# xiph/daala

Measured on NVIDIA H100. Metric: encoder Mpixels/s on 4K YUV420 intra, higher is better.
Workload: dtype int32

## Files before the change

### daala_b200/csrc/abi_host.cu

```cuda
#include <cuda_runtime.h>
#include <stdio.h>
#include <stdlib.h>
#include <string.h>

#include <stddef.h>

#include <mutex>

#include "daala_b200.h"
#include "frame_transform.h"

extern "C" {
int daala_b200_launch_forward(const FrameXformParams* prm, int nplanes, cudaStream_t stream);
int daala_b200_launch_forward_no_tma(const FrameXformParams* prm, int nplanes, cudaStream_t stream);
int daala_b200_launch_inverse(const FrameXformParams* prm, int nplanes, cudaStream_t stream);
int daala_b200_launch_inverse_lapped_only(const FrameXformParams* prm, int nplanes, cudaStream_t stream);
int daala_b200_launch_sb_postfilter_store(const FrameXformParams* prm, int nplanes, cudaStream_t stream);
int daala_b200_launch_plane_sb_filter(int32_t* c, int stride, int nhsb, int nvsb, int xdec, int ydec,
                                      int post, cudaStream_t stream);
int daala_b200_launch_block_transform(int32_t* blocks, int count, int ln, int mode, cudaStream_t stream);
int daala_b200_launch_filter4(int32_t* v, long count, int post, cudaStream_t stream);
int daala_b200_launch_haar_blocks(int32_t* blocks, int count, int ln, int inverse, cudaStream_t stream);
int daala_b200_pvq_helper_launch(void* buf, int op, void* stream);
int daala_b200_pvq_helper_bytes(void);
int daala_b200_launch_lapfilter(int32_t* v, long count, int n, int post, cudaStream_t stream);
int daala_b200_launch_split_filter(int32_t* blocks, int count, int n, int post, int hfilter, int vfilter,
                                   cudaStream_t stream);
}

namespace {

[[noreturn]] void fatal(const char* what, cudaError_t err) {
  fprintf(stderr, "libdaala_b200: fatal: %s: %s (no CPU fallback exists)\n", what,
          cudaGetErrorString(err));
  abort();
}

#define CK(call)                                    \
  do {                                              \
    cudaError_t e_ = (call);                        \
    if (e_ != cudaSuccess) fatal(#call, e_);        \
  } while (0)

struct HostCtx {
  cudaStream_t stream = nullptr;
  void* pinned = nullptr;
  void* dev = nullptr;
  size_t cap = 0;
  std::mutex mu;

  void ensure(size_t bytes) {
    if (!stream) {
      int n = 0;
      cudaError_t e = cudaGetDeviceCount(&n);
      if (e != cudaSuccess || n == 0) fatal("cudaGetDeviceCount", e == cudaSuccess ? cudaErrorNoDevice : e);
      CK(cudaStreamCreateWithFlags(&stream, cudaStreamNonBlocking));
    }
    if (bytes > cap) {
      size_t ncap = cap ? cap : (size_t)1 << 20;
      while (ncap < bytes) ncap <<= 1;
      if (pinned) CK(cudaFreeHost(pinned));
      if (dev) CK(cudaFree(dev));
      CK(cudaMallocHost(&pinned, ncap));
      CK(cudaMalloc(&dev, ncap));
      cap = ncap;
    }
  }
  void h2d(size_t bytes) { CK(cudaMemcpyAsync(dev, pinned, bytes, cudaMemcpyHostToDevice, stream)); }
  void d2h(size_t bytes) {
    CK(cudaMemcpyAsync(pinned, dev, bytes, cudaMemcpyDeviceToHost, stream));
    CK(cudaStreamSynchronize(stream));
  }
};

HostCtx& ctx() {
  static HostCtx c;
  return c;
}

void check_launch(int rc, const char* what) {
  if (rc != 0) fatal(what, (cudaError_t)rc);
}

void dct1d(int ln, bool inverse, od_coeff* out, int out_stride, const od_coeff* in, int in_stride) {
  HostCtx& c = ctx();
  std::lock_guard<std::mutex> g(c.mu);
  const int n = 1 << ln;
  c.ensure(sizeof(od_coeff) * n * n);
  od_coeff* p = (od_coeff*)c.pinned;
  memset(p, 0, sizeof(od_coeff) * n * n);
  for (int i = 0; i < n; i++) p[i] = in[i * in_stride];
  c.h2d(sizeof(od_coeff) * n * n);
  check_launch(daala_b200_launch_block_transform((int32_t*)c.dev, 1, ln, inverse ? 3 : 2, c.stream),
               "block_transform(1d)");
  c.d2h(sizeof(od_coeff) * n);
  for (int i = 0; i < n; i++) out[i * out_stride] = p[i];
}

void haar2d(int ln, bool inverse, od_coeff* out, int out_stride, const od_coeff* in, int in_stride) {
  HostCtx& c = ctx();
  std::lock_guard<std::mutex> g(c.mu);
  const int n = 1 << ln;
  c.ensure(sizeof(od_coeff) * n * n);
  od_coeff* p = (od_coeff*)c.pinned;
  for (int i = 0; i < n; i++) memcpy(p + i * n, in + (size_t)i * in_stride, sizeof(od_coeff) * n);
  c.h2d(sizeof(od_coeff) * n * n);
  check_launch(daala_b200_launch_haar_blocks((int32_t*)c.dev, 1, ln, inverse ? 1 : 0, c.stream), "haar_blocks");
  c.d2h(sizeof(od_coeff) * n * n);
  for (int i = 0; i < n; i++) memcpy(out + (size_t)i * out_stride, p + i * n, sizeof(od_coeff) * n);
}

void dct2d(int ln, bool inverse, od_coeff* out, int out_stride, const od_coeff* in, int in_stride) {
  HostCtx& c = ctx();
  std::lock_guard<std::mutex> g(c.mu);
  const int n = 1 << ln;
  c.ensure(sizeof(od_coeff) * n * n);
  od_coeff* p = (od_coeff*)c.pinned;
  for (int i = 0; i < n; i++) memcpy(p + i * n, in + (size_t)i * in_stride, sizeof(od_coeff) * n);
  c.h2d(sizeof(od_coeff) * n * n);
  check_launch(daala_b200_launch_block_transform((int32_t*)c.dev, 1, ln, inverse ? 1 : 0, c.stream),
               "block_transform(2d)");
  c.d2h(sizeof(od_coeff) * n * n);
  for (int i = 0; i < n; i++) memcpy(out + (size_t)i * out_stride, p + i * n, sizeof(od_coeff) * n);
}

void filter4(bool post, od_coeff* out, const od_coeff* in) {
  HostCtx& c = ctx();
  std::lock_guard<std::mutex> g(c.mu);
  c.ensure(sizeof(od_coeff) * 4);
  memcpy(c.pinned, in, sizeof(od_coeff) * 4);
  c.h2d(sizeof(od_coeff) * 4);
  check_launch(daala_b200_launch_filter4((int32_t*)c.dev, 1, post, c.stream), "filter4");
  c.d2h(sizeof(od_coeff) * 4);
  memcpy(out, c.pinned, sizeof(od_coeff) * 4);
}

void lapfilter_n(int n, bool post, od_coeff* out, const od_coeff* in) {
  HostCtx& c = ctx();
  std::lock_guard<std::mutex> g(c.mu);
  c.ensure(sizeof(od_coeff) * n);
  memcpy(c.pinned, in, sizeof(od_coeff) * n);
  c.h2d(sizeof(od_coeff) * n);
  check_launch(daala_b200_launch_lapfilter((int32_t*)c.dev, 1, n, post, c.stream), "lapfilter");
  c.d2h(sizeof(od_coeff) * n);
  memcpy(out, c.pinned, sizeof(od_coeff) * n);
}

void split_filter(bool post, od_coeff* c0, int stride, int bs, int hfilter, int vfilter) {
  HostCtx& c = ctx();
  std::lock_guard<std::mutex> g(c.mu);
  const int n = 4 << bs;
  c.ensure(sizeof(od_coeff) * n * n);
  od_coeff* p = (od_coeff*)c.pinned;
  for (int i = 0; i < n; i++) memcpy(p + i * n, c0 + (size_t)i * stride, sizeof(od_coeff) * n);
  c.h2d(sizeof(od_coeff) * n * n);
  check_launch(daala_b200_launch_split_filter((int32_t*)c.dev, 1, n, post, hfilter, vfilter, c.stream),
               "split_filter");
  c.d2h(sizeof(od_coeff) * n * n);
  for (int i = 0; i < n; i++) memcpy(c0 + (size_t)i * stride, p + i * n, sizeof(od_coeff) * n);
}

void plane_sb_filter(bool post, od_coeff* c0, int stride, int nhsb, int nvsb, int xdec, int ydec) {
  HostCtx& c = ctx();
  std::lock_guard<std::mutex> g(c.mu);
  const int w = (nhsb * 64) >> xdec, h = (nvsb * 64) >> ydec;
  const size_t bytes = sizeof(od_coeff) * (size_t)w * h;
  c.ensure(bytes);
  od_coeff* p = (od_coeff*)c.pinned;
  for (int i = 0; i < h; i++) memcpy(p + (size_t)i * w, c0 + (size_t)i * stride, sizeof(od_coeff) * w);
  c.h2d(bytes);
  check_launch(daala_b200_launch_plane_sb_filter((int32_t*)c.dev, w, nhsb, nvsb, xdec, ydec, post, c.stream),
               "plane_sb_filter");
  c.d2h(bytes);
  for (int i = 0; i < h; i++) memcpy(c0 + (size_t)i * stride, p + (size_t)i * w, sizeof(od_coeff) * w);
}

}

extern "C" {

#define DAALA_B200_DCT(N, LN)                                                                     \
  void od_bin_fdct##N(od_coeff* y, const od_coeff* x, int xstride) { dct1d(LN, false, y, 1, x, xstride); } \
  void od_bin_idct##N(od_coeff* x, int xstride, const od_coeff* y) { dct1d(LN, true, x, xstride, y, 1); }  \
  void od_bin_fdct##N##x##N(od_coeff* y, int ystride, const od_coeff* x, int xstride) {          \
    dct2d(LN, false, y, ystride, x, xstride);                                                    \
  }                                                                                              \
  void od_bin_idct##N##x##N(od_coeff* x, int xstride, const od_coeff* y, int ystride) {          \
    dct2d(LN, true, x, xstride, y, ystride);                                                     \
  }
DAALA_B200_DCT(4, 2)
DAALA_B200_DCT(8, 3)
DAALA_B200_DCT(16, 4)
DAALA_B200_DCT(32, 5)
DAALA_B200_DCT(64, 6)

void od_haar(od_coeff* y, int ystride, const od_coeff* x, int xstride, int ln) { haar2d(ln, false, y, ystride, x, xstride); }
void od_haar_inv(od_coeff* x, int xstride, const od_coeff* y, int ystride, int ln) { haar2d(ln, true, x, xstride, y, ystride); }

const od_dct_func_2d OD_FDCT_2D_CUDA[6] = {od_bin_fdct4x4,   od_bin_fdct8x8,   od_bin_fdct16x16,
                                           od_bin_fdct32x32, od_bin_fdct64x64, nullptr};
const od_dct_func_2d OD_IDCT_2D_CUDA[6] = {od_bin_idct4x4,   od_bin_idct8x8,   od_bin_idct16x16,
                                           od_bin_idct32x32, od_bin_idct64x64, nullptr};

void od_pre_filter4(od_coeff _y[4], const od_coeff _x[4]) { filter4(false, _y, _x); }
void od_post_filter4(od_coeff _x[4], const od_coeff _y[4]) { filter4(true, _x, _y); }

void od_pre_filter8(od_coeff _y[8], const od_coeff _x[8]) { lapfilter_n(8, false, _y, _x); }
void od_post_filter8(od_coeff _x[8], const od_coeff _y[8]) { lapfilter_n(8, true, _x, _y); }
void od_pre_filter16(od_coeff _y[16], const od_coeff _x[16]) { lapfilter_n(16, false, _y, _x); }
void od_post_filter16(od_coeff _x[16], const od_coeff _y[16]) { lapfilter_n(16, true, _x, _y); }
void od_pre_filter32(od_coeff _y[32], const od_coeff _x[32]) { lapfilter_n(32, false, _y, _x); }
void od_post_filter32(od_coeff _x[32], const od_coeff _y[32]) { lapfilter_n(32, true, _x, _y); }

const od_dct_func_2d OD_FDCT_2D_C[6] = {od_bin_fdct4x4,   od_bin_fdct8x8,   od_bin_fdct16x16,
                                        od_bin_fdct32x32, od_bin_fdct64x64, nullptr};
const od_dct_func_2d OD_IDCT_2D_C[6] = {od_bin_idct4x4,   od_bin_idct8x8,   od_bin_idct16x16,
                                        od_bin_idct32x32, od_bin_idct64x64, nullptr};
const od_fdct_func_1d OD_FDCT_1D[6] = {od_bin_fdct4, od_bin_fdct8, od_bin_fdct16, od_bin_fdct32, od_bin_fdct64, nullptr};
const od_idct_func_1d OD_IDCT_1D[6] = {od_bin_idct4, od_bin_idct8, od_bin_idct16, od_bin_idct32, od_bin_idct64, nullptr};

const od_filter_func OD_PRE_FILTER_CUDA[4] = {od_pre_filter4, od_pre_filter8, od_pre_filter16, od_pre_filter32};
const od_filter_func OD_POST_FILTER_CUDA[4] = {od_post_filter4, od_post_filter8, od_post_filter16, od_post_filter32};

const od_filter_func OD_PRE_FILTER[5] = {od_pre_filter4, od_pre_filter8, od_pre_filter16, od_pre_filter32, nullptr};
const od_filter_func OD_POST_FILTER[5] = {od_post_filter4, od_post_filter8, od_post_filter16, od_post_filter32, nullptr};
const int OD_FILTER_PARAMS4[4] = {85, 75, -15, 33};

int daala_b200_lapfilter(int32_t* v, long count, int n, int post, void* stream) {
  return daala_b200_launch_lapfilter(v, count, n, post, (cudaStream_t)stream);
}

void od_prefilter_split(od_coeff* c0, int stride, int bs, int f, int hfilter, int vfilter) {
  (void)f;
  split_filter(false, c0, stride, bs, hfilter, vfilter);
}

void od_postfilter_split(od_coeff* c0, int stride, int bs, int f, int q, unsigned char* skip,
                         int skip_stride, int hfilter, int vfilter) {
  (void)f; (void)q; (void)skip; (void)skip_stride;
  split_filter(true, c0, stride, bs, hfilter, vfilter);
}

void od_apply_prefilter_frame_sbs(od_coeff* c, int stride, int nhsb, int nvsb, int xdec, int ydec) {
  plane_sb_filter(false, c, stride, nhsb, nvsb, xdec, ydec);
}

void od_apply_postfilter_frame_sbs(od_coeff* c, int stride, int nhsb, int nvsb, int xdec, int ydec,
                                   int q, unsigned char* skip, int skip_stride) {
  (void)q; (void)skip; (void)skip_stride;
  plane_sb_filter(true, c, stride, nhsb, nvsb, xdec, ydec);
}

void od_mc_predict1fmv8_cuda(void* state, unsigned char* dst, const unsigned char* src, int systride,
                             int32_t mvx, int32_t mvy, int log_xblk_sz, int log_yblk_sz) {
  (void)state;
  HostCtx& c = ctx();
  std::lock_guard<std::mutex> g(c.mu);
  const int nx = 1 << log_xblk_sz, ny = 1 << log_yblk_sz;
  const int W = nx + 5, H = ny + 5;
  const size_t win = (size_t)W * H, job_off = (win + 15) & ~(size_t)15, out_off = job_off + 16;
  c.ensure(out_off + (size_t)nx * ny);
  unsigned char* p = (unsigned char*)c.pinned;
  const unsigned char* s0 = src + ((mvx >> 3) - 2) + (ptrdiff_t)((mvy >> 3) - 2) * systride;
  const int c_lo = (mvx & 7) ? 0 : 2, c_hi = (mvx & 7) ? W : 2 + nx;
  const int r_lo = (mvy & 7) ? 0 : 2, r_hi = (mvy & 7) ? H : 2 + ny;
  memset(p, 0, win);
  for (int r = r_lo; r < r_hi; r++) memcpy(p + (size_t)r * W + c_lo, s0 + (ptrdiff_t)r * systride + c_lo, c_hi - c_lo);
  daala_b200_match_job job;
  memset(&job, 0, sizeof(job));
  job.mvx = mvx & 7; job.mvy = mvy & 7; job.x0 = 2; job.y0 = 2; job.log_blk = (uint8_t)log_xblk_sz;
  memcpy(p + job_off, &job, sizeof(job));
  c.h2d(out_off);
  unsigned char* d = (unsigned char*)c.dev;
  check_launch(daala_b200_mc_predict1fmv_batch(d, W, d + out_off, nx * ny, (const daala_b200_match_job*)(d + job_off),
                                               1, log_yblk_sz, c.stream), "mc_predict1fmv");
  CK(cudaMemcpyAsync(p + out_off, d + out_off, (size_t)nx * ny, cudaMemcpyDeviceToHost, c.stream));
  CK(cudaStreamSynchronize(c.stream));
  memcpy(dst, p + out_off, (size_t)nx * ny);
}

static void blend_host(unsigned char* dst, int dystride, const unsigned char* src[4], int oc, int s, int lx, int ly) {
  HostCtx& c = ctx();
  std::lock_guard<std::mutex> g(c.mu);
  const int nx = 1 << lx, ny = 1 << ly, n2 = nx * ny;
  c.ensure((size_t)5 * n2);
  unsigned char* p = (unsigned char*)c.pinned;
  for (int k = 0; k < 4; k++) memcpy(p + (size_t)k * n2, src[k], n2);
  c.h2d((size_t)4 * n2);
  unsigned char* d = (unsigned char*)c.dev;
  check_launch(daala_b200_mc_blend_packed(d, n2, d + (size_t)4 * n2, nx, oc, s, lx, ly, c.stream), "mc_blend");
  CK(cudaMemcpyAsync(p + (size_t)4 * n2, d + (size_t)4 * n2, n2, cudaMemcpyDeviceToHost, c.stream));
  CK(cudaStreamSynchronize(c.stream));
  for (int j = 0; j < ny; j++) memcpy(dst + (size_t)j * dystride, p + (size_t)4 * n2 + (size_t)j * nx, nx);
}

void od_mc_blend_full8_cuda(unsigned char* dst, int dystride, const unsigned char* src[4], int log_xblk_sz,
                            int log_yblk_sz) {
  blend_host(dst, dystride, src, 0, 3, log_xblk_sz, log_yblk_sz);
}

void od_mc_blend_full_split8_cuda(unsigned char* dst, int dystride, const unsigned char* src[4], int c, int s,
                                  int log_xblk_sz, int log_yblk_sz) {
  blend_host(dst, dystride, src, c, s, log_xblk_sz, log_yblk_sz);
}

static int32_t match_host(int ln, int use_satd, const unsigned char* src, int systride, const unsigned char* ref,
                          int dystride) {
  HostCtx& c = ctx();
  std::lock_guard<std::mutex> g(c.mu);
  const int n = 1 << ln, n2 = n * n;
  const size_t job_off = (size_t)2 * n2, res_off = job_off + 16;
  c.ensure(res_off + 16);
  unsigned char* p = (unsigned char*)c.pinned;
  for (int j = 0; j < n; j++) {
    memcpy(p + (size_t)j * n, src + (ptrdiff_t)j * systride, n);
    memcpy(p + n2 + (size_t)j * n, ref + (ptrdiff_t)j * dystride, n);
  }
  daala_b200_match_job job;
  memset(&job, 0, sizeof(job));
  job.log_blk = (uint8_t)ln;
  memcpy(p + job_off, &job, sizeof(job));
  c.h2d(res_off);
  unsigned char* d = (unsigned char*)c.dev;
  check_launch(daala_b200_mc_match_candidates(d, n, d + n2, n, (const daala_b200_match_job*)(d + job_off), 1,
                                              use_satd, (int32_t*)(d + res_off), c.stream), "mc_match");
  CK(cudaMemcpyAsync(p + res_off, d + res_off, 4, cudaMemcpyDeviceToHost, c.stream));
  CK(cudaStreamSynchronize(c.stream));
  int32_t r;
  memcpy(&r, p + res_off, 4);
  return r;
}

#define DAALA_B200_MATCH(N, LN)                                                                            \
  int32_t od_mc_compute_sad8_##N##x##N##_cuda(const unsigned char* src, int systride, const unsigned char* ref, \
                                              int dystride) {                                             \
    return match_host(LN, 0, src, systride, ref, dystride);                                               \
  }                                                                                                       \
  int32_t od_mc_compute_satd8_##N##x##N##_cuda(const unsigned char* src, int systride, const unsigned char* ref, \
                                               int dystride) {                                            \
    return match_host(LN, 1, src, systride, ref, dystride);                                               \
  }
DAALA_B200_MATCH(4, 2)
DAALA_B200_MATCH(8, 3)
DAALA_B200_MATCH(16, 4)
DAALA_B200_MATCH(32, 5)
DAALA_B200_MATCH(64, 6)

struct PvqHelperBuf {
  int32_t args[16];
  int16_t a16[2][128];
  int32_t a32[2][128];
  int16_t qmi[128];
  double dargs[2];
};

static PvqHelperBuf* helper_begin(HostCtx& c) {
  if ((size_t)daala_b200_pvq_helper_bytes() != sizeof(PvqHelperBuf)) fatal("pvq helper layout", cudaErrorInvalidValue);
  c.ensure(sizeof(PvqHelperBuf));
  PvqHelperBuf* b = (PvqHelperBuf*)c.pinned;
  memset(b, 0, sizeof(*b));
  return b;
}

static void helper_run(HostCtx& c, int op) {
  c.h2d(sizeof(PvqHelperBuf));
  check_launch(daala_b200_pvq_helper_launch(c.dev, op, c.stream), "pvq_helper");
  c.d2h(sizeof(PvqHelperBuf));
}

#define HELPER_SCALAR(OP, ...)                      \
  HostCtx& c = ctx();                               \
  std::lock_guard<std::mutex> g_(c.mu);             \
  PvqHelperBuf* b = helper_begin(c);                \
  { int32_t v_[] = {__VA_ARGS__}; memcpy(b->args, v_, sizeof(v_)); } \
  helper_run(c, OP);

int16_t od_pvq_sin(int32_t x) { HELPER_SCALAR(0, x) return (int16_t)b->args[15]; }
int16_t od_pvq_cos(int32_t x) { HELPER_SCALAR(1, x) return (int16_t)b->args[15]; }
int32_t od_gain_expand(int32_t cg, int q0, int16_t beta) { HELPER_SCALAR(6, cg, q0, beta) return b->args[15]; }
int od_pvq_compute_max_theta(int32_t qcg, int16_t beta) { HELPER_SCALAR(8, qcg, beta) return b->args[15]; }
int32_t od_pvq_compute_theta(int t, int max_theta) { HELPER_SCALAR(9, t, max_theta) return b->args[15]; }
int od_pvq_compute_k(int32_t qcg, int itheta, int32_t theta, int noref, int n, int16_t beta, int nodesync) {
  (void)theta; (void)nodesync;
  HELPER_SCALAR(10, qcg, itheta, noref, n, beta)
  return b->args[15];
}

int od_vector_log_mag(const od_coeff* x, int n) {
  HostCtx& c = ctx();
  std::lock_guard<std::mutex> g_(c.mu);
  PvqHelperBuf* b = helper_begin(c);
  b->args[0] = n;
  memcpy(b->a32[0], x, sizeof(od_coeff) * n);
  helper_run(c, 2);
  return b->args[15];
}

int od_compute_householder(int16_t* r, int n, int32_t gr, int* sign, int shift) {
  HostCtx& c = ctx();
  std::lock_guard<std::mutex> g_(c.mu);
  PvqHelperBuf* b = helper_begin(c);
  b->args[0] = n; b->args[1] = gr; b->args[2] = shift;
  memcpy(b->a16[0], r, sizeof(int16_t) * n);
  helper_run(c, 3);
  memcpy(r, b->a16[0], sizeof(int16_t) * n);
  *sign = b->args[14];
  return b->args[15];
}

void od_apply_householder(int16_t* out, const int16_t* x, const int16_t* r, int n) {
  HostCtx& c = ctx();
  std::lock_guard<std::mutex> g_(c.mu);
  PvqHelperBuf* b = helper_begin(c);
  b->args[0] = n;
  memcpy(b->a16[0], r, sizeof(int16_t) * n);
  memcpy(b->a16[1], x, sizeof(int16_t) * n);
  helper_run(c, 4);
  memcpy(out, b->a16[1], sizeof(int16_t) * n);
}

void od_pvq_synthesis_partial(od_coeff* xcoeff, const od_coeff* ypulse, const int16_t* r, int n, int noref,
                              int32_t g, int32_t theta, int m, int s, const int16_t* qm_inv) {
  HostCtx& c = ctx();
  std::lock_guard<std::mutex> g_(c.mu);
  PvqHelperBuf* b = helper_begin(c);
  b->args[0] = n; b->args[1] = noref; b->args[2] = g; b->args[3] = theta; b->args[4] = m; b->args[5] = s;
  memcpy(b->a32[0], ypulse, sizeof(od_coeff) * (n - !noref));
  if (r) memcpy(b->a16[0], r, sizeof(int16_t) * n);
  memcpy(b->qmi, qm_inv, sizeof(int16_t) * n);
  helper_run(c, 5);
  memcpy(xcoeff, b->a32[1], sizeof(od_coeff) * n);
}

int32_t od_pvq_compute_gain(const int16_t* x, int n, int q0, int32_t* g, int16_t beta, int bshift) {
  HostCtx& c = ctx();
  std::lock_guard<std::mutex> g_(c.mu);
  PvqHelperBuf* b = helper_begin(c);
  b->args[0] = n; b->args[1] = q0; b->args[2] = beta; b->args[3] = bshift;
  memcpy(b->a16[0], x, sizeof(int16_t) * n);
  helper_run(c, 7);
  *g = b->args[14];
  return b->args[15];
}

int od_rdo_quant(od_coeff x, int q, double delta0, double pvq_norm_lambda) {
  HostCtx& c = ctx();
  std::lock_guard<std::mutex> g_(c.mu);
  PvqHelperBuf* b = helper_begin(c);
  b->args[0] = x; b->args[1] = q; b->dargs[0] = delta0; b->dargs[1] = pvq_norm_lambda;
  helper_run(c, 11);
  return b->args[15];
}

int daala_b200_forward_frame(const daala_b200_frame* f, int nplanes, void* stream) {
  return daala_b200_launch_forward(f, nplanes, (cudaStream_t)stream);
}
int daala_b200_forward_frame_no_tma(const daala_b200_frame* f, int nplanes, void* stream) {
  return daala_b200_launch_forward_no_tma(f, nplanes, (cudaStream_t)stream);
}
int daala_b200_inverse_frame(const daala_b200_frame* f, int nplanes, void* stream) {
  return daala_b200_launch_inverse(f, nplanes, (cudaStream_t)stream);
}
int daala_b200_inverse_frame_lapped(const daala_b200_frame* f, int nplanes, void* stream) {
  return daala_b200_launch_inverse_lapped_only(f, nplanes, (cudaStream_t)stream);
}
int daala_b200_sb_postfilter_store_frame(const daala_b200_frame* f, int nplanes, void* stream) {
  return daala_b200_launch_sb_postfilter_store(f, nplanes, (cudaStream_t)stream);
}
int daala_b200_plane_sb_filter(int32_t* c, int stride, int nhsb, int nvsb, int xdec, int ydec, int post,
                               void* stream) {
  return daala_b200_launch_plane_sb_filter(c, stride, nhsb, nvsb, xdec, ydec, post, (cudaStream_t)stream);
}
int daala_b200_haar_blocks(int32_t* blocks, int count, int ln, int inverse, void* stream) {
  return daala_b200_launch_haar_blocks(blocks, count, ln, inverse, (cudaStream_t)stream);
}

int daala_b200_block_transform(int32_t* blocks, int count, int ln, int mode, void* stream) {
  return daala_b200_launch_block_transform(blocks, count, ln, mode, (cudaStream_t)stream);
}

int daala_b200_device_count(void) {
  int n = 0;
  if (cudaGetDeviceCount(&n) != cudaSuccess) return 0;
  return n;
}

const char* daala_b200_version(void) { return "daala_b200 0.1 (sm_90a)"; }

}
```

### daala_b200/csrc/frame_transform.cu

```cuda
#include <cuda.h>
#include <cuda_runtime.h>
#include <cudaTypedefs.h>
#include <stdint.h>
#include <stdio.h>
#include <string.h>

#include "gen/dct_lifting.cuh"
#include "lapped_filter.cuh"
#include "frame_transform.h"

namespace daala_b200 {

#ifndef DAALA_XFORM_THREADS
#define DAALA_XFORM_THREADS 64
#endif
constexpr int kThreads = DAALA_XFORM_THREADS;
constexpr int kPostThreads = 128;
constexpr int kCtasPerSm = 512 / kThreads;
constexpr int kGridCap = 132 * 8;
constexpr int kMaxB = 64;
constexpr int kHalo = 2;
constexpr int kMaxT = kMaxB + 2 * kHalo;
constexpr int kMaxPitch = kMaxT + 1;

// ... 413 lines not shown
k_inverse_sb(const __grid_constant__ FrameXformParams prm) {
  __shared__ int tile_s[kMaxB * kMaxPitch];
  __shared__ SbLists lists;
  const PlaneXform& pl = prm.plane[blockIdx.y];
  if (pl.xdec == 0) inverse_sb_body<0>(prm, pl, tile_s, lists);
  else inverse_sb_body<1>(prm, pl, tile_s, lists);
}

template <int XDEC>
__device__ __forceinline__ void sb_postfilter_store_body(const FrameXformParams& prm,
                                                         const PlaneXform& pl, int* tile_s) {
  constexpr int B = kMaxB >> XDEC;
  constexpr int T = B + 2 * kHalo;
  constexpr int P = T + 1;
  const int sbx = blockIdx.x % prm.nhsb, sby = prm.sb_row0 + blockIdx.x / prm.nhsb;
  const int fr = blockIdx.z;
  const int32_t* lap = pl.lapped + fr * pl.lapped_frame_pitch;
  const int x0 = sbx * B, y0 = sby * B;
  const int pw = prm.nhsb * B, ph = prm.nvsb * B;
  const int32_t* core = lap + (size_t)y0 * pl.lapped_stride + x0;
  if (rows_aligned16(core, pl.lapped_stride)) {
    tile_copy4<B, P, false, kPostThreads>(tile_s + kHalo * P + kHalo, const_cast<int32_t*>(core), pl.lapped_stride);
    for (int i = threadIdx.x; i < 4 * T + 4 * B; i += kPostThreads) {
      int r, c;
      if (i < 4 * T) {
        const int k = i / T;
        r = k < 2 ? k : B + k;
        c = i - k * T;
      } else {
        const int j = i - 4 * T, k = j / B;
        c = k < 2 ? k : B + k;
        r = j - k * B + kHalo;
      }
      const int gx = x0 + c - kHalo, gy = y0 + r - kHalo;
      int v = 0;
      if (gx >= 0 && gx < pw && gy >= 0 && gy < ph) v = lap[(size_t)gy * pl.lapped_stride + gx];
      tile_s[r * P + c] = v;
    }
  } else {
    for (int i = threadIdx.x; i < T * T; i += kPostThreads) {
      int r = i / T, c = i - r * T;
      int gx = x0 + c - kHalo, gy = y0 + r - kHalo;
      int v = 0;
      if (gx >= 0 && gx < pw && gy >= 0 && gy < ph) v = lap[(size_t)gy * pl.lapped_stride + gx];
      tile_s[r * P + c] = v;
    }
  }
  __syncthreads();
  const bool left = sbx > 0, right = sbx + 1 < prm.nhsb;
  for (int i = threadIdx.x; i < 2 * T; i += kPostThreads) {
    int e = i >= T, r = i - e * T;
    if (e == 0 ? left : right) lap4_inplace<true>(tile_s + r * P + (e ? B : 0), 1);
  }
  __syncthreads();
  const bool top = sby > 0, bottom = sby + 1 < prm.nvsb;
  for (int i = threadIdx.x; i < 2 * B; i += kPostThreads) {
    int c = i % B + kHalo, e = i / B;
    if (e == 0 ? top : bottom) lap4_inplace<true>(tile_s + (e ? B : 0) * P + c, P);
  }
  __syncthreads();
  if (prm.post16[blockIdx.y]) {
    int16_t* d16 = prm.post16[blockIdx.y] + fr * pl.pixel_out_frame_pitch + (size_t)y0 * pl.pixel_out_stride + x0;
    for (int i = threadIdx.x; i < B * B / 2; i += kPostThreads) {
      int r = i / (B / 2), c2 = (i % (B / 2)) * 2;
      const int* p = tile_s + (r + kHalo) * P + c2 + kHalo;
      const unsigned w = ((unsigned)p[0] & 0xffffu) | ((unsigned)p[1] << 16);
      *reinterpret_cast<unsigned*>(d16 + (size_t)r * pl.pixel_out_stride + c2) = w;
    }
    return;
  }
  uint8_t* dst = pl.pixels_out + fr * pl.pixel_out_frame_pitch + (size_t)y0 * pl.pixel_out_stride + x0;
  for (int i = threadIdx.x; i < B * B / 4; i += kPostThreads) {
    int r = i / (B / 4), c4 = (i % (B / 4)) * 4;
    const int* p = tile_s + (r + kHalo) * P + c4 + kHalo;
    unsigned w = 0;
#pragma unroll
    for (int k = 0; k < 4; k++) {
      int v = ((p[k] + 8) >> 4) + 128;
      v = v < 0 ? 0 : (v > 255 ? 255 : v);
      w |= (unsigned)v << (8 * k);
    }
    *reinterpret_cast<unsigned*>(dst + (size_t)r * pl.pixel_out_stride + c4) = w;
  }
}

__global__ void __launch_bounds__(kPostThreads)
k_sb_postfilter_store(const __grid_constant__ FrameXformParams prm) {
  __shared__ int tile_s[kMaxT * kMaxPitch];
  const PlaneXform& pl = prm.plane[blockIdx.y];
  if (pl.xdec == 0) sb_postfilter_store_body<0>(prm, pl, tile_s);
  else sb_postfilter_store_body<1>(prm, pl, tile_s);
}

template <bool kPost>
__global__ void k_plane_sb_edges(int32_t* c, int stride, int nhsb, int nvsb, int sbw, int sbh,
                                 bool vertical_taps) {
  const int w = nhsb * sbw, h = nvsb * sbh;
  const int along = vertical_taps ? w : h;
  const int edges = (vertical_taps ? nvsb : nhsb) - 1;
  const long total = (long)along * edges;
  for (long i = blockIdx.x * (long)blockDim.x + threadIdx.x; i < total;
       i += (long)gridDim.x * blockDim.x) {
    int a = (int)(i % along), e = (int)(i / along) + 1;
    if (vertical_taps) lap4_inplace<kPost>(c + (size_t)(e * sbh - 2) * stride + a, stride);
    else lap4_inplace<kPost>(c + (size_t)a * stride + e * sbw - 2, 1);
  }
}

template <int L>
__global__ void __launch_bounds__(64)
k_block_transform(int32_t* blocks, int mode) {
  constexpr int N = 1 << L;
  constexpr int P = N + 5;
  __shared__ int t[N * P];
  int32_t* blk = blocks + (size_t)blockIdx.x * N * N;
  for (int i = threadIdx.x; i < N * N; i += blockDim.x) t[(i / N) * P + (i % N)] = blk[i];
  __syncthreads();
  const bool fwd = (mode & 1) == 0;
  const int passes = mode < 2 ? 2 : 1;
  for (int pass = 0; pass < passes; pass++) {
    bool cols = mode < 2 ? (fwd ? pass == 0 : pass == 1) : false;
    if (threadIdx.x < N) {
      int* p = cols ? t + threadIdx.x : t + threadIdx.x * P;
      int stride = cols ? P : 1;
      int v[N];
#pragma unroll
      for (int k = 0; k < N; k++) v[k] = p[k * stride];
      if (fwd) Lifting<N>::fwd(v); else Lifting<N>::inv(v);
#pragma unroll
      for (int k = 0; k < N; k++) p[k * stride] = v[k];
    }
    __syncthreads();
  }
  for (int i = threadIdx.x; i < N * N; i += blockDim.x) blk[i] = t[(i / N) * P + (i % N)];
}

__global__ void k_filter4_batch(int32_t* v, long count, int post) {
  for (long i = blockIdx.x * (long)blockDim.x + threadIdx.x; i < count;
       i += (long)gridDim.x * blockDim.x) {
    if (post) lap4_inplace<true>(v + 4 * i, 1); else lap4_inplace<false>(v + 4 * i, 1);
  }
}

template <int N>
__global__ void k_lapfilter_batch(int32_t* v, long count, int post) {
  for (long i = blockIdx.x * (long)blockDim.x + threadIdx.x; i < count; i += (long)gridDim.x * blockDim.x) {
    int t[N];
#pragma unroll
    for (int k = 0; k < N; k++) t[k] = v[i * N + k];
    if (post) LapFilter<N>::post(t); else LapFilter<N>::pre(t);
#pragma unroll
    for (int k = 0; k < N; k++) v[i * N + k] = t[k];
  }
}

__global__ void k_split_filter_batch(int32_t* blocks, int n, int post, int hfilter, int vfilter) {
  int32_t* b = blocks + (size_t)blockIdx.x * n * n;
  for (int phase = 0; phase < 2; phase++) {
    bool vertical_taps = post ? phase == 1 : phase == 0;
    if (vertical_taps ? hfilter : vfilter) {
      for (int i = threadIdx.x; i < n; i += blockDim.x) {
        if (vertical_taps) {
          if (post) lap4_inplace<true>(b + (n / 2 - 2) * n + i, n); else lap4_inplace<false>(b + (n / 2 - 2) * n + i, n);
        } else {
          if (post) lap4_inplace<true>(b + i * n + n / 2 - 2, 1); else lap4_inplace<false>(b + i * n + n / 2 - 2, 1);
        }
      }
    }
    __syncthreads();
  }
}

}

using namespace daala_b200;

template <bool kInverse>
__global__ void __launch_bounds__(256) k_haar_blocks(int32_t* __restrict__ blocks, int ln) {
  __shared__ int t[64 * 64];
  const int n = 1 << ln;
  int32_t* g = blocks + (size_t)blockIdx.x * n * n;
  if (!kInverse) {
    for (int i = threadIdx.x; i < n * n; i += 256) t[i] = g[i];
    __syncthreads();
    for (int level = 0; level < ln; level++) {
      const int np = n >> level >> 1;
      int keep[4];
      int q = 0;
      for (int idx = threadIdx.x; idx < np * np; idx += 256, q++) {
        const int i = idx / np, j = idx - i * np;
        int ll = t[2 * i * n + 2 * j], lh = t[(2 * i + 1) * n + 2 * j];
        int hl = t[2 * i * n + 2 * j + 1], hh = t[(2 * i + 1) * n + 2 * j + 1];
        ll += hl;
        hh -= lh;
        const int m = (ll - hh) >> 1;
        lh = m - lh;
        hl = m - hl;
        ll -= lh;
        hh += hl;
        keep[q] = ll;
        g[i * n + j + np] = lh;
        g[(i + np) * n + j] = hl;
        g[(i + np) * n + j + np] = hh;
      }
      __syncthreads();
      q = 0;
      for (int idx = threadIdx.x; idx < np * np; idx += 256, q++) {
        const int i = idx / np, j = idx - i * np;
        t[i * n + j] = keep[q];
      }
      __syncthreads();
    }
    if (threadIdx.x == 0) g[0] = t[0];
  } else {
    if (threadIdx.x == 0) t[0] = g[0];
    __syncthreads();
    for (int level = ln - 1; level >= 0; level--) {
      const int np = 1 << (ln - 1 - level);
      int a4[4], b4[4], c4[4], d4[4];
      int q = 0;
      for (int idx = threadIdx.x; idx < np * np; idx += 256, q++) {
        const int i = idx / np, j = idx - i * np;
        int ll = t[i * n + j], lh = g[i * n + j + np], hl = g[(i + np) * n + j], hh = g[(i + np) * n + j + np];
        ll += hl;
        hh -= lh;
        const int m = (ll - hh) >> 1;
        lh = m - lh;
        hl = m - hl;
        ll -= lh;
        hh += hl;
        a4[q] = ll; b4[q] = lh; c4[q] = hl; d4[q] = hh;
      }
      __syncthreads();
      q = 0;
      for (int idx = threadIdx.x; idx < np * np; idx += 256, q++) {
        const int i = idx / np, j = idx - i * np;
        t[2 * i * n + 2 * j] = a4[q];
        t[(2 * i + 1) * n + 2 * j] = b4[q];
        t[2 * i * n + 2 * j + 1] = c4[q];
        t[(2 * i + 1) * n + 2 * j + 1] = d4[q];
      }
      __syncthreads();
    }
    for (int i = threadIdx.x; i < n * n; i += 256) g[i] = t[i];
  }
}

extern "C" {

static bool encode_input_maps(const FrameXformParams* prm, int nplanes, TmaMaps* maps) {
  static PFN_cuTensorMapEncodeTiled_v12000 encode = nullptr;
  static bool tried = false;
  if (!tried) {
    tried = true;
    void* fn = nullptr;
    cudaDriverEntryPointQueryResult q;
    if (cudaGetDriverEntryPoint("cuTensorMapEncodeTiled", &fn, cudaEnableDefault, &q) == cudaSuccess &&
        q == cudaDriverEntryPointSuccess)
      encode = (PFN_cuTensorMapEncodeTiled_v12000)fn;
  }
  if (!encode) return false;
  memset(maps, 0, sizeof(*maps));
  for (int p = 0; p < nplanes; p++) {
    const PlaneXform& pl = prm->plane[p];
    const int B = kMaxB >> pl.xdec;
    const cuuint64_t w = (cuuint64_t)prm->nhsb * B, h = (cuuint64_t)prm->nvsb * B;
    const cuuint64_t fpitch = prm->nframes > 1 ? (cuuint64_t)pl.pixel_frame_pitch : w * h;
    if (((uintptr_t)pl.pixels & 15) || (pl.pixel_stride & 15) || (fpitch & 15) || pl.pixel_stride <= 0) return false;
    cuuint64_t dims[3] = {w, h, (cuuint64_t)prm->nframes};
    cuuint64_t strides[2] = {(cuuint64_t)pl.pixel_stride, fpitch};
    cuuint32_t box[3] = {(cuuint32_t)(pl.xdec ? RawTile<1>::width : RawTile<0>::width),
                         (cuuint32_t)(B + 2 * kHalo), 1};
    cuuint32_t estr[3] = {1, 1, 1};
    CUresult r = encode(&maps->plane[p], CU_TENSOR_MAP_DATA_TYPE_UINT8, 3, (void*)pl.pixels, dims, strides, box,
                        estr, CU_TENSOR_MAP_INTERLEAVE_NONE, CU_TENSOR_MAP_SWIZZLE_NONE,
                        CU_TENSOR_MAP_L2_PROMOTION_L2_128B, CU_TENSOR_MAP_FLOAT_OOB_FILL_NONE);
    if (r != CUDA_SUCCESS) return false;
  }
  return true;
}

int daala_b200_launch_forward(const FrameXformParams* prm, int nplanes, cudaStream_t stream) {
  dim3 grid(prm->nhsb * prm->sb_rows, nplanes, prm->nframes);
  TmaMaps maps;
  if (encode_input_maps(prm, nplanes, &maps))
    k_forward_sb_tma<<<grid, kThreads, 0, stream>>>(*prm, maps.plane[0], maps.plane[1], maps.plane[2]);
  else k_forward_sb<<<grid, kThreads, 0, stream>>>(*prm);
  return (int)cudaGetLastError();
}

int daala_b200_launch_forward_no_tma(const FrameXformParams* prm, int nplanes, cudaStream_t stream) {
  dim3 grid(prm->nhsb * prm->sb_rows, nplanes, prm->nframes);
  k_forward_sb<<<grid, kThreads, 0, stream>>>(*prm);
  return (int)cudaGetLastError();
}

int daala_b200_launch_inverse(const FrameXformParams* prm, int nplanes, cudaStream_t stream) {
  dim3 grid(prm->nhsb * prm->sb_rows, nplanes, prm->nframes);
  k_inverse_sb<<<grid, kThreads, 0, stream>>>(*prm);
  k_sb_postfilter_store<<<grid, kPostThreads, 0, stream>>>(*prm);
  return (int)cudaGetLastError();
}

int daala_b200_launch_inverse_lapped_only(const FrameXformParams* prm, int nplanes, cudaStream_t stream) {
  dim3 grid(prm->nhsb * prm->sb_rows, nplanes, prm->nframes);
  k_inverse_sb<<<grid, kThreads, 0, stream>>>(*prm);
  return (int)cudaGetLastError();
}

int daala_b200_launch_sb_postfilter_store(const FrameXformParams* prm, int nplanes, cudaStream_t stream) {
  dim3 grid(prm->nhsb * prm->sb_rows, nplanes, prm->nframes);
  k_sb_postfilter_store<<<grid, kPostThreads, 0, stream>>>(*prm);
  return (int)cudaGetLastError();
}

int daala_b200_launch_plane_sb_filter(int32_t* c, int stride, int nhsb, int nvsb, int xdec, int ydec,
                                      int post, cudaStream_t stream) {
  const int sbw = 64 >> xdec, sbh = 64 >> ydec;
  for (int phase = 0; phase < 2; phase++) {
    bool vertical_taps = post ? phase == 1 : phase == 0;
    long total = vertical_taps ? (long)nhsb * sbw * (nvsb - 1) : (long)nvsb * sbh * (nhsb - 1);
    if (total <= 0) continue;
    int blocks = (int)((total + 255) / 256);
    if (blocks > kGridCap) blocks = kGridCap;
    if (post) k_plane_sb_edges<true><<<blocks, 256, 0, stream>>>(c, stride, nhsb, nvsb, sbw, sbh, vertical_taps);
    else k_plane_sb_edges<false><<<blocks, 256, 0, stream>>>(c, stride, nhsb, nvsb, sbw, sbh, vertical_taps);
  }
  return (int)cudaGetLastError();
}

int daala_b200_launch_block_transform(int32_t* blocks, int count, int ln, int mode, cudaStream_t stream) {
  if (count <= 0) return 0;
  switch (ln) {
    case 2: k_block_transform<2><<<count, 64, 0, stream>>>(blocks, mode); break;
    case 3: k_block_transform<3><<<count, 64, 0, stream>>>(blocks, mode); break;
    case 4: k_block_transform<4><<<count, 64, 0, stream>>>(blocks, mode); break;
    case 5: k_block_transform<5><<<count, 64, 0, stream>>>(blocks, mode); break;
    case 6: k_block_transform<6><<<count, 64, 0, stream>>>(blocks, mode); break;
    default: return (int)cudaErrorInvalidValue;
  }
  return (int)cudaGetLastError();
}

int daala_b200_launch_haar_blocks(int32_t* blocks, int count, int ln, int inverse, cudaStream_t stream) {
  if (count <= 0) return 0;
  if (ln < 1 || ln > 6) return (int)cudaErrorInvalidValue;
  if (inverse) k_haar_blocks<true><<<count, 256, 0, stream>>>(blocks, ln);
  else k_haar_blocks<false><<<count, 256, 0, stream>>>(blocks, ln);
  return (int)cudaGetLastError();
}

int daala_b200_launch_filter4(int32_t* v, long count, int post, cudaStream_t stream) {
  if (count <= 0) return 0;
  int blocks = (int)((count + 255) / 256);
  if (blocks > kGridCap) blocks = kGridCap;
  k_filter4_batch<<<blocks, 256, 0, stream>>>(v, count, post);
  return (int)cudaGetLastError();
}

int daala_b200_launch_lapfilter(int32_t* v, long count, int n, int post, cudaStream_t stream) {
  if (count <= 0) return 0;
  int blocks = (int)((count + 127) / 128);
  if (blocks > kGridCap) blocks = kGridCap;
  if (n == 4) k_filter4_batch<<<blocks, 128, 0, stream>>>(v, count, post);
  else if (n == 8) k_lapfilter_batch<8><<<blocks, 128, 0, stream>>>(v, count, post);
  else if (n == 16) k_lapfilter_batch<16><<<blocks, 128, 0, stream>>>(v, count, post);
  else if (n == 32) k_lapfilter_batch<32><<<blocks, 128, 0, stream>>>(v, count, post);
  else return (int)cudaErrorInvalidValue;
  return (int)cudaGetLastError();
}

int daala_b200_launch_split_filter(int32_t* blocks, int count, int n, int post, int hfilter, int vfilter,
                                   cudaStream_t stream) {
  if (count <= 0) return 0;
  k_split_filter_batch<<<count, 64, 0, stream>>>(blocks, n, post, hfilter, vfilter);
  return (int)cudaGetLastError();
}

}
```

### daala_b200/csrc/kf_engine.cu

```cuda
#include <cuda_runtime.h>
#include <math.h>
#include <stdint.h>
#include <stdio.h>
#include <stdlib.h>
#include <string.h>

#include <algorithm>
#include <cmath>
#include <mutex>
#include <new>
#include <vector>

#include "daala_b200.h"
#include "dering_search.h"
#include "late_skip.h"
#include "mc_batch.h"
#include "gen/coding_order.inc"
#include "pvq_math.cuh"
#include "pvq_warp.cuh"
#include "pvq_common.cuh"

namespace daala_b200 {
namespace kf {

using namespace daala_b200::pvq;

enum Cnt {
  kNLuma = 0, kNChroma, kLumaCoefs, kChromaCoefs,
  kNItemsL = 4,
  kNItemsC = 7,
  kTotalHi = 14,
  kNHeads = 15,
  kNHeads0 = 16,
  kError = 17,
  kDepsDone = 18,
  kMcBadRef = 19,
  kMcBeyond = 20,
  kHeadLoL = 32,
  kHeadLoC = 64,
  kHeadHi = 96,
  kTailHi = 128,
  kDoneHi = 160,
  kHeadCh = 192,
  kWaiters = 224,
  kTraceN = 240,
  kCntWords = 256
};

constexpr int kTile = 1024;
constexpr int kMaxLevels = 4096;
constexpr int kLevelBins = kMaxLevels * 3;

struct Lists {
  const uint8_t* bsize;
  int bstride;
  long long bsize_pitch;
  int F, UW, UH;
  int u_row0, u_rows;
  int ntiles;
  int4* tile_sum;
  int32_t* unit_lbase;
  daala_b200_pvq_block* luma;
  daala_b200_pvq_block* chroma;
  int32_t* dep_top;
  int32_t* dep_left;
  int32_t* succ_bottom;
  int32_t* succ_right;
  uint32_t* items_l[3];
  uint32_t* items_c[3];
  uint32_t* heads;
  uint32_t* heads0;
  uint32_t* heads_raw;
  int32_t* head_bin;
  int32_t* head_hist;
  int32_t* head_cursor;
  int32_t* cnt;
  int32_t* lvl_hist;
  int32_t* lvl_cursor;
  uint32_t* lvl_items;
  int nlevels;
  int max_luma, max_chroma;
};

__device__ __forceinline__ int4 add4(int4 a, int4 b) { return make_int4(a.x + b.x, a.y + b.y, a.z + b.z, a.w + b.w); }

__device__ __forceinline__ int4 unit_counts(int b, int ux, int uy) {
  if (b == 0) return make_int4(4, 64, 1, 16);
  const int span = 1 << (b - 1);
  if ((ux & (span - 1)) | (uy & (span - 1))) return make_int4(0, 0, 0, 0);
  const int lc = b == 1 ? 64 : b == 2 ? 256 : 512;
  const int cc = b == 1 ? 16 : b == 2 ? 64 : b == 3 ? 256 : 512;
  return make_int4(1, lc, 1, cc);
}

__device__ __forceinline__ bool unit_of(const Lists& L, long long i, int* f, int* uy, int* ux, int* b) {
  const long long per = (long long)L.u_rows * L.UW;
  if (i >= per * L.F) return false;
  *f = (int)(i / per);
  const int r = (int)(i - (long long)*f * per);
  *uy = L.u_row0 + r / L.UW;
  *ux = r % L.UW;
  *b = L.bsize[*f * L.bsize_pitch + (long long)*uy * L.bstride + *ux];
  return true;
}

__global__ void __launch_bounds__(kTile) k_unit_tile_sums(const __grid_constant__ Lists L) {
  __shared__ int4 part[32];
  const long long i = (long long)blockIdx.x * kTile + threadIdx.x;
  int f, uy, ux, b;
  int4 v = make_int4(0, 0, 0, 0);
  if (unit_of(L, i, &f, &uy, &ux, &b)) v = unit_counts(b, ux, uy);
#pragma unroll
  for (int o = 16; o > 0; o >>= 1) {
    v.x += __shfl_xor_sync(0xffffffffu, v.x, o);
    v.y += __shfl_xor_sync(0xffffffffu, v.y, o);
    v.z += __shfl_xor_sync(0xffffffffu, v.z, o);
    v.w += __shfl_xor_sync(0xffffffffu, v.w, o);
  }
  if ((threadIdx.x & 31) == 0) part[threadIdx.x >> 5] = v;
  __syncthreads();
  if (threadIdx.x == 0) {
    int4 s = make_int4(0, 0, 0, 0);
    for (int w = 0; w < kTile / 32; w++) s = add4(s, part[w]);
    L.tile_sum[blockIdx.x] = s;
  }
}

__global__ void __launch_bounds__(1024) k_tile_scan(const __grid_constant__ Lists L) {
  __shared__ int4 part[1024];
  __shared__ int4 carry;
  const int t = threadIdx.x;
  if (t == 0) carry = make_int4(0, 0, 0, 0);
  __syncthreads();
  for (int base = 0; base < L.ntiles; base += 1024) {
    const int i = base + t;
    const int4 v = i < L.ntiles ? L.tile_sum[i] : make_int4(0, 0, 0, 0);
    part[t] = v;
    __syncthreads();
    for (int o = 1; o < 1024; o <<= 1) {
      const int4 a = t >= o ? part[t - o] : make_int4(0, 0, 0, 0);
      __syncthreads();
      part[t] = add4(part[t], a);
      __syncthreads();
    }
    const int4 incl = part[t], c = carry;
    if (i < L.ntiles) L.tile_sum[i] = make_int4(c.x + incl.x - v.x, c.y + incl.y - v.y, c.z + incl.z - v.z, c.w + incl.w - v.w);
    __syncthreads();
    if (t == 1023) carry = add4(c, incl);
    __syncthreads();
  }
  if (t == 0) {
    const int4 tot = carry;
    L.cnt[kNLuma] = tot.x;
    L.cnt[kLumaCoefs] = tot.y;
    L.cnt[kNChroma] = 2 * tot.z;
    L.cnt[kChromaCoefs] = 2 * tot.w;
    for (int c = 0; c < 3; c++) {
      L.cnt[kNItemsL + c] = 0;
      L.cnt[kNItemsC + c] = 0;
    }
    L.cnt[kTotalHi] = 0;
    L.cnt[kNHeads] = 0;
    L.cnt[kNHeads0] = 0;
    L.cnt[kDepsDone] = 0;
    L.cnt[kError] = tot.x > L.max_luma || 2 * tot.z > L.max_chroma ? 1 : 0;
  }
}

__device__ __forceinline__ void put_block(daala_b200_pvq_block* dst, int coef_off, int x0, int y0, int bs, int pli,
                                          int xdec, int frame) {
  int32_t* w = reinterpret_cast<int32_t*>(dst);
  w[0] = coef_off;
  w[1] = (x0 & 0xffff) | (y0 << 16);
  w[2] = bs | (pli << 8) | (xdec << 16) | (frame << 24);
}

__global__ void __launch_bounds__(kTile) k_unit_emit(const __grid_constant__ Lists L) {
  __shared__ int4 wsum[32];
  const long long i = (long long)blockIdx.x * kTile + threadIdx.x;
  const int lane = threadIdx.x & 31, warp = threadIdx.x >> 5;
  int f = 0, uy = 0, ux = 0, b = 0;
  const bool valid = unit_of(L, i, &f, &uy, &ux, &b);
  const int4 v = valid ? unit_counts(b, ux, uy) : make_int4(0, 0, 0, 0);
  int4 s = v;
#pragma unroll
  for (int o = 1; o < 32; o <<= 1) {
    int4 a;
    a.x = __shfl_up_sync(0xffffffffu, s.x, o);
    a.y = __shfl_up_sync(0xffffffffu, s.y, o);
    a.z = __shfl_up_sync(0xffffffffu, s.z, o);
    a.w = __shfl_up_sync(0xffffffffu, s.w, o);
    if (lane >= o) s = add4(s, a);
  }
  if (lane == 31) wsum[warp] = s;
  __syncthreads();
  int4 pre = L.tile_sum[blockIdx.x];
  for (int w = 0; w < warp; w++) pre = add4(pre, wsum[w]);
  pre = make_int4(pre.x + s.x - v.x, pre.y + s.y - v.y, pre.z + s.z - v.z, pre.w + s.w - v.w);
  if (!valid) return;
  L.unit_lbase[((long long)f * L.UH + uy) * L.UW + ux] = pre.x;
  if (v.x == 0) return;
  if (pre.x + v.x > L.max_luma || 2 * (pre.z + v.z) > L.max_chroma) return;
  if (b == 0) {
    for (int q = 0; q < 4; q++)
      put_block(L.luma + pre.x + q, pre.y + 16 * q, ux * 8 + (q & 1) * 4, uy * 8 + (q >> 1) * 4, 0, 0, 0, f);
  } else {
    put_block(L.luma + pre.x, pre.y, ux * 8, uy * 8, b, 0, 0, f);
  }
  const int cbs = (b > 1 ? b : 1) - 1;
  const int xd = 1 | (b == 0 ? 0x80 : 0);
  put_block(L.chroma + 2 * pre.z, 2 * pre.w, ux * 4, uy * 4, cbs, 1, xd, f);
  put_block(L.chroma + 2 * pre.z + 1, 2 * pre.w + v.w, ux * 4, uy * 4, cbs, 2, xd, f);
}

__device__ __forceinline__ int band_class(int band) { return band < 3 ? 0 : band < 6 ? 1 : 2; }

__device__ __forceinline__ int level_bin(int band, int bs, int x0, int y0, int y_first) {
  const int sh = bs + 2, bx = x0 >> sh, by = (y0 - y_first) >> sh;
  const int r = band % 3;
  const int lvl = band == 0 ? bx + by : r == 1 ? by : bx;
  return lvl * 3 + (2 - band_class(band));
}

__device__ __forceinline__ int append(uint32_t* list, int32_t* counter, bool pred, uint32_t v) {
  const unsigned m = __ballot_sync(__activemask(), pred);
  if (!pred) return -1;
  const int lane = threadIdx.x & 31, leader = __ffs(m) - 1;
  int base = 0;
  if (lane == leader) base = atomicAdd(counter, __popc(m));
  base = __shfl_sync(m, base, leader);
  const int pos = base + __popc(m & ((1u << lane) - 1u));
  list[pos] = v;
  return pos;
}

__device__ __forceinline__ int count_key(int32_t* ctr, int key) {
  const unsigned same = __match_any_sync(__activemask(), key);
  const int lane = threadIdx.x & 31, leader = __ffs(same) - 1;
  int base = 0;
  if (lane == leader) base = atomicAdd(&ctr[key], __popc(same));
  return __shfl_sync(same, base, leader) + __popc(same & ((1u << lane) - 1u));
}

constexpr int kChainCost0 = 7, kChainCost1 = 9, kChainCost2 = 18;
__device__ __forceinline__ int weight_bin(int len, int band) {
  const int c = band_class(band);
  const int w = len * (c == 0 ? kChainCost0 : c == 1 ? kChainCost1 : kChainCost2);
  return kLevelBins - 1 - min(w, kLevelBins - 1);
}

__device__ int chain_length(const Lists& L, const uint8_t* map, int x0, int y0, int bs, bool down) {
  const int nn = 4 << bs, y_end = (L.u_row0 + L.u_rows) * 8, x_end = L.UW * 8;
  int len = 1;
  for (int x = x0 + (down ? 0 : nn), y = y0 + (down ? nn : 0); x < x_end && y < y_end;
       x += down ? 0 : nn, y += down ? nn : 0, len++) {
    if (map[(long long)(y >> 3) * L.bstride + (x >> 3)] != bs) break;
    const int py = down ? y - 1 : y, px = down ? x : x - 1;
    if (map[(long long)(py >> 3) * L.bstride + (px >> 3)] != bs) break;
  }
  return len;
}

template <int kThreads>
__device__ __forceinline__ void scan_bins(int32_t* hist, int32_t* cursor) {
  __shared__ int part[kThreads];
  constexpr int kPer = kLevelBins / kThreads;
  const int t = threadIdx.x;
  int v[kPer], sum = 0;
#pragma unroll
  for (int i = 0; i < kPer; i++) {
    v[i] = __ldcg(hist + t * kPer + i);
    sum += v[i];
  }
  part[t] = sum;
  __syncthreads();
  for (int o = 1; o < kThreads; o <<= 1) {
    const int add = t >= o ? part[t - o] : 0;
    __syncthreads();
    part[t] += add;
    __syncthreads();
  }
  int run = part[t] - sum;
#pragma unroll
  for (int i = 0; i < kPer; i++) {
    hist[t * kPer + i] = run;
    cursor[t * kPer + i] = run;
    run += v[i];
  }
}

__global__ void __launch_bounds__(256) k_luma_deps(const __grid_constant__ Lists L) {
  const int n = min(L.cnt[kNLuma], L.max_luma);
  const int nth = gridDim.x * blockDim.x;
  for (int base = blockIdx.x * blockDim.x; base < n; base += nth) {
    const int blk = base + threadIdx.x;
    const bool in = blk < n;
    int bs = 0, top = -1, left = -1;
    if (in) {
      const daala_b200_pvq_block b = L.luma[blk];
      const int x0 = b.x0, y0 = b.y0, f = b.frame;
      bs = b.bs;
      const int nn = 4 << bs;
      const uint8_t* map = L.bsize + f * L.bsize_pitch;
      if (y0 - nn >= L.u_row0 * 8 && map[(long long)((y0 - 1) >> 3) * L.bstride + (x0 >> 3)] == bs) {
        const int ty = y0 - nn;
        top = L.unit_lbase[((long long)f * L.UH + (ty >> 3)) * L.UW + (x0 >> 3)] +
              (bs == 0 ? ((ty >> 2) & 1) * 2 + ((x0 >> 2) & 1) : 0);
      }
      if (x0 > 0 && map[(long long)(y0 >> 3) * L.bstride + ((x0 - 1) >> 3)] == bs) {
        const int lx = x0 - nn;
        left = L.unit_lbase[((long long)f * L.UH + (y0 >> 3)) * L.UW + (lx >> 3)] +
               (bs == 0 ? ((y0 >> 2) & 1) * 2 + ((lx >> 2) & 1) : 0);
      }
      L.dep_top[blk] = top;
      L.dep_left[blk] = left;
      if (top >= 0) L.succ_bottom[top] = blk;
      if (left >= 0) L.succ_right[left] = blk;
    }
    const int nb = in ? num_bands(bs) : 0;
    int len_down = 0, len_across = 0;
    if (nb > 1) {
      const daala_b200_pvq_block b = L.luma[blk];
      const uint8_t* map = L.bsize + b.frame * L.bsize_pitch;
      if (top < 0) len_down = chain_length(L, map, b.x0, b.y0, bs, true);
      if (left < 0) len_across = chain_length(L, map, b.x0, b.y0, bs, false);
    }
    int chain = 0;
    for (int band = 0; band < 9; band++) {
      const bool has = band < nb;
      const bool is_free = band == 3 || band == 6;
      const int r = band % 3;
      const bool waits = band == 0 ? (top >= 0 || left >= 0) : r == 1 ? top >= 0 : left >= 0;
      const uint32_t item = ((uint32_t)blk << 4) | band;
      if (band == 3 || band == 6) {
        append(L.items_l[band_class(band)], &L.cnt[kNItemsL + band_class(band)], has, item);
      } else if (band == 0) {
        append(L.heads0, &L.cnt[kNHeads0], has && !waits, item);
      } else {
        const int pos = append(L.heads_raw, &L.cnt[kNHeads], has && !waits, item);
        if (pos >= 0) {
          const int bin = weight_bin(r == 1 ? len_down : len_across, band);
          L.head_bin[pos] = bin;
          count_key(L.head_hist, bin);
        }
      }
      chain += has && !is_free;
      if (has && !is_free && L.lvl_hist) {
        const daala_b200_pvq_block b = L.luma[blk];
        atomicAdd(&L.lvl_hist[level_bin(band, bs, b.x0, b.y0, L.u_row0 * 8)], 1);
      }
    }
#pragma unroll
    for (int o = 16; o > 0; o >>= 1) chain += __shfl_xor_sync(0xffffffffu, chain, o);
    if ((threadIdx.x & 31) == 0 && chain) atomicAdd(&L.cnt[kTotalHi], chain);
  }
  __shared__ bool last;
  __threadfence();
  __syncthreads();
  if (threadIdx.x == 0) last = atomicAdd(&L.cnt[kDepsDone], 1) == (int)gridDim.x - 1;
  __syncthreads();
  if (last) {
    __threadfence();
    scan_bins<256>(L.head_hist, L.head_cursor);
  }
}

__global__ void __launch_bounds__(1024) k_level_scan(const __grid_constant__ Lists L) {
  scan_bins<1024>(L.lvl_hist, L.lvl_cursor);
}

__global__ void __launch_bounds__(256) k_level_scatter(const __grid_constant__ Lists L) {
  const int n = min(L.cnt[kNLuma], L.max_luma);
  for (int blk = blockIdx.x * blockDim.x + threadIdx.x; blk < n; blk += gridDim.x * blockDim.x) {
    const daala_b200_pvq_block b = L.luma[blk];
    const int nb = num_bands(b.bs);
    for (int band = 0; band < nb; band++) {
      if (band == 3 || band == 6) continue;
      const int pos = atomicAdd(&L.lvl_cursor[level_bin(band, b.bs, b.x0, b.y0, L.u_row0 * 8)], 1);
      L.lvl_items[pos] = ((uint32_t)blk << 4) | band;
    }
  }
}

__global__ void __launch_bounds__(256) k_chroma_items(const __grid_constant__ Lists L) {
  const int nh = L.cnt[kNHeads];
  for (int i = blockIdx.x * blockDim.x + threadIdx.x; i < nh; i += gridDim.x * blockDim.x)
    L.heads[count_key(L.head_cursor, L.head_bin[i])] = L.heads_raw[i];
  const int n = min(L.cnt[kNChroma], L.max_chroma);
  for (int blk = blockIdx.x * blockDim.x + threadIdx.x; blk < n; blk += gridDim.x * blockDim.x) {
    const int bs = L.chroma[blk].bs;
    const int nb = num_bands(bs);
    for (int band = 0; band < nb; band++) {
      const int c = band_class(band);
      const unsigned m = __activemask();
      const unsigned same = __match_any_sync(m, c);
      const int leader = __ffs(same) - 1, lane = threadIdx.x & 31;
      int base = 0;
      if (lane == leader) base = atomicAdd(&L.cnt[kNItemsC + c], __popc(same));
      base = __shfl_sync(same, base, leader);
      L.items_c[c][base + __popc(same & ((1u << lane) - 1u))] = ((uint32_t)blk << 4) | band;
    }
  }
}

__global__ void __launch_bounds__(256) k_luma_items(const __grid_constant__ Lists L) {
  const int n = min(L.cnt[kNLuma], L.max_luma);
  const int nth = gridDim.x * blockDim.x;
  for (int base = blockIdx.x * blockDim.x; base < n; base += nth) {
    const int blk = base + threadIdx.x;
    const int nb = blk < n ? num_bands(L.luma[blk].bs) : 0;
    for (int band = 0; band < 9; band++) {
      const int c = band_class(band);
      append(L.items_l[c], &L.cnt[kNItemsL + c], band < nb, ((uint32_t)blk << 4) | band);
    }
  }
}

struct Stage {
  daala_b200_pvq_params prm;
  const uint32_t* items[3];
  const uint32_t* heads;
  const uint32_t* heads0;
  uint32_t* ring;
  const int32_t* dep_top;
  const int32_t* dep_left;
  const int32_t* succ_bottom;
  const int32_t* succ_right;
  int32_t* join0;
  int32_t* cnt;
  int n_items_at, head_lo_at, n_blocks_at;
  int max_blocks;
  int16_t* sp_vec[3];
  int32_t* sp_lanes[3];
  int32_t* sp_uni[3];
  int16_t* sp_snap[3];
  int sp_slots[3];
  int sp_chunks[3];
  const int32_t* lvl_off;
  const uint32_t* lvl_items;
  int nlevels, lvl_slots;
  int16_t* lv_vec; int32_t* lv_lanes; int32_t* lv_uni; int16_t* lv_snap;
  int32_t* lv_bar;
  int32_t* pre_ev;
  int16_t* pre_snap;
  int max_waiters;
  int skip_lo;
  const double* rsqrt_tbl;
  int16_t* res_pack;
  const int32_t* cfl_plane;
  long long cfl_pitch;
  int cfl_stride;
  int32_t* dc_resid;
  const daala_b200_kf_frame_quant* fq;
#ifdef DAALA_B200_CHAIN_TRACE
  struct ChainTraceRec* trace;
  int trace_cap;
#endif
};

#ifdef DAALA_B200_CHAIN_TRACE
struct ChainTraceRec {
  unsigned long long t0, t1;
  uint32_t item;
  uint32_t cta;
  uint16_t sm;
  uint8_t bs;
  uint8_t kind;
  uint32_t pad;
};

__device__ __forceinline__ unsigned long long globaltimer() {
  unsigned long long t;
  asm volatile("mov.u64 %0, %%globaltimer;" : "=l"(t));
  return t;
}

__device__ __noinline__ void trace_item(const Stage& S, uint32_t item, int kind, unsigned long long t0, int lane) {
  __syncwarp();
  if (lane != 0) return;
  const unsigned long long t1 = globaltimer();
  const int i = atomicAdd(&S.cnt[kTraceN], 1);
  if (i >= S.trace_cap) return;
  uint32_t sm;
  asm volatile("mov.u32 %0, %%smid;" : "=r"(sm));
  ChainTraceRec r;
  r.t0 = t0;
  r.t1 = t1;
  r.item = item;
  r.cta = blockIdx.x;
  r.sm = (uint16_t)sm;
  r.bs = (uint8_t)S.prm.blocks[item >> 4].bs;
  r.kind = (uint8_t)kind;
  r.pad = 0;
  S.trace[i] = r;
}
#endif

enum { kGatherLuma = 0, kGatherChroma = 1, kGatherInter = 2 };
template <int kKind>
__global__ void __launch_bounds__(256) k_gather(const __grid_constant__ Stage S) {
  const daala_b200_pvq_params& prm = S.prm;
  const int n = min(S.cnt[S.n_blocks_at], S.max_blocks);
  const int lane = threadIdx.x & 31;
  const int nwarps = (gridDim.x * blockDim.x) >> 5;
  for (int blk = (blockIdx.x * blockDim.x + threadIdx.x) >> 5; blk < n; blk += nwarps) {
    const daala_b200_pvq_block b = prm.blocks[blk];
    const int ln = b.bs + 2;
    const int len = ln >= 5 ? 512 : 1 << (2 * ln);
    const int stride = prm.plane_stride[b.pli];
    const int32_t* src = prm.coef_plane[b.pli] + b.frame * prm.plane_frame_pitch[b.pli] + (size_t)b.y0 * stride + b.x0;
    int32_t* vin = prm.in + b.coef_off;
    if (kKind == kGatherLuma) {
      for (int i = lane; i < len; i += 32) vin[i] = i == 0 ? src[0] : src[scan_to_raster(i, ln, stride)];
    } else if (kKind == kGatherInter) {
      const int32_t* psrc = prm.pred_plane[b.pli] + b.frame * prm.plane_frame_pitch[b.pli] + (size_t)b.y0 * stride + b.x0;
      int32_t* vref = prm.ref + b.coef_off;
      for (int i = lane; i < len; i += 32) {
        const int at = i == 0 ? 0 : scan_to_raster(i, ln, stride);
        vin[i] = src[at];
        vref[i] = psrc[at];
      }
    } else {
      const int32_t* psrc = S.cfl_plane + b.frame * S.cfl_pitch + (size_t)b.y0 * S.cfl_stride + b.x0;
      int32_t* vref = prm.ref + b.coef_off;
      const int qoff = prm.qm_stride + ((((1 << (2 * b.bs)) - 1) << 4) / 3);
      int32_t xy = 0;
      for (int i = lane; i < len; i += 32) {
        const int32_t vi = i == 0 ? src[0] : src[scan_to_raster(i, ln, stride)];
        const int32_t vr = i == 0 ? psrc[0] : psrc[scan_to_raster(i, ln, S.cfl_stride)];
        vin[i] = vi;
        vref[i] = vr;
        if (i >= 1 && i < 16) {
          const int32_t rq = vr * prm.qm[qoff + i], inq = vi * prm.qm[qoff + i];
          xy += (int32_t)((rq * (int64_t)inq) >> ((kQmShift + 4) << 1));
        }
      }
#pragma unroll
      for (int o = 16; o > 0; o >>= 1) xy += __shfl_xor_sync(0xffffffffu, xy, o);
      const int flip = xy < 0;
      __syncwarp();
      if (flip) {
        const int end = band_start(num_bands(b.bs));
        for (int i = 1 + lane; i < end; i += 32) vref[i] = -vref[i];
      }
      if (lane == 0) prm.res_flip[blk] = flip;
    }
  }
}

__global__ void __launch_bounds__(256) k_cfl_plane(const __grid_constant__ Stage S, int32_t* pred_plane) {
  const daala_b200_pvq_params& prm = S.prm;
  const int n = min(S.cnt[S.n_blocks_at], S.max_blocks);
  const int lane = threadIdx.x & 31;
  const int nwarps = (gridDim.x * blockDim.x) >> 5;
  for (int blk = (blockIdx.x * blockDim.x + threadIdx.x) >> 5; blk < n; blk += nwarps) {
    const daala_b200_pvq_block b = prm.blocks[blk];
    if (b.pli != 1) continue;
    const int nn = 4 << b.bs;
    const int lstride = prm.plane_stride[0];
    const int32_t* luma = prm.coef_plane[0] + b.frame * prm.plane_frame_pitch[0] + (size_t)(2 * b.y0) * lstride + 2 * b.x0;
    int32_t* dst = pred_plane + b.frame * S.cfl_pitch + (size_t)b.y0 * S.cfl_stride + b.x0;
    if (b.xdec & 0x80) {
      const int scaling4[4][4] = {{128, 128, 100, 36}, {128, 80, 71, 35}, {100, 71, 35, 31}, {36, 35, 31, 18}};
      if (lane < 4) {
        const int x = lane & 1, y = lane >> 1;
        int ll = luma[(size_t)y * lstride + x], lh = luma[(size_t)y * lstride + x + 4];
        int hl = luma[(size_t)(y + 4) * lstride + x], hh = luma[(size_t)(y + 4) * lstride + x + 4];
        ll += lh; hh -= hl;
        const int t = (ll - hh) >> 1;
        hl = t - hl; lh = t - lh;
        ll -= hl; hh += lh;
        const int hs = x & 1, vs = y & 1;
        int r, c;
        r = 2 * y + vs; c = 2 * x + hs;         dst[(size_t)r * S.cfl_stride + c] = (scaling4[c][r] * ll + 64) >> 7;
        r = 2 * y + vs; c = 2 * x + 1 - hs;     dst[(size_t)r * S.cfl_stride + c] = (scaling4[c][r] * lh + 64) >> 7;
        r = 2 * y + 1 - vs; c = 2 * x + hs;     dst[(size_t)r * S.cfl_stride + c] = (scaling4[c][r] * hl + 64) >> 7;
        r = 2 * y + 1 - vs; c = 2 * x + 1 - hs; dst[(size_t)r * S.cfl_stride + c] = (scaling4[c][r] * hh + 64) >> 7;
      }
    } else {
      const int lim = nn > 32 ? 32 : nn;
      for (int i = lane; i < lim * lim; i += 32) {
        const int r = i / lim, c = i % lim;
        dst[(size_t)r * S.cfl_stride + c] = luma[(size_t)r * lstride + c];
      }
    }
  }
}

constexpr int kPersistThreads = 32;
constexpr int kPersistCtas = 32;
static_assert(kPersistCtas * (kPersistThreads / 32 * kSnapEntries * (int)sizeof(int16_t) + 1024) <= 228 * 1024,
              "k_pvq_persist's shared scratch does not fit kPersistCtas CTAs per SM");
constexpr uint32_t kNoItem = 0xffffffffu;
constexpr uint32_t kExit = 0xfffffffeu;

__device__ __forceinline__ int ld_relaxed(const int32_t* p) {
  int v;
  asm volatile("ld.relaxed.gpu.global.s32 %0, [%1];" : "=r"(v) : "l"(p) : "memory");
  return v;
}

__device__ __forceinline__ void push_chain(const Stage& S, int blk, int band) {
  const int pos = atomicAdd(&S.cnt[kTailHi], 1) - S.cnt[kNHeads0];
  st_release((int*)&S.ring[pos], (int)(((uint32_t)blk << 4) | band));
}

template <bool kIntra>
__device__ __forceinline__ uint32_t next_item(const Stage& S, int lane, int* done, bool* waiter) {
  int slot = -1, head = -1, lo = -1, nheads0 = 0, fin = -1;
  if (lane == 0) {
    const int n2 = S.cnt[S.n_items_at + 2], n1 = S.cnt[S.n_items_at + 1], n0 = S.cnt[S.n_items_at];
    const int nlo = S.skip_lo ? 0 : n0 + n1 + n2;
    if (kIntra) {
      nheads0 = S.cnt[kNHeads0];
      if (*done) {
        const int d = atomicAdd(&S.cnt[kDoneHi], *done) + *done;
        if (d == S.cnt[kNLuma]) {
          __threadfence();
          fin = ld_relaxed(&S.cnt[kTailHi]) - nheads0;
        }
      }
      if (ld_relaxed(&S.cnt[kHeadHi]) < ld_relaxed(&S.cnt[kTailHi])) slot = atomicAdd(&S.cnt[kHeadHi], 1);
      if (slot < 0 && ld_relaxed(&S.cnt[kHeadCh]) < S.cnt[kNHeads]) {
        const int h = atomicAdd(&S.cnt[kHeadCh], 1);
        if (h < S.cnt[kNHeads]) head = h;
      }
    }
    if (slot < 0 && head < 0 && ld_relaxed(&S.cnt[S.head_lo_at]) < nlo) {
      const int l = atomicAdd(&S.cnt[S.head_lo_at], 1);
      if (l < nlo) lo = l;
    }
    if (kIntra && slot < 0 && head < 0 && lo < 0) {
      if (!*waiter && atomicAdd(&S.cnt[kWaiters], 1) < S.max_waiters) *waiter = true;
      if (*waiter) slot = atomicAdd(&S.cnt[kHeadHi], 1);
    }
  }
  *done = 0;
  if (kIntra) {
    fin = __shfl_sync(0xffffffffu, fin, 0);
    if (fin >= 0) {
      const int nw = (gridDim.x * blockDim.x) >> 5;
#pragma unroll 1
      for (int i = lane; i <= nw; i += 32) st_release((int*)&S.ring[fin + i], (int)kExit);
    }
    head = __shfl_sync(0xffffffffu, head, 0);
    if (head >= 0) return S.heads[head];
  }
  slot = __shfl_sync(0xffffffffu, slot, 0);
  lo = __shfl_sync(0xffffffffu, lo, 0);
  if (slot >= 0) {
    nheads0 = __shfl_sync(0xffffffffu, nheads0, 0);
    if (slot < nheads0) return S.heads0[slot];
    uint32_t v;
    while ((v = (uint32_t)ld_acquire((const int*)&S.ring[slot - nheads0])) == kNoItem) __nanosleep(500);
    return v == kExit ? kNoItem : v;
  }
  if (lo >= 0) {
    const int n2 = S.cnt[S.n_items_at + 2], n1 = S.cnt[S.n_items_at + 1];
    return lo < n2 ? S.items[2][lo] : lo < n2 + n1 ? S.items[1][lo - n2] : S.items[0][lo - n2 - n1];
  }
  return kNoItem;
}

__device__ __forceinline__ void intra_band_ref(const Stage& S, int blk, int band, int coef_off, int lane) {
  const daala_b200_pvq_params& prm = S.prm;
  const int start = band_start(band);
  const int bn = band_start(band + 1) - start;
  const int r = band % 3;
  int top = -1, left = -1;
  if (band == 0 || r == 1) top = S.dep_top[blk];
  if (band == 0 || r == 2) left = S.dep_left[blk];
  if (band == 3 || band == 6) top = left = -1;
  const int32_t* ot = top >= 0 ? prm.out + prm.blocks[top].coef_off : nullptr;
  const int32_t* ol = left >= 0 ? prm.out + prm.blocks[left].coef_off : nullptr;
  bool low_from_top = false;
  if (band == 0) {
    double g1 = 0, g2 = 0;
    if (ot) { double a = __ldcg(ot + 2), bb = __ldcg(ot + 5), c = __ldcg(ot + 9); g1 += a * a; g1 += bb * bb; g1 += c * c; }
    if (ol) { double a = __ldcg(ol + 1), bb = __ldcg(ol + 4), c = __ldcg(ol + 7); g2 += a * a; g2 += bb * bb; g2 += c * c; }
    low_from_top = g1 > g2;
  }
  int32_t* vref = prm.ref + coef_off;
  for (int i = start + lane; i < start + bn; i += 32) {
    int r2, c2;
    scan_rc(i, &r2, &c2);
    int32_t p = 0;
    if (r2 == 0 && c2 > 0 && ot && (c2 >= 4 || low_from_top)) p = __ldcg(ot + i);
    if (c2 == 0 && r2 > 0 && ol && (r2 >= 4 || !low_from_top)) p = __ldcg(ol + i);
    vref[i] = p;
  }
}

template <bool kIntra>
__device__ __forceinline__ void run_item(const Stage& S, uint32_t item, int lane, int16_t* snap) {
  const daala_b200_pvq_params& prm = S.prm;
  const int blk = (int)(item >> 4), band = (int)(item & 15);
  const daala_b200_pvq_block b = prm.blocks[blk];
  const int bs = b.bs, pli = b.pli;
  const int start = band_start(band);
  const int bn = band_start(band + 1) - start;
  const size_t off = (size_t)b.coef_off + start;
  if (kIntra) intra_band_ref(S, blk, band, b.coef_off, lane);
  int qidx = bs * (bs + 1) + (band + 1) - (band + 1) / 3;
  int q = (prm.q0 * prm.pvq_qm_q4[pli][qidx]) >> 4;
  if (q < 1) q = 1;
  const int beta = (prm.use_masking && pli == 0 && bs > 0) ? kBeta15 : kBeta1;
  const int qoff = (b.xdec & 1 ? prm.qm_stride : 0) + ((((1 << (2 * bs)) - 1) << 4) / 3) + start;
  int itheta, max_theta, k;
  double skip_term;
  const bool pre = kIntra && S.pre_ev && band != 3 && band != 6;
  const int32_t* pev = pre ? S.pre_ev + (off >> 3) * kPreEvWords : nullptr;
  const int16_t* psn = pre ? S.pre_snap + 2 * off : nullptr;
  const int gain = quantise_band_warp<0>(lane, snap, S.rsqrt_tbl, prm.out + off, prm.in + off, prm.ref + off, bn, q,
                                         prm.y + off, &itheta, &max_theta, &k, beta, &skip_term, prm.is_keyframe, pli,
                                         prm.qm + qoff, prm.qm_inv + qoff, prm.pvq_norm_lambda, pev, psn);
  if (lane == 0) {
    const size_t r = (size_t)blk * 9 + band;
    prm.res_skip_term[r] = skip_term;
    short4 pk;
    pk.x = (short)gain; pk.y = (short)itheta; pk.z = (short)max_theta; pk.w = (short)k;
    reinterpret_cast<short4*>(S.res_pack)[r] = pk;
  }
}

struct ItemGeom {
  int blk, band, bn, q, beta, pli, qoff;
  size_t off;
};
__device__ __forceinline__ int band_q(const daala_b200_pvq_params& prm, const daala_b200_kf_frame_quant* fq, int frame,
                                      int pli, int qidx) {
  return fq ? (fq[frame].q0 * fq[frame].pvq_qm_q4[pli][qidx]) >> 4 : (prm.q0 * prm.pvq_qm_q4[pli][qidx]) >> 4;
}
__device__ __forceinline__ ItemGeom item_geom(const daala_b200_pvq_params& prm, uint32_t item,
                                              const daala_b200_kf_frame_quant* fq) {
  ItemGeom g;
  g.blk = (int)(item >> 4);
  g.band = (int)(item & 15);
  const daala_b200_pvq_block b = prm.blocks[g.blk];
  const int bs = b.bs;
  g.pli = b.pli;
  const int start = band_start(g.band);
  g.bn = band_start(g.band + 1) - start;
  g.off = (size_t)b.coef_off + start;
  const int qidx = bs * (bs + 1) + (g.band + 1) - (g.band + 1) / 3;
  int q = band_q(prm, fq, b.frame, g.pli, qidx);
  g.q = q < 1 ? 1 : q;
  g.beta = (prm.use_masking && g.pli == 0 && bs > 0) ? kBeta15 : kBeta1;
  g.qoff = (b.xdec & 1 ? prm.qm_stride : 0) + ((((1 << (2 * bs)) - 1) << 4) / 3) + start;
  return g;
}

template <int kPhase, bool kZeroRef, int kMode, bool kFq = false>
__global__ void __launch_bounds__(128) k_pvq_split(const __grid_constant__ Stage S, int cls, int chunk) {
  const daala_b200_pvq_params& prm = S.prm;
  const int lane = threadIdx.x & 31;
  const int slots = S.sp_slots[cls];
  const int first = chunk * slots;
  const int count = min(S.cnt[S.n_items_at + cls] - first, slots);
  const int vs = cls == 2 ? 128 : 32;
  const int nwarps = (gridDim.x * blockDim.x) >> 5;
  for (int i = (blockIdx.x * blockDim.x + threadIdx.x) >> 5; i < count; i += nwarps) {
    const ItemGeom g = item_geom(prm, S.items[cls][first + i], kFq ? S.fq : nullptr);
    int16_t* vec = S.sp_vec[cls] + (size_t)i * 3 * vs;
    int32_t* lanes = S.sp_lanes[cls] + (size_t)i * kCtxLaneWords * 16;
    int32_t* uni = S.sp_uni[cls] + (size_t)i * kCtxUniWords;
    int16_t* snap = S.sp_snap[cls] + (size_t)i * kMaxEvents * vs;
    const int32_t* r0 = kZeroRef ? nullptr : prm.ref + g.off;
    BandCtx B;
    if (kPhase == 0) {
      band_setup<kMode>(lane, B, prm.in + g.off, r0, g.bn, g.q, g.beta, prm.is_keyframe, g.pli, prm.qm + g.qoff,
                 prm.pvq_norm_lambda, S.rsqrt_tbl);
      band_ctx_store_setup(lane, B, g.bn, vec, vs, lanes, uni);
    } else if (kPhase == 1) {
      band_ctx_load_search(lane, B, g.bn, vec, vs, lanes);
      band_search<kMode>(lane, B, g.bn, snap, vs, S.rsqrt_tbl);
      band_ctx_store_search(lane, B, lanes);
    } else {
      band_ctx_load_finish(lane, B, g.bn, vec, vs, lanes, uni);
      int itheta, max_theta, k;
      double skip_term;
      const int gain = band_finish<kMode>(lane, B, snap, vs, prm.out + g.off, r0, g.bn, g.q, prm.y + g.off, &itheta, &max_theta, &k,
                                   g.beta, &skip_term, prm.is_keyframe, g.pli, prm.qm_inv + g.qoff, prm.pvq_norm_lambda);
      if (lane == 0) {
        const size_t r = (size_t)g.blk * 9 + g.band;
        prm.res_skip_term[r] = skip_term;
        short4 pk;
        pk.x = (short)gain; pk.y = (short)itheta; pk.z = (short)max_theta; pk.w = (short)k;
        reinterpret_cast<short4*>(S.res_pack)[r] = pk;
      }
    }
  }
}

template <int kMode>
__global__ void __launch_bounds__(128) k_pvq_prepass(const __grid_constant__ Stage S) {
  const daala_b200_pvq_params& prm = S.prm;
  __shared__ int16_t snap_all[4][2 * kMaxN];
  const int lane = threadIdx.x & 31;
  int16_t* snap = snap_all[threadIdx.x >> 5];
  const int nblk = min(S.cnt[S.n_blocks_at], S.max_blocks);
  const int nwarps = (gridDim.x * blockDim.x) >> 5;
  const int per = kMode == 2 ? 2 : 5;
  for (long long i = (blockIdx.x * blockDim.x + threadIdx.x) >> 5; i < (long long)nblk * per; i += nwarps) {
    const int blk = (int)(i / per), sel = (int)(i % per);
    const int band = kMode == 2 ? 7 + sel : (sel < 3 ? sel : sel + 1);
    if (band >= num_bands(prm.blocks[blk].bs)) continue;
    const ItemGeom g = item_geom(prm, ((uint32_t)blk << 4) | band, nullptr);
    BandCtx B;
    band_setup<kMode>(lane, B, prm.in + g.off, nullptr, g.bn, g.q, g.beta, prm.is_keyframe, g.pli, prm.qm + g.qoff,
                      prm.pvq_norm_lambda, S.rsqrt_tbl);
    band_search<kMode>(lane, B, g.bn, snap, kMaxN, S.rsqrt_tbl);
    band_noref_export(lane, B, g.bn, snap, kMaxN, S.pre_ev + (g.off >> 3) * kPreEvWords, S.pre_snap + 2 * g.off);
  }
}

__device__ __forceinline__ void grid_barrier(int32_t* bar, int* target, int nctas) {
  __syncthreads();
  if (threadIdx.x == 0) {
    *target += nctas;
    __threadfence();
    atomicAdd(bar, 1);
    while (ld_acquire(bar) < *target) {}
  }
  __syncthreads();
}

__global__ void __launch_bounds__(128, 4) k_pvq_levels(const __grid_constant__ Stage S) {
  const daala_b200_pvq_params& prm = S.prm;
  __shared__ int bar_target;
  if (threadIdx.x == 0) bar_target = 0;
  const int lane = threadIdx.x & 31;
  const int w = (blockIdx.x * blockDim.x + threadIdx.x) >> 5;
  const int nwarps = (gridDim.x * blockDim.x) >> 5;
  const int total = S.cnt[kTotalHi];
  constexpr int vs = 128;
  for (int lvl = 0; lvl < S.nlevels; lvl++) {
    const int base = S.lvl_off[lvl * 3];
    const int end = lvl + 1 < kMaxLevels ? S.lvl_off[(lvl + 1) * 3] : total;
    if (end - base > S.lvl_slots && threadIdx.x == 0 && blockIdx.x == 0) S.cnt[kError] = 2;
    const int n = min(end - base, S.lvl_slots);
    if (n <= 0) continue;
    for (int phase = 0; phase < 3; phase++) {
      for (int i = w; i < n; i += nwarps) {
        const uint32_t item = S.lvl_items[base + i];
        const ItemGeom g = item_geom(prm, item, nullptr);
        int16_t* vec = S.lv_vec + (size_t)i * 3 * vs;
        int32_t* lanes = S.lv_lanes + (size_t)i * kCtxLaneWords * 16;
        int32_t* uni = S.lv_uni + (size_t)i * kCtxUniWords;
        int16_t* snap = S.lv_snap + (size_t)i * kMaxEvents * vs;
        BandCtx B;
        if (phase == 0) {
          intra_band_ref(S, g.blk, g.band, (int)(g.off - band_start(g.band)), lane);
          band_setup<0>(lane, B, prm.in + g.off, prm.ref + g.off, g.bn, g.q, g.beta, prm.is_keyframe, g.pli,
                        prm.qm + g.qoff, prm.pvq_norm_lambda, S.rsqrt_tbl);
          band_ctx_store_setup(lane, B, g.bn, vec, vs, lanes, uni);
        } else if (phase == 1) {
          band_ctx_load_search(lane, B, g.bn, vec, vs, lanes);
          band_search<0>(lane, B, g.bn, snap, vs, S.rsqrt_tbl);
          band_ctx_store_search(lane, B, lanes);
        } else {
          band_ctx_load_finish(lane, B, g.bn, vec, vs, lanes, uni);
          int itheta, max_theta, k;
          double skip_term;
          const int gain = band_finish<0>(lane, B, snap, vs, prm.out + g.off, prm.ref + g.off, g.bn, g.q, prm.y + g.off,
                                          &itheta, &max_theta, &k, g.beta, &skip_term, prm.is_keyframe, g.pli,
                                          prm.qm_inv + g.qoff, prm.pvq_norm_lambda);
          if (lane == 0) {
            const size_t r = (size_t)g.blk * 9 + g.band;
            prm.res_skip_term[r] = skip_term;
            short4 pk;
            pk.x = (short)gain; pk.y = (short)itheta; pk.z = (short)max_theta; pk.w = (short)k;
            reinterpret_cast<short4*>(S.res_pack)[r] = pk;
          }
        }
      }
      grid_barrier(S.lv_bar, &bar_target, gridDim.x);
    }
  }
}

template <bool kIntra>
__global__ void __launch_bounds__(kPersistThreads, kPersistCtas) k_pvq_persist(const __grid_constant__ Stage S) {
  __shared__ __align__(16) int16_t snap_all[kPersistThreads / 32][kSnapEntries];
  const int lane = threadIdx.x & 31;
  int16_t* snap = snap_all[threadIdx.x >> 5];
  int done = 0;
  bool waiter = false;
  for (;;) {
    uint32_t item = next_item<kIntra>(S, lane, &done, &waiter);
    if (item == kNoItem) return;
#ifdef DAALA_B200_CHAIN_TRACE
    int kind = (item & 15) == 0 ? 0 : (item & 15) == 3 || (item & 15) == 6 ? 2 : 1;
#endif
    for (;;) {
      const int band = (int)(item & 15);
#ifdef DAALA_B200_CHAIN_TRACE
      const unsigned long long t0 = globaltimer();
#endif
      run_item<kIntra>(S, item, lane, snap);
#ifdef DAALA_B200_CHAIN_TRACE
      if (kIntra) trace_item(S, item, kind, t0, lane);
      kind = 3;
#endif
      if (!kIntra || band == 3 || band == 6) break;
      done += band == 0;
      __threadfence();
      __syncwarp();
      uint32_t next = kNoItem;
      if (lane == 0) {
        const int blk = (int)(item >> 4);
        if (band == 0) {
          const int nb[2] = {S.succ_bottom[blk], S.succ_right[blk]};
          for (int i = 0; i < 2; i++) {
            if (nb[i] < 0) continue;
            const int need = (S.dep_top[nb[i]] >= 0) + (S.dep_left[nb[i]] >= 0);
            if (need == 2 && atomicAdd(&S.join0[nb[i]], 1) != 1) continue;
            if (next == kNoItem) {
              next = (uint32_t)nb[i] << 4;
            } else {
              __threadfence();
              push_chain(S, nb[i], 0);
            }
          }
        } else {
          const int nb = band % 3 == 1 ? S.succ_bottom[blk] : S.succ_right[blk];
          if (nb >= 0) next = ((uint32_t)nb << 4) | band;
        }
      }
      next = __shfl_sync(0xffffffffu, next, 0);
      if (next == kNoItem) break;
      __threadfence();
      item = next;
    }
  }
}

__global__ void k_fill_rsqrt(double* tbl) {
  const int i = blockIdx.x * blockDim.x + threadIdx.x;
  if (i < kTableDoubles) pvq_fill_rsqrt_table(tbl, i);
}

__global__ void k_begin_pvq(int32_t* cnt, int luma) {
  if (threadIdx.x == 0 && blockIdx.x == 0) {
    if (luma) {
      cnt[kHeadLoL] = 0;
      cnt[kHeadHi] = 0;
      cnt[kTailHi] = cnt[kNHeads0];
      cnt[kDoneHi] = 0;
      cnt[kHeadCh] = 0;
      cnt[kWaiters] = 0;
#ifdef DAALA_B200_CHAIN_TRACE
      cnt[kTraceN] = 0;
#endif
    } else {
      cnt[kHeadLoC] = 0;
    }
  }
}

template <bool kInter>
__global__ void __launch_bounds__(256) k_finish_scatter(const __grid_constant__ Stage S) {
  const daala_b200_pvq_params& prm = S.prm;
  const int n = min(S.cnt[S.n_blocks_at], S.max_blocks);
  const int lane = threadIdx.x & 31;
  const int nwarps = (gridDim.x * blockDim.x) >> 5;
  for (int blk = (blockIdx.x * blockDim.x + threadIdx.x) >> 5; blk < n; blk += nwarps) {
    const daala_b200_pvq_block b = prm.blocks[blk];
    const int ln = b.bs + 2, nn = 1 << ln;
    const int len = ln >= 5 ? 512 : 1 << (2 * ln);
    const int stride = prm.plane_stride[b.pli];
    int32_t* dst = prm.coef_plane[b.pli] + b.frame * prm.plane_frame_pitch[b.pli] + (size_t)b.y0 * stride + b.x0;
    const int32_t* src = prm.out + b.coef_off;
    if (lane == 0) {
      const int nb = num_bands(b.bs);
      double sd = 0;
      for (int i = 0; i < nb; i++) sd += prm.res_skip_term[(size_t)blk * 9 + i];
      prm.res_skip_diff[blk] = sd;
      if (!kInter) {
        prm.out[b.coef_off] = prm.in[b.coef_off];
      } else {
        int dc_quant = band_q(prm, S.fq, b.frame, b.pli, b.bs * (b.bs + 1));
        if (dc_quant < 1) dc_quant = 1;
        const int32_t r = prm.ref[b.coef_off], diff = prm.in[b.coef_off] - r;
        int qdc = 0;
        if (abs(diff) >= dc_quant * 141 / 256) {
          const int half = ((dc_quant + 1) >> 1) - 1;
          qdc = (diff + (diff < 0 ? -half : half)) / dc_quant;
        }
        prm.out[b.coef_off] = dst[0] = qdc * dc_quant + r;
        prm.res_dc[blk] = qdc;
        if (S.dc_resid) S.dc_resid[blk] = diff;
      }
    }
    if (ln >= 5) {
      const int32_t* mdp = kInter ? prm.pred_plane[b.pli] + b.frame * prm.plane_frame_pitch[b.pli] + (size_t)b.y0 * stride + b.x0
                                  : nullptr;
      for (int i = lane; i < nn * nn; i += 32) {
        const size_t at = (size_t)(i >> ln) * stride + (i & (nn - 1));
        if (i) dst[at] = kInter ? mdp[at] : 0;
      }
      __syncwarp();
    }
    for (int i = lane + 1; i < len; i += 32) dst[scan_to_raster(i, ln, stride)] = src[i];
    const int32_t* y = prm.y + b.coef_off;
    for (int i = lane; i < len; i += 32) prm.y16[b.coef_off + i] = i ? (int16_t)y[i] : (int16_t)0;
  }
}

__global__ void k_dering_thresholds(const uint8_t* __restrict__ level, int32_t* __restrict__ thr_luma,
                                    int32_t* __restrict__ thr_chroma, int n, int4 tl_lo, int2 tl_hi, int4 tc_lo, int2 tc_hi,
                                    const uint8_t* __restrict__ coded, uint8_t* __restrict__ applied,
                                    const int32_t* __restrict__ frame_tbl, int nsb) {
  const int i = blockIdx.x * blockDim.x + threadIdx.x;
  if (i >= n) return;
  const int tl[6] = {tl_lo.x, tl_lo.y, tl_lo.z, tl_lo.w, tl_hi.x, tl_hi.y};
  const int tc[6] = {tc_lo.x, tc_lo.y, tc_lo.z, tc_lo.w, tc_hi.x, tc_hi.y};
  int g = level[i] < 6 ? level[i] : 5;
  if (coded) {
    if (!coded[i]) g = 0;
    applied[i] = (uint8_t)g;
  }
  if (frame_tbl) {
    const int32_t* t = frame_tbl + (size_t)(i / nsb) * 12;
    thr_luma[i] = t[g];
    thr_chroma[i] = t[6 + g];
  } else {
    thr_luma[i] = tl[g];
    thr_chroma[i] = tc[g];
  }
}

struct Fin {
  const daala_b200_pvq_block* blocks[2];
  const uint8_t* skip[2];
  const int32_t* dc[2];
  const int32_t* cnt;
  int max_blocks[2];
  const int32_t* d[3];
  const int32_t* md[3];
  int32_t* out[3];
  long long plane_pitch[3];
  int plane_stride[3];
  uint8_t* bskip[3];
  long long skip_pitch[3];
  int skip_stride;
  uint8_t* coded;
  int nhsb, nvsb;
  int q0;
  uint8_t pvq_qm_q4[3][32];
  const daala_b200_kf_frame_quant* fq;
};

__device__ __forceinline__ bool fin_block(const Fin& P, int i, int* list, int* blk) {
  const int nl = min(P.cnt[kNLuma], P.max_blocks[0]), nc = min(P.cnt[kNChroma], P.max_blocks[1]);
  if (i >= nl + nc) return false;
  *list = i >= nl;
  *blk = i >= nl ? i - nl : i;
  return true;
}

__global__ void __launch_bounds__(256) k_fin_patch(const __grid_constant__ Fin P) {
  const int lane = threadIdx.x & 31;
  const int nwarps = (gridDim.x * blockDim.x) >> 5;
  int list, blk;
  for (int i = (blockIdx.x * blockDim.x + threadIdx.x) >> 5; fin_block(P, i, &list, &blk); i += nwarps) {
    const daala_b200_pvq_block b = P.blocks[list][blk];
    const int ln = b.bs + 2, nn = 1 << ln;
    const int stride = P.plane_stride[b.pli];
    const size_t o = b.frame * P.plane_pitch[b.pli] + (size_t)b.y0 * stride + b.x0;
    const int32_t* src = (P.skip[list][blk] ? P.md[b.pli] : P.d[b.pli]) + o;
    const int32_t* mdp = P.md[b.pli] + o;
    int32_t* dst = P.out[b.pli] + o;
    const int qidx = b.bs * (b.bs + 1);
    int dc_quant = P.fq ? (P.fq[b.frame].q0 * P.fq[b.frame].pvq_qm_q4[b.pli][qidx]) >> 4 : (P.q0 * P.pvq_qm_q4[b.pli][qidx]) >> 4;
    if (dc_quant < 1) dc_quant = 1;
    const int32_t dc0 = mdp[0] + P.dc[list][blk] * dc_quant;
    for (int k = lane; k < nn * nn; k += 32) {
      const size_t at = (size_t)(k >> ln) * stride + (k & (nn - 1));
      dst[at] = k ? src[at] : dc0;
    }
  }
}

__global__ void __launch_bounds__(256) k_fin_skip_map(const __grid_constant__ Fin P) {
  const int lane = threadIdx.x & 31;
  const int nwarps = (gridDim.x * blockDim.x) >> 5;
  int list, blk;
  for (int i = (blockIdx.x * blockDim.x + threadIdx.x) >> 5; fin_block(P, i, &list, &blk); i += nwarps) {
    const daala_b200_pvq_block b = P.blocks[list][blk];
    const uint8_t s = P.skip[list][blk] && P.dc[list][blk] == 0;
    const int nu = 1 << b.bs;
    uint8_t* m = P.bskip[b.pli] + b.frame * P.skip_pitch[b.pli] + (size_t)(b.y0 >> 2) * P.skip_stride + (b.x0 >> 2);
    for (int k = lane; k < nu * nu; k += 32) m[(size_t)(k >> b.bs) * P.skip_stride + (k & (nu - 1))] = s;
    if (lane == 0 && b.pli == 0 && !s) P.coded[((size_t)b.frame * P.nvsb + (b.y0 >> 6)) * P.nhsb + (b.x0 >> 6)] = 1;
  }
}

struct PoolStore {
  const uint8_t* src[3];
  uint8_t* pool[3];
  long long plane_bytes[3];
  const int32_t* slot;
};

__global__ void __launch_bounds__(256) k_fin_pool_store(const __grid_constant__ PoolStore S) {
  const int f = blockIdx.y / 3, p = blockIdx.y - 3 * f;
  const int slot = S.slot[f];
  if (slot < 0) return;
  const long long n = S.plane_bytes[p] >> 4;
  const uint4* __restrict__ src = reinterpret_cast<const uint4*>(S.src[p] + f * S.plane_bytes[p]);
  uint4* __restrict__ dst = reinterpret_cast<uint4*>(S.pool[p] + slot * S.plane_bytes[p]);
  for (long long i = (long long)blockIdx.x * blockDim.x + threadIdx.x; i < n; i += (long long)gridDim.x * blockDim.x)
    dst[i] = src[i];
}

struct Sym {
  const uint8_t* bsize;
  int bstride;
  long long bsize_pitch;
  int F, nhsb, sb_rows, u_row0;
  int nsb;
  uint32_t* unit_rank;
  uint32_t* sb_cnt;
  int32_t* sb_base;
  uint32_t* order;
  longlong2* off;
  longlong2* tile;
  long long* tot;
  int ntiles, cap_blocks;
  long long cap_bands, cap_bytes;
  daala_b200_kf_sym_frame* index;
  daala_b200_kf_sym_block* blocks;
  short4* bands;
  uint8_t* pulses;
  const daala_b200_pvq_block* list[2];
  const short4* res[2];
  const int32_t* y[2];
  const double* skip_diff[2];
  const int32_t* flip;
  const int32_t* cnt;
  int max_luma, max_chroma;
  daala_b200_kf_sym_dc* dc;
  const int32_t* qdc[2];
  const int32_t* dc_resid[2];
  daala_b200_kf_late_skip* late_skip;
  const daala_b200_kf_late_skip* ls_block[2];
};

__device__ __forceinline__ int sym_band_bytes(int band, short4 r) {
  if (r.w <= 0) return 0;
  const int n = band_start(band + 1) - band_start(band) - (r.y != -1);
  return r.w > 127 ? 2 * n : n;
}

__global__ void __launch_bounds__(256) k_sym_rank(const __grid_constant__ Sym S) {
  const int lane = threadIdx.x & 31;
  const int sb = (blockIdx.x * blockDim.x + threadIdx.x) >> 5;
  if (sb >= S.F * S.nsb) return;
  const int f = sb / S.nsb, r = sb % S.nsb;
  const int sby = r / S.nhsb, sbx = r % S.nhsb;
  const int uw = S.nhsb * 8;
  uint32_t v[2];
  long long at[2];
  for (int h = 0; h < 2; h++) {
    const int m = 2 * lane + h;
    const int dx = (m & 1) | ((m >> 1) & 2) | ((m >> 2) & 4);
    const int dy = ((m >> 1) & 1) | ((m >> 2) & 2) | ((m >> 3) & 4);
    const int ux = sbx * 8 + dx, uy = S.u_row0 + sby * 8 + dy;
    const int b = S.bsize[f * S.bsize_pitch + (long long)uy * S.bstride + ux];
    const int4 c = unit_counts(b, ux, uy);
    v[h] = (uint32_t)c.x | ((uint32_t)c.z << 16);
    at[h] = ((long long)f * S.sb_rows * 8 + (uy - S.u_row0)) * uw + ux;
  }
  const uint32_t s = v[0] + v[1];
  uint32_t inc = s;
#pragma unroll
  for (int o = 1; o < 32; o <<= 1) {
    const uint32_t a = __shfl_up_sync(0xffffffffu, inc, o);
    if (lane >= o) inc += a;
  }
  S.unit_rank[at[0]] = inc - s;
  S.unit_rank[at[1]] = inc - s + v[0];
  if (lane == 31) S.sb_cnt[sb] = inc;
}

__global__ void __launch_bounds__(1024) k_sym_sb_scan(const __grid_constant__ Sym S) {
  __shared__ int part[1024];
  __shared__ int carry;
  const int t = threadIdx.x;
  const int n = S.F * S.nsb;
  if (t == 0) carry = 0;
  __syncthreads();
  for (int base = 0; base < n; base += 1024) {
    const int i = base + t;
    const uint32_t c = i < n ? S.sb_cnt[i] : 0u;
    const int v = (int)(c & 0xffff) + 2 * (int)(c >> 16);
    part[t] = v;
    __syncthreads();
    for (int o = 1; o < 1024; o <<= 1) {
      const int a = t >= o ? part[t - o] : 0;
      __syncthreads();
      part[t] += a;
      __syncthreads();
    }
    const int incl = part[t], c0 = carry;
    if (i < n) S.sb_base[i] = c0 + incl - v;
    __syncthreads();
    if (t == 1023) carry = c0 + incl;
    __syncthreads();
  }
  if (t == 0) S.tot[0] = min(carry, S.cap_blocks);
}

__global__ void __launch_bounds__(256) k_sym_place(const __grid_constant__ Sym S) {
  const int nl = min(S.cnt[kNLuma], S.max_luma), nc = min(S.cnt[kNChroma], S.max_chroma);
  const int uw = S.nhsb * 8;
  for (int i = blockIdx.x * blockDim.x + threadIdx.x; i < nl + nc; i += gridDim.x * blockDim.x) {
    const int ch = i >= nl;
    const int blk = ch ? i - nl : i;
    const daala_b200_pvq_block b = S.list[ch][blk];
    const int sh = ch ? 2 : 3;
    const int ux = b.x0 >> sh, uy = b.y0 >> sh;
    const int sb = b.frame * S.nsb + ((uy - S.u_row0) >> 3) * S.nhsb + (ux >> 3);
    const uint32_t rk = S.unit_rank[((long long)b.frame * S.sb_rows * 8 + (uy - S.u_row0)) * uw + ux];
    const uint32_t sc = S.sb_cnt[sb];
    int pos = S.sb_base[sb];
    if (!ch) pos += (int)(rk & 0xffff) + (b.bs == 0 ? ((b.y0 >> 2) & 1) * 2 + ((b.x0 >> 2) & 1) : 0);
    else pos += (int)(sc & 0xffff) + (b.pli - 1) * (int)(sc >> 16) + (int)(rk >> 16);
    if (pos >= S.cap_blocks) continue;
    S.order[pos] = (uint32_t)blk | (ch ? 0x80000000u : 0u);
    const short4* r = S.res[ch] + (size_t)blk * 9;
    const int nb = num_bands(b.bs);
    long long bytes = 0;
    for (int j = 0; j < nb; j++) bytes += sym_band_bytes(j, r[j]);
    S.off[pos] = make_longlong2(nb, bytes);
  }
}

__device__ __forceinline__ longlong2 add2(longlong2 a, longlong2 b) { return make_longlong2(a.x + b.x, a.y + b.y); }

__global__ void __launch_bounds__(kTile) k_sym_tile_sums(const __grid_constant__ Sym S) {
  __shared__ longlong2 part[32];
  const long long i = (long long)blockIdx.x * kTile + threadIdx.x;
  longlong2 v = i < S.tot[0] ? S.off[i] : make_longlong2(0, 0);
#pragma unroll
  for (int o = 16; o > 0; o >>= 1) {
    v.x += __shfl_xor_sync(0xffffffffu, v.x, o);
    v.y += __shfl_xor_sync(0xffffffffu, v.y, o);
  }
  if ((threadIdx.x & 31) == 0) part[threadIdx.x >> 5] = v;
  __syncthreads();
  if (threadIdx.x == 0) {
    longlong2 s = make_longlong2(0, 0);
    for (int w = 0; w < kTile / 32; w++) s = add2(s, part[w]);
    S.tile[blockIdx.x] = s;
  }
}

__global__ void __launch_bounds__(1024) k_sym_tile_scan(const __grid_constant__ Sym S) {
  __shared__ longlong2 part[1024];
  __shared__ longlong2 carry;
  const int t = threadIdx.x;
  if (t == 0) carry = make_longlong2(0, 0);
  __syncthreads();
  for (int base = 0; base < S.ntiles; base += 1024) {
    const int i = base + t;
    const longlong2 v = i < S.ntiles ? S.tile[i] : make_longlong2(0, 0);
    part[t] = v;
    __syncthreads();
    for (int o = 1; o < 1024; o <<= 1) {
      const longlong2 a = t >= o ? part[t - o] : make_longlong2(0, 0);
      __syncthreads();
      part[t] = add2(part[t], a);
      __syncthreads();
    }
    const longlong2 incl = part[t], c = carry;
    if (i < S.ntiles) S.tile[i] = make_longlong2(c.x + incl.x - v.x, c.y + incl.y - v.y);
    __syncthreads();
    if (t == 1023) carry = add2(c, incl);
    __syncthreads();
  }
  if (t == 0) {
    S.tot[1] = carry.x;
    S.tot[2] = carry.y;
  }
}

__global__ void __launch_bounds__(kTile) k_sym_offsets(const __grid_constant__ Sym S) {
  __shared__ longlong2 wsum[32];
  const long long i = (long long)blockIdx.x * kTile + threadIdx.x;
  const int lane = threadIdx.x & 31, warp = threadIdx.x >> 5;
  const bool valid = i < S.tot[0];
  const longlong2 v = valid ? S.off[i] : make_longlong2(0, 0);
  longlong2 s = v;
#pragma unroll
  for (int o = 1; o < 32; o <<= 1) {
    const long long ax = __shfl_up_sync(0xffffffffu, s.x, o), ay = __shfl_up_sync(0xffffffffu, s.y, o);
    if (lane >= o) s = make_longlong2(s.x + ax, s.y + ay);
  }
  if (lane == 31) wsum[warp] = s;
  __syncthreads();
  longlong2 pre = S.tile[blockIdx.x];
  for (int w = 0; w < warp; w++) pre = add2(pre, wsum[w]);
  if (valid) S.off[i] = make_longlong2(pre.x + s.x - v.x, pre.y + s.y - v.y);
}

template <bool kInter>
__global__ void __launch_bounds__(256) k_sym_pack(const __grid_constant__ Sym S) {
  const int lane = threadIdx.x & 31;
  const long long n = S.tot[0];
  const int nwarps = (gridDim.x * blockDim.x) >> 5;
  for (long long slot = (blockIdx.x * blockDim.x + threadIdx.x) >> 5; slot < n; slot += nwarps) {
    const uint32_t id = S.order[slot];
    const int ch = id >> 31, blk = (int)(id & 0x7fffffffu);
    const daala_b200_pvq_block b = S.list[ch][blk];
    const long long first = S.sb_base[b.frame * S.nsb];
    const longlong2 o = S.off[slot], o0 = first < n ? S.off[first] : o;
    const short4* r = S.res[ch] + (size_t)blk * 9;
    const int nb = num_bands(b.bs);
    int bytes = 0;
    for (int j = 0; j < nb; j++) bytes += sym_band_bytes(j, r[j]);
    if (o.x + nb > S.cap_bands || o.y + bytes > S.cap_bytes) continue;
    if (lane == 0) {
      daala_b200_kf_sym_block rec;
      rec.skip_diff = S.skip_diff[ch][blk];
      rec.pulse_off = (uint32_t)(o.y - o0.y);
      rec.band_off = (uint32_t)(o.x - o0.x);
      rec.x0 = b.x0;
      rec.y0 = b.y0;
      rec.bs = b.bs;
      rec.pli = b.pli;
      rec.flip = !kInter && ch ? (uint8_t)S.flip[blk] : 0;
      rec.reserved = 0;
      S.blocks[slot] = rec;
      if (kInter) {
        daala_b200_kf_sym_dc d;
        d.qdc = S.qdc[ch][blk];
        d.dc_resid = S.dc_resid[ch][blk];
        S.dc[slot] = d;
        if (S.late_skip) S.late_skip[slot] = S.ls_block[ch][blk];
      }
    }
    if (lane < nb) S.bands[o.x + lane] = r[lane];
    const int32_t* y = S.y[ch] + b.coef_off;
    uint8_t* dst = S.pulses + o.y;
    for (int j = 0; j < nb; j++) {
      const short4 q = r[j];
      const int len = sym_band_bytes(j, q);
      if (!len) continue;
      const int st = band_start(j);
      if (q.w > 127) {
        for (int t = lane; t < len / 2; t += 32) {
          const int v = y[st + t];
          dst[2 * t] = (uint8_t)(v & 0xff);
          dst[2 * t + 1] = (uint8_t)((v >> 8) & 0xff);
        }
      } else {
        for (int t = lane; t < len; t += 32) dst[t] = (uint8_t)(y[st + t] & 0xff);
      }
      dst += len;
    }
  }
}

__global__ void k_sym_index(const __grid_constant__ Sym S) {
  for (int f = threadIdx.x; f < S.F; f += blockDim.x) {
    const long long n = S.tot[0];
    const long long s0 = S.sb_base[f * S.nsb];
    const long long s1 = f + 1 < S.F ? S.sb_base[(f + 1) * S.nsb] : n;
    const longlong2 a = s0 < n ? S.off[s0] : make_longlong2(S.tot[1], S.tot[2]);
    const longlong2 e = s1 < n ? S.off[s1] : make_longlong2(S.tot[1], S.tot[2]);
    daala_b200_kf_sym_frame x;
    x.first_block = s0;
    x.n_blocks = s1 - s0;
    x.first_band = a.x;
    x.n_bands = e.x - a.x;
    x.first_byte = a.y;
    x.n_bytes = e.y - a.y;
    S.index[f] = x;
  }
}

constexpr int kSymSegs = 6;
struct SymCopy {
  const uint8_t* src[kSymSegs];
  uint8_t* dst[kSymSegs];
  long long unit[kSymSegs];
  long long cap[kSymSegs];
  long long index_bytes;
  const long long* tot;
};

__global__ void __launch_bounds__(256) k_sym_copy(const __grid_constant__ SymCopy C) {
  const long long tid = (long long)blockIdx.x * blockDim.x + threadIdx.x;
  const long long nth = (long long)gridDim.x * blockDim.x;
  for (int seg = 0; seg < kSymSegs; seg++) {
    if (!C.dst[seg]) continue;
    const long long want = seg == 0 ? C.index_bytes : C.tot[seg >= 4 ? 0 : seg - 1] * C.unit[seg];
    const long long len = want < C.cap[seg] ? want : C.cap[seg];
    const uint8_t* s = C.src[seg];
    uint8_t* d = C.dst[seg];
    long long done = 0;
    if ((((uintptr_t)s | (uintptr_t)d) & 15) == 0) {
      const long long n16 = len >> 4;
      for (long long i = tid; i < n16; i += nth)
        reinterpret_cast<uint4*>(d)[i] = reinterpret_cast<const uint4*>(s)[i];
      done = n16 << 4;
    }
    for (long long i = done + tid; i < len; i += nth) d[i] = s[i];
  }
}

struct Unstream {
  const uint32_t* order;
  const long long* tot;
  const uint8_t* skip;
  const int32_t* dc;
  uint8_t* fin_skip[2];
  int32_t* fin_dc[2];
  const int32_t* form;
};

__global__ void __launch_bounds__(256) k_fin_unstream(const __grid_constant__ Unstream U) {
  if (!*U.form) return;
  const long long n = U.tot[0];
  for (long long slot = (long long)blockIdx.x * blockDim.x + threadIdx.x; slot < n;
       slot += (long long)gridDim.x * blockDim.x) {
    const uint32_t id = U.order[slot];
    const int ch = id >> 31, blk = (int)(id & 0x7fffffffu);
    U.fin_skip[ch][blk] = U.skip[slot];
    U.fin_dc[ch][blk] = U.dc[slot];
  }
}

}
}

using namespace daala_b200::kf;

extern "C" int daala_b200_launch_forward(const daala_b200_frame* prm, int nplanes, cudaStream_t stream);
extern "C" int daala_b200_launch_inverse(const daala_b200_frame* prm, int nplanes, cudaStream_t stream);
extern "C" int daala_b200_launch_inverse_lapped_only(const daala_b200_frame* prm, int nplanes, cudaStream_t stream);
extern "C" int daala_b200_launch_sb_postfilter_store(const daala_b200_frame* prm, int nplanes, cudaStream_t stream);

struct Dering {
  daala_b200_frame frame;
  const uint8_t* skip[3];
  long long skip_pitch[3];
  int skip_stride;
  uint8_t* level;
  const uint8_t* coded;
  uint8_t* applied;
  int tbl[2][6];
  const int32_t* frame_tbl;
  int32_t* thr[2];
  int32_t* dir;
  bool search;
  daala_b200_dering_search_batch sb;
};

struct daala_b200_kf {
  daala_b200_kf_config cfg;
  int nhsb, nvsb, F;
  int plane_w[3], plane_h[3];
  cudaStream_t stream;
  bool own_stream;
  cudaGraph_t graph;
  cudaGraphExec_t exec;
  bool captured;
  uint8_t* pixels[3];
  int32_t* coeffs[3];
  int32_t* lapped[3];
  uint8_t* pixels_out[3];
  uint8_t* pred_pixels[3];
  int32_t* pred_coeffs[3];
  uint8_t* bsize;
  int32_t* cfl_plane;
  int16_t *qm, *qm_inv;
  double* rsqrt_tbl;
  int16_t* sp_vec[3];
  int32_t* sp_lanes[3];
  int32_t* sp_uni[3];
  int16_t* sp_snap[3];
  int sp_slots[3];
  int16_t* lv_vec;
  int32_t* lv_lanes;
  int32_t* lv_uni;
  int16_t* lv_snap;
  int32_t* lv_bar;
  int lvl_slots, lvl_grid;
  Dering dering;
  Lists lists;
  Stage luma, chroma;
  Sym sym;
  daala_b200_frame frame;
  daala_b200_frame frame_pred;
  uint8_t* ref_pixels[3];
  int32_t* ref_slot;
  daala_b200_mv_pt* mv_grid;
  int32_t* ref_slot_next;
  int32_t* mv1_grid;
  uint32_t* mc_leaves;
  int32_t* mc_nleaves;
  daala_b200_mc_batch mc;
  uint8_t* fin_skip[2];
  int32_t* fin_dc[2];
  int32_t* dc_resid[2];
  int32_t* fin_coeffs[3];
  uint8_t* fin_pixels[3];
  uint8_t* fin_bskip[3];
  uint8_t *fin_level, *fin_coded;
  Fin fin;
  cudaGraph_t fin_graph;
  cudaGraphExec_t fin_exec;
  bool fin_captured;
  int fin_dc_limit;
  daala_b200_kf_frame_quant* fq;
  int32_t* fq_tbl;
  std::vector<int32_t> fq_tbl_host;
  int32_t* fin_slot_out;
  PoolStore store;
  uint8_t* fin_stream_skip;
  int32_t* fin_stream_dc;
  int32_t* fin_form;
  Unstream unstream;
  int32_t* d_orig[3];
  daala_b200_kf_late_skip* late_skip[2];
  daala_b200_late_skip_batch lsb;
  std::vector<uint8_t> slot_filled;
  bool have_step;
  daala_b200_kf_totals last_tot;
  std::vector<void*> allocs;
  size_t bytes_allocated;
  size_t chain_cap;
  int sms;
  char err[256];
};

#define KF_CHECK(x)                                                                       \
  do {                                                                                    \
    cudaError_t e_ = (x);                                                                 \
    if (e_ != cudaSuccess) {                                                              \
      snprintf(kf->err, sizeof(kf->err), "%s: %s", #x, cudaGetErrorString(e_));           \
      return (int)e_;                                                                     \
    }                                                                                     \
  } while (0)

template <class T>
static cudaError_t dalloc(daala_b200_kf* kf, T** p, size_t n) {
  const size_t bytes = (n ? n : 1) * sizeof(T);
  cudaError_t e = cudaMalloc((void**)p, bytes);
  if (e == cudaSuccess) {
    kf->allocs.push_back(*p);
    kf->bytes_allocated += bytes;
    e = cudaMemset(*p, 0, bytes);
  }
  return e;
}

static int kf_alloc(daala_b200_kf* kf) {
  const int F = kf->F;
  const bool inter = kf->cfg.inter != 0;
  const long long luma_px = (long long)kf->plane_w[0] * kf->plane_h[0];
  for (int p = 0; p < 3; p++) {
    const size_t n = (size_t)kf->plane_w[p] * kf->plane_h[p] * F;
    KF_CHECK(dalloc(kf, &kf->pixels[p], n));
    KF_CHECK(dalloc(kf, &kf->coeffs[p], n));
    KF_CHECK(dalloc(kf, &kf->lapped[p], n));
    KF_CHECK(dalloc(kf, &kf->pixels_out[p], n));
    if (inter) {
      KF_CHECK(dalloc(kf, &kf->pred_pixels[p], n));
      KF_CHECK(dalloc(kf, &kf->pred_coeffs[p], n));
    }
  }
  const int UW = kf->nhsb * 8, UH = kf->nvsb * 8;
  KF_CHECK(dalloc(kf, &kf->bsize, (size_t)F * UW * UH));
  if (!inter) KF_CHECK(dalloc(kf, &kf->cfl_plane, (size_t)kf->plane_w[1] * kf->plane_h[1] * F));
  if (kf->cfg.inter_mc) {
    daala_b200_mc_batch& B = kf->mc;
    const size_t nsb = (size_t)kf->nhsb * kf->nvsb;
    for (int p = 0; p < 3; p++) {
      KF_CHECK(dalloc(kf, &kf->ref_pixels[p], (size_t)kf->plane_w[p] * kf->plane_h[p] * kf->cfg.mc_refs));
      B.ref[p] = kf->ref_pixels[p];
      B.pred[p] = kf->pred_pixels[p];
      B.plane_w[p] = kf->plane_w[p];
      B.plane_h[p] = kf->plane_h[p];
    }
    KF_CHECK(dalloc(kf, &kf->ref_slot, (size_t)2 * F));
    KF_CHECK(dalloc(kf, &kf->mv_grid, (size_t)F * (kf->nvsb * 8 + 1) * (kf->nhsb * 8 + 1)));
    KF_CHECK(dalloc(kf, &kf->mc_leaves, (size_t)F * nsb * 64));
    KF_CHECK(dalloc(kf, &kf->mc_nleaves, (size_t)F * nsb));
    B.grid = kf->mv_grid;
    B.ref_slot = kf->ref_slot;
    B.leaves = kf->mc_leaves;
    B.nleaves = kf->mc_nleaves;
    B.F = F;
    B.nhsb = kf->nhsb;
    B.nvsb = kf->nvsb;
    B.nslots = kf->cfg.mc_refs;
    if (kf->cfg.mc_next) {
      KF_CHECK(dalloc(kf, &kf->ref_slot_next, (size_t)F));
      KF_CHECK(dalloc(kf, &kf->mv1_grid, (size_t)F * (kf->nvsb * 8 + 1) * (kf->nhsb * 8 + 1) * 2));
      B.ref_slot_next = kf->ref_slot_next;
      B.mv1 = kf->mv1_grid;
    }
  }
  if (kf->cfg.frame_quant) {
    KF_CHECK(dalloc(kf, &kf->fq, (size_t)F));
    KF_CHECK(dalloc(kf, &kf->fq_tbl, (size_t)F * 12));
    kf->fq_tbl_host.assign((size_t)F * 12, 0);
  }
  KF_CHECK(dalloc(kf, &kf->qm, (size_t)2 * kf->cfg.qm_stride));
  KF_CHECK(dalloc(kf, &kf->qm_inv, (size_t)2 * kf->cfg.qm_stride));
  KF_CHECK(dalloc(kf, &kf->rsqrt_tbl, (size_t)kTableDoubles));
  KF_CHECK(cudaMemcpy(kf->qm, kf->cfg.qm, sizeof(int16_t) * 2 * kf->cfg.qm_stride, cudaMemcpyHostToDevice));
  KF_CHECK(cudaMemcpy(kf->qm_inv, kf->cfg.qm_inv, sizeof(int16_t) * 2 * kf->cfg.qm_stride, cudaMemcpyHostToDevice));

  Lists& L = kf->lists;
  memset(&L, 0, sizeof(L));
  L.bsize = kf->bsize;
  L.bstride = UW;
  L.bsize_pitch = (long long)UW * UH;
  L.F = F;
  L.UW = UW;
  L.UH = UH;
  L.u_row0 = kf->cfg.sb_row0 * 8;
  L.u_rows = kf->cfg.sb_rows * 8;
  const long long nunits = (long long)F * L.u_rows * UW;
  L.ntiles = (int)((nunits + kTile - 1) / kTile);
  const int div = kf->cfg.max_blocks_div > 0 ? kf->cfg.max_blocks_div : 1;
  L.max_luma = (int)(nunits * 4 / div) + 64;
  L.max_chroma = (int)(nunits * 2 / div) + 64;
  KF_CHECK(dalloc(kf, &L.tile_sum, (size_t)L.ntiles));
  KF_CHECK(dalloc(kf, &L.unit_lbase, (size_t)F * UW * UH));
  KF_CHECK(dalloc(kf, &L.luma, (size_t)L.max_luma));
  KF_CHECK(dalloc(kf, &L.chroma, (size_t)L.max_chroma));
  const size_t ndep = inter ? 0 : (size_t)L.max_luma;
  KF_CHECK(dalloc(kf, &L.dep_top, ndep));
  KF_CHECK(dalloc(kf, &L.dep_left, ndep));
  KF_CHECK(dalloc(kf, &L.succ_bottom, ndep));
  KF_CHECK(dalloc(kf, &L.succ_right, ndep));
  const size_t luma_shard_px = (size_t)F * L.u_rows * UW * 64;
  kf->chain_cap = luma_shard_px / 16 + 64 + (size_t)kf->sms * 64;
  const size_t cap_l0 = (size_t)L.max_luma * 3 < luma_shard_px / 16 ? (size_t)L.max_luma * 3 : luma_shard_px / 16;
  const size_t cap_l[3] = {inter ? cap_l0 + 64 : 64, luma_shard_px / 64 + 64, luma_shard_px / 256 + 64};
  const size_t cap_c[3] = {(size_t)L.max_chroma * 3 / 2 + 64, luma_shard_px / 4 * 2 * 3 / 64 + 64,
                           luma_shard_px / 4 * 2 * 3 / 256 + 64};
  for (int c = 0; c < 3; c++) {
    KF_CHECK(dalloc(kf, &L.items_l[c], cap_l[c]));
    KF_CHECK(dalloc(kf, &L.items_c[c], cap_c[c]));
  }
  if (kf->cfg.split_free > 0 || inter) {
    const int slots[3] = {1 << 19, 1 << 19, 3 << 15};
    for (int c = 0; c < 3; c++) {
      const int vs = c == 2 ? 128 : 32;
      kf->sp_slots[c] = slots[c];
      KF_CHECK(dalloc(kf, &kf->sp_vec[c], (size_t)slots[c] * 3 * vs));
      KF_CHECK(dalloc(kf, &kf->sp_lanes[c], (size_t)slots[c] * kCtxLaneWords * 16));
      KF_CHECK(dalloc(kf, &kf->sp_uni[c], (size_t)slots[c] * kCtxUniWords));
      KF_CHECK(dalloc(kf, &kf->sp_snap[c], (size_t)slots[c] * kMaxEvents * vs));
    }
  }
  if (kf->cfg.level_chains) {
    KF_CHECK(dalloc(kf, &L.lvl_hist, (size_t)kLevelBins));
    KF_CHECK(dalloc(kf, &L.lvl_cursor, (size_t)kLevelBins));
    KF_CHECK(dalloc(kf, &L.lvl_items, kf->chain_cap));
    L.nlevels = (kf->plane_w[0] + L.u_rows * 8) / 4 + 2;
    if (L.nlevels >= kMaxLevels) return (int)cudaErrorInvalidValue;
    kf->lvl_slots = 2048 * F;
    KF_CHECK(dalloc(kf, &kf->lv_vec, (size_t)kf->lvl_slots * 3 * 128));
    KF_CHECK(dalloc(kf, &kf->lv_lanes, (size_t)kf->lvl_slots * kCtxLaneWords * 16));
    KF_CHECK(dalloc(kf, &kf->lv_uni, (size_t)kf->lvl_slots * kCtxUniWords));
    KF_CHECK(dalloc(kf, &kf->lv_snap, (size_t)kf->lvl_slots * kMaxEvents * 128));
    KF_CHECK(dalloc(kf, &kf->lv_bar, (size_t)32));
    int per_sm = 0;
    KF_CHECK(cudaOccupancyMaxActiveBlocksPerMultiprocessor(&per_sm, k_pvq_levels, 128, 0));
    if (per_sm < 1) return (int)cudaErrorLaunchOutOfResources;
    kf->lvl_grid = per_sm * kf->sms;
  }
  {
    const int want = kf->cfg.persist_ctas_per_sm > 0 ? kf->cfg.persist_ctas_per_sm : kPersistCtas;
    int per_sm[2] = {0, 0};
    KF_CHECK(cudaFuncSetAttribute(k_pvq_persist<true>, cudaFuncAttributePreferredSharedMemoryCarveout,
                                  cudaSharedmemCarveoutMaxShared));
    KF_CHECK(cudaFuncSetAttribute(k_pvq_persist<false>, cudaFuncAttributePreferredSharedMemoryCarveout,
                                  cudaSharedmemCarveoutMaxShared));
    KF_CHECK(cudaOccupancyMaxActiveBlocksPerMultiprocessor(&per_sm[0], k_pvq_persist<true>, kPersistThreads, 0));
    KF_CHECK(cudaOccupancyMaxActiveBlocksPerMultiprocessor(&per_sm[1], k_pvq_persist<false>, kPersistThreads, 0));
    if (per_sm[0] < want || per_sm[1] < want) {
      snprintf(kf->err, sizeof(kf->err), "k_pvq_persist: %d / %d CTAs per SM resident, %d wanted", per_sm[0],
               per_sm[1], want);
      return (int)cudaErrorLaunchOutOfResources;
    }
  }
  KF_CHECK(dalloc(kf, &L.heads, inter ? 0 : kf->chain_cap));
  KF_CHECK(dalloc(kf, &L.heads_raw, inter ? 0 : kf->chain_cap));
  KF_CHECK(dalloc(kf, &L.head_bin, inter ? 0 : kf->chain_cap));
  KF_CHECK(dalloc(kf, &L.head_hist, inter ? 0 : (size_t)kLevelBins));
  KF_CHECK(dalloc(kf, &L.head_cursor, inter ? 0 : (size_t)kLevelBins));
  KF_CHECK(dalloc(kf, &L.heads0, ndep));
  KF_CHECK(dalloc(kf, &L.cnt, (size_t)kCntWords));
  kf->mc.bad_ref = L.cnt + kMcBadRef;
  kf->mc.beyond = L.cnt + kMcBeyond;

  auto setup_stage = [&](Stage& S, bool chroma) -> int {
    memset(&S, 0, sizeof(S));
    daala_b200_pvq_params& p = S.prm;
    const size_t ncoef = chroma ? luma_shard_px / 2 + 1024 : luma_shard_px + 1024;
    const size_t nblk = chroma ? L.max_chroma : L.max_luma;
    p.blocks = chroma ? L.chroma : L.luma;
    KF_CHECK(dalloc(kf, &p.in, ncoef));
    KF_CHECK(dalloc(kf, &p.ref, ncoef));
    KF_CHECK(dalloc(kf, &p.out, ncoef));
    KF_CHECK(dalloc(kf, &p.y, ncoef));
    KF_CHECK(dalloc(kf, &p.y16, ncoef));
    KF_CHECK(dalloc(kf, &p.res_skip_term, nblk * 9));
    KF_CHECK(dalloc(kf, &p.res_skip_diff, nblk));
    KF_CHECK(dalloc(kf, &p.res_flip, nblk));
    KF_CHECK(dalloc(kf, &S.res_pack, nblk * 9 * 4));
    p.res_gain = p.res_theta = p.res_max_theta = p.res_k = nullptr;
    p.res_dc = nullptr;
    if (inter) KF_CHECK(dalloc(kf, &p.res_dc, nblk));
    p.qm = kf->qm;
    p.qm_inv = kf->qm_inv;
    for (int i = 0; i < 3; i++) {
      p.coef_plane[i] = kf->coeffs[i];
      p.pred_plane[i] = kf->pred_coeffs[i];
      p.plane_frame_pitch[i] = (long long)kf->plane_w[i] * kf->plane_h[i];
      p.plane_stride[i] = kf->plane_w[i];
    }
    p.qm_stride = kf->cfg.qm_stride;
    p.q0 = kf->cfg.q0 > 1 ? kf->cfg.q0 : 1;
    p.is_keyframe = inter ? 0 : 1;
    p.use_masking = kf->cfg.use_masking;
    p.pvq_norm_lambda = kf->cfg.pvq_norm_lambda;
    memcpy(p.pvq_qm_q4, kf->cfg.pvq_qm_q4, sizeof(p.pvq_qm_q4));
    S.fq = kf->fq;
    for (int c = 0; c < 3; c++) S.items[c] = chroma ? L.items_c[c] : L.items_l[c];
    S.cnt = L.cnt;
    S.rsqrt_tbl = kf->rsqrt_tbl;
    for (int c = 0; c < 3; c++) {
      S.sp_vec[c] = kf->sp_vec[c];
      S.sp_lanes[c] = kf->sp_lanes[c];
      S.sp_uni[c] = kf->sp_uni[c];
      S.sp_snap[c] = kf->sp_snap[c];
      S.sp_slots[c] = kf->sp_slots[c];
      const size_t cap = chroma ? cap_c[c] : cap_l[c];
      S.sp_chunks[c] = kf->sp_slots[c] > 0 ? (int)((cap + kf->sp_slots[c] - 1) / kf->sp_slots[c]) : 0;
    }
    S.skip_lo = chroma ? 0 : kf->cfg.split_free > 1;
    S.max_waiters = getenv("DAALA_B200_MAX_WAITERS") ? atoi(getenv("DAALA_B200_MAX_WAITERS")) : kf->sms * 8;
    if (!chroma && kf->cfg.noref_prepass) {
      KF_CHECK(dalloc(kf, &S.pre_ev, (ncoef / 8 + 2) * kPreEvWords));
      KF_CHECK(dalloc(kf, &S.pre_snap, 2 * ncoef));
    }
    if (!chroma) {
      S.lvl_off = L.lvl_hist;
      S.lvl_items = L.lvl_items;
      S.nlevels = L.nlevels;
      S.lvl_slots = kf->lvl_slots;
      S.lv_vec = kf->lv_vec;
      S.lv_lanes = kf->lv_lanes;
      S.lv_uni = kf->lv_uni;
      S.lv_snap = kf->lv_snap;
      S.lv_bar = kf->lv_bar;
    }
    S.n_items_at = chroma ? kNItemsC : kNItemsL;
    S.head_lo_at = chroma ? kHeadLoC : kHeadLoL;
    S.n_blocks_at = chroma ? kNChroma : kNLuma;
    S.max_blocks = (int)nblk;
#ifdef DAALA_B200_CHAIN_TRACE
    if (!chroma && !inter) {
      S.trace_cap = (int)(luma_shard_px / 16);
      KF_CHECK(dalloc(kf, &S.trace, (size_t)S.trace_cap));
    }
#endif
    if (!chroma) {
      S.dep_top = L.dep_top;
      S.dep_left = L.dep_left;
      S.succ_bottom = L.succ_bottom;
      S.succ_right = L.succ_right;
      S.heads = L.heads;
      S.heads0 = L.heads0;
      KF_CHECK(dalloc(kf, &S.ring, inter ? 0 : kf->chain_cap));
      KF_CHECK(dalloc(kf, &S.join0, ndep));
    } else {
      S.cfl_plane = kf->cfl_plane;
      S.cfl_pitch = (long long)kf->plane_w[1] * kf->plane_h[1];
      S.cfl_stride = kf->plane_w[1];
    }
    return 0;
  };
  int rc = setup_stage(kf->luma, false);
  if (rc) return rc;
  rc = setup_stage(kf->chroma, true);
  if (rc) return rc;
  (void)luma_px;
  if (kf->cfg.inter_finish || kf->cfg.symbol_stream == 2)
    for (int c = 0; c < 2; c++) {
      Stage& S = c ? kf->chroma : kf->luma;
      KF_CHECK(dalloc(kf, &kf->dc_resid[c], (size_t)S.max_blocks));
      S.dc_resid = kf->dc_resid[c];
    }
  if (kf->cfg.symbol_stream) {
    Sym& Y = kf->sym;
    memset(&Y, 0, sizeof(Y));
    Y.bsize = kf->bsize;
    Y.bstride = UW;
    Y.bsize_pitch = (long long)UW * UH;
    Y.F = F;
    Y.nhsb = kf->nhsb;
    Y.sb_rows = kf->cfg.sb_rows;
    Y.u_row0 = L.u_row0;
    Y.nsb = kf->nhsb * kf->cfg.sb_rows;
    Y.cap_blocks = L.max_luma + L.max_chroma;
    Y.ntiles = (Y.cap_blocks + kTile - 1) / kTile;
    const size_t ncoef = (luma_shard_px + 1024) + (luma_shard_px / 2 + 1024);
    KF_CHECK(dalloc(kf, &Y.unit_rank, (size_t)F * L.u_rows * UW));
    KF_CHECK(dalloc(kf, &Y.sb_cnt, (size_t)F * Y.nsb));
    KF_CHECK(dalloc(kf, &Y.sb_base, (size_t)F * Y.nsb));
    KF_CHECK(dalloc(kf, &Y.order, (size_t)Y.cap_blocks));
    KF_CHECK(dalloc(kf, &Y.off, (size_t)Y.cap_blocks));
    KF_CHECK(dalloc(kf, &Y.tile, (size_t)Y.ntiles));
    KF_CHECK(dalloc(kf, &Y.tot, (size_t)4));
    KF_CHECK(dalloc(kf, &Y.index, (size_t)F));
    KF_CHECK(dalloc(kf, &Y.blocks, (size_t)Y.cap_blocks));
    Y.cap_bands = (long long)(ncoef / 16);
    Y.cap_bytes = (long long)(2 * ncoef);
    KF_CHECK(dalloc(kf, &Y.bands, ncoef / 16));
    KF_CHECK(dalloc(kf, &Y.pulses, 2 * ncoef));
    for (int c = 0; c < 2; c++) {
      const Stage& S = c ? kf->chroma : kf->luma;
      Y.list[c] = S.prm.blocks;
      Y.res[c] = reinterpret_cast<const short4*>(S.res_pack);
      Y.y[c] = S.prm.y;
      Y.skip_diff[c] = S.prm.res_skip_diff;
    }
    Y.flip = kf->chroma.prm.res_flip;
    Y.cnt = L.cnt;
    Y.max_luma = L.max_luma;
    Y.max_chroma = L.max_chroma;
    if (kf->cfg.symbol_stream == 2) {
      KF_CHECK(dalloc(kf, &Y.dc, (size_t)Y.cap_blocks));
      for (int c = 0; c < 2; c++) {
        Y.qdc[c] = (c ? kf->chroma : kf->luma).prm.res_dc;
        Y.dc_resid[c] = kf->dc_resid[c];
      }
    }
  }
  if (kf->cfg.late_skip) {
    daala_b200_late_skip_batch& B = kf->lsb;
    memset(&B, 0, sizeof(B));
    long long px = 0;
    for (int p = 0; p < 3; p++) {
      const size_t n = (size_t)kf->plane_w[p] * kf->plane_h[p] * F;
      KF_CHECK(dalloc(kf, &kf->d_orig[p], n));
      px += (long long)n;
      B.d_orig[p] = kf->d_orig[p];
      B.d[p] = kf->coeffs[p];
      B.md[p] = kf->pred_coeffs[p];
      B.plane_pitch[p] = (long long)kf->plane_w[p] * kf->plane_h[p];
      B.plane_stride[p] = kf->plane_w[p];
    }
    for (int c = 0; c < 2; c++) {
      const Stage& S = c ? kf->chroma : kf->luma;
      KF_CHECK(dalloc(kf, &kf->late_skip[c], (size_t)S.max_blocks));
      B.blocks[c] = S.prm.blocks;
      B.count[c] = L.cnt + S.n_blocks_at;
      B.max_blocks[c] = S.max_blocks;
      B.out[c] = kf->late_skip[c];
    }
    KF_CHECK(dalloc(kf, &B.cls_items, (size_t)daala_b200_late_skip_class_caps(px, B.cls_off, B.cls_cap)));
    KF_CHECK(dalloc(kf, &B.cls_n, (size_t)4));
    B.q0 = kf->luma.prm.q0;
    memcpy(B.pvq_qm_q4, kf->cfg.pvq_qm_q4, sizeof(B.pvq_qm_q4));
    B.qm_is_flat = kf->cfg.qm_is_flat;
    B.use_activity_masking = kf->cfg.use_masking;
    B.coded_quantizer = kf->cfg.coded_quantizer;
    B.fq = kf->fq;
    if (kf->cfg.symbol_stream == 2) {
      Sym& Y = kf->sym;
      KF_CHECK(dalloc(kf, &Y.late_skip, (size_t)Y.cap_blocks));
      Y.ls_block[0] = kf->late_skip[0];
      Y.ls_block[1] = kf->late_skip[1];
    }
  }

  daala_b200_frame& f = kf->frame;
  memset(&f, 0, sizeof(f));
  for (int p = 0; p < 3; p++) {
    daala_b200_plane& pl = f.plane[p];
    pl.pixels = kf->pixels[p];
    pl.coeffs = kf->coeffs[p];
    pl.lapped = kf->lapped[p];
    pl.pixels_out = kf->pixels_out[p];
    pl.pixel_stride = pl.coeff_stride = pl.lapped_stride = pl.pixel_out_stride = kf->plane_w[p];
    pl.xdec = p ? 1 : 0;
    pl.pixel_frame_pitch = pl.coeff_frame_pitch = pl.lapped_frame_pitch = pl.pixel_out_frame_pitch =
        (long long)kf->plane_w[p] * kf->plane_h[p];
  }
  f.bsize = kf->bsize;
  f.bstride = UW;
  f.bsize_frame_pitch = (long long)UW * UH;
  f.nhsb = kf->nhsb;
  f.nvsb = kf->nvsb;
  f.pic_w = kf->cfg.pic_w;
  f.pic_h = kf->cfg.pic_h;
  f.haar_dc = inter ? 0 : 1;
  f.nframes = F;
  f.sb_row0 = kf->cfg.sb_row0;
  f.sb_rows = kf->cfg.sb_rows;
  kf->frame_pred = f;
  for (int p = 0; p < 3; p++) {
    kf->frame_pred.plane[p].pixels = kf->pred_pixels[p];
    kf->frame_pred.plane[p].coeffs = kf->pred_coeffs[p];
  }
  if (kf->cfg.inter_finish) {
    const size_t nsb = (size_t)F * kf->nhsb * kf->nvsb;
    Fin& P = kf->fin;
    memset(&P, 0, sizeof(P));
    for (int c = 0; c < 2; c++) {
      const Stage& S = c ? kf->chroma : kf->luma;
      KF_CHECK(dalloc(kf, &kf->fin_skip[c], (size_t)S.max_blocks));
      KF_CHECK(dalloc(kf, &kf->fin_dc[c], (size_t)S.max_blocks));
      P.blocks[c] = S.prm.blocks;
      P.skip[c] = kf->fin_skip[c];
      P.dc[c] = kf->fin_dc[c];
      P.max_blocks[c] = S.max_blocks;
    }
    P.cnt = L.cnt;
    P.skip_stride = kf->nhsb * 16;
    for (int p = 0; p < 3; p++) {
      const size_t n = (size_t)kf->plane_w[p] * kf->plane_h[p] * F;
      KF_CHECK(dalloc(kf, &kf->fin_coeffs[p], n));
      KF_CHECK(dalloc(kf, &kf->fin_pixels[p], n));
      P.skip_pitch[p] = (long long)(kf->plane_h[p] / 4) * P.skip_stride;
      KF_CHECK(dalloc(kf, &kf->fin_bskip[p], (size_t)P.skip_pitch[p] * F));
      P.d[p] = kf->coeffs[p];
      P.md[p] = kf->pred_coeffs[p];
      P.out[p] = kf->fin_coeffs[p];
      P.plane_pitch[p] = (long long)kf->plane_w[p] * kf->plane_h[p];
      P.plane_stride[p] = kf->plane_w[p];
      P.bskip[p] = kf->fin_bskip[p];
    }
    KF_CHECK(dalloc(kf, &kf->fin_level, nsb));
    KF_CHECK(dalloc(kf, &kf->fin_coded, nsb));
    P.coded = kf->fin_coded;
    P.nhsb = kf->nhsb;
    P.nvsb = kf->nvsb;
    P.q0 = kf->luma.prm.q0;
    memcpy(P.pvq_qm_q4, kf->cfg.pvq_qm_q4, sizeof(P.pvq_qm_q4));
    int dq_max = 1;
    for (int p = 0; p < 3; p++)
      for (int bs = 0; bs < 5; bs++) {
        const int dq = (P.q0 * P.pvq_qm_q4[p][bs * (bs + 1)]) >> 4;
        if (dq > dq_max) dq_max = dq;
      }
    kf->fin_dc_limit = DAALA_B200_KF_FINISH_DC_LIMIT / dq_max;
    P.fq = kf->fq;
    if (kf->cfg.inter_mc) {
      KF_CHECK(dalloc(kf, &kf->fin_slot_out, (size_t)F));
      PoolStore& W = kf->store;
      for (int p = 0; p < 3; p++) {
        W.src[p] = kf->fin_pixels[p];
        W.pool[p] = kf->ref_pixels[p];
        W.plane_bytes[p] = (long long)kf->plane_w[p] * kf->plane_h[p];
      }
      W.slot = kf->fin_slot_out;
    }
    if (kf->cfg.symbol_stream == 2) {
      Unstream& U = kf->unstream;
      KF_CHECK(dalloc(kf, &kf->fin_stream_skip, (size_t)kf->sym.cap_blocks));
      KF_CHECK(dalloc(kf, &kf->fin_stream_dc, (size_t)kf->sym.cap_blocks));
      KF_CHECK(dalloc(kf, &kf->fin_form, (size_t)1));
      U.order = kf->sym.order;
      U.tot = kf->sym.tot;
      U.skip = kf->fin_stream_skip;
      U.dc = kf->fin_stream_dc;
      for (int c = 0; c < 2; c++) {
        U.fin_skip[c] = kf->fin_skip[c];
        U.fin_dc[c] = kf->fin_dc[c];
      }
      U.form = kf->fin_form;
    }
  }
  const int dering = kf->cfg.dering ? kf->cfg.dering : kf->cfg.inter_finish;
  if (dering) {
    const size_t nsb = (size_t)F * kf->nhsb * kf->nvsb;
    Dering& D = kf->dering;
    D.frame = kf->frame;
    D.skip_stride = kf->nhsb * 16;
    uint8_t* zero_skip = nullptr;
    if (!kf->cfg.inter_finish) KF_CHECK(dalloc(kf, &zero_skip, nsb * 256 + 64));
    for (int p = 0; p < 3; p++) {
      KF_CHECK(dalloc(kf, &D.frame.post16[p], (size_t)kf->plane_w[p] * kf->plane_h[p] * F));
      if (kf->cfg.inter_finish) {
        D.frame.plane[p].coeffs = D.frame.plane[p].lapped = kf->fin_coeffs[p];
        D.frame.plane[p].pixels_out = kf->fin_pixels[p];
        D.skip[p] = kf->fin_bskip[p];
        D.skip_pitch[p] = kf->fin.skip_pitch[p];
      } else {
        D.skip[p] = zero_skip;
      }
    }
    KF_CHECK(dalloc(kf, &D.level, nsb));
    KF_CHECK(dalloc(kf, &D.thr[0], nsb));
    KF_CHECK(dalloc(kf, &D.thr[1], nsb));
    KF_CHECK(dalloc(kf, &D.dir, nsb * 64));
    D.coded = kf->fin_coded;
    D.applied = kf->fin_level;
    daala_b200_dering_threshold_table(kf->cfg.q0, D.tbl);
    D.frame_tbl = kf->fq_tbl;
    D.search = dering == 2;
    if (D.search) {
      daala_b200_dering_search_batch& b = D.sb;
      b.etmp = D.frame.post16[0];
      b.src = kf->pixels[0];
      b.etmp_pitch = b.src_pitch = (long long)kf->plane_w[0] * kf->plane_h[0];
      b.etmp_stride = b.src_stride = kf->plane_w[0];
      b.nframes = F;
      b.nhsb = kf->nhsb;
      b.nvsb = kf->nvsb;
      memcpy(b.threshold, D.tbl[0], sizeof(b.threshold));
      b.coded_quantizer = kf->cfg.coded_quantizer;
      b.qm_is_flat = kf->cfg.qm_is_flat;
      b.use_activity_masking = kf->cfg.use_masking;
      b.dering_lambda = kf->cfg.dering_lambda;
      b.bskip = D.skip[0];
      b.skip_stride = D.skip_stride;
      b.skip_pitch = D.skip_pitch[0];
      b.coded = D.coded;
      b.is_keyframe = inter ? 0 : 1;
      KF_CHECK(dalloc(kf, &b.filt, (size_t)kf->plane_w[0] * kf->plane_h[0] * F));
      KF_CHECK(dalloc(kf, &b.orig, nsb * 4096));
      KF_CHECK(dalloc(kf, &b.cand, nsb * 4096));
      KF_CHECK(dalloc(kf, &b.dist, nsb * 6));
      b.dir = D.dir;
      b.levels = D.level;
      if (kf->cfg.frame_quant) {
        b.fq = kf->fq;
        b.frame_tbl = kf->fq_tbl;
        KF_CHECK(dalloc(kf, &b.cand_thr, nsb * 5));
      }
    }
  }
  KF_CHECK(cudaDeviceSynchronize());
  k_fill_rsqrt<<<(kTableDoubles + 255) / 256, 256, 0, kf->stream>>>(kf->rsqrt_tbl);
  KF_CHECK(cudaGetLastError());
  KF_CHECK(cudaStreamSynchronize(kf->stream));
  return 0;
}

static int enqueue_dering(daala_b200_kf* kf, const Dering& D, cudaStream_t s) {
  int rc = daala_b200_launch_inverse_lapped_only(&D.frame, 3, s);
  if (!rc) rc = daala_b200_launch_sb_postfilter_store(&D.frame, 3, s);
  if (!rc && D.search) rc = daala_b200_dering_search_enqueue(&D.sb, s);
  if (rc) return rc;
  const int nsb = kf->nhsb * kf->nvsb;
  k_dering_thresholds<<<(kf->F * nsb + 255) / 256, 256, 0, s>>>(
      D.level, D.thr[0], D.thr[1], kf->F * nsb, make_int4(D.tbl[0][0], D.tbl[0][1], D.tbl[0][2], D.tbl[0][3]),
      make_int2(D.tbl[0][4], D.tbl[0][5]), make_int4(D.tbl[1][0], D.tbl[1][1], D.tbl[1][2], D.tbl[1][3]),
      make_int2(D.tbl[1][4], D.tbl[1][5]), D.coded, D.applied, D.frame_tbl, nsb);
  for (int p = 0; p < 3; p++) {
    const long long per = (long long)kf->plane_w[p] * kf->plane_h[p];
    daala_b200_dering_params dp;
    memset(&dp, 0, sizeof(dp));
    dp.y = nullptr;
    dp.x = D.frame.post16[p];
    dp.dir = D.dir;
    dp.bskip = D.skip[p];
    dp.sb_threshold = D.thr[p ? 1 : 0];
    dp.ystride = dp.xstride = kf->plane_w[p];
    dp.dir_stride = kf->nhsb * 8;
    dp.skip_stride = D.skip_stride;
    dp.nhsb = kf->nhsb;
    dp.nvsb = kf->nvsb;
    dp.xdec = p ? 1 : 0;
    dp.pli = p;
    dp.overlap = 1;
    dp.coeff_shift = 4;
    dp.dir_format = D.search ? 2 : 0;
    rc = daala_b200_dering_plane_frames(&dp, kf->F, per, per, (long long)nsb * 64, nsb, D.skip_pitch[p],
                                        D.frame.plane[p].pixels_out, s);
    if (rc) return rc;
  }
  return 0;
}

static int dering_launches(const Dering& D) { return 1 + 1 + (D.search ? 5 + 6 + 6 + 1 : 0) + 1 + 3; }

template <bool kZeroRef, bool kFq = false>
static void enqueue_split(daala_b200_kf* kf, const Stage& S, cudaStream_t s) {
  const int grid = kf->sms * 16;
  for (int cls = 2; cls >= 0; cls--) {
    for (int chunk = 0; chunk < S.sp_chunks[cls]; chunk++) {
      if (cls == 2) {
        k_pvq_split<0, kZeroRef, 2, kFq><<<grid, 128, 0, s>>>(S, cls, chunk);
        k_pvq_split<1, kZeroRef, 2><<<grid, 128, 0, s>>>(S, cls, chunk);
        k_pvq_split<2, kZeroRef, 2, kFq><<<grid, 128, 0, s>>>(S, cls, chunk);
      } else {
        k_pvq_split<0, kZeroRef, 1, kFq><<<grid, 128, 0, s>>>(S, cls, chunk);
        k_pvq_split<1, kZeroRef, 1><<<grid, 128, 0, s>>>(S, cls, chunk);
        k_pvq_split<2, kZeroRef, 1, kFq><<<grid, 128, 0, s>>>(S, cls, chunk);
      }
    }
  }
}

template <bool kInter>
static void enqueue_sym(const Sym& Y, int wide, cudaStream_t s) {
  k_sym_rank<<<(Y.F * Y.nsb + 7) / 8, 256, 0, s>>>(Y);
  k_sym_sb_scan<<<1, 1024, 0, s>>>(Y);
  k_sym_place<<<wide, 256, 0, s>>>(Y);
  k_sym_tile_sums<<<Y.ntiles, kTile, 0, s>>>(Y);
  k_sym_tile_scan<<<1, 1024, 0, s>>>(Y);
  k_sym_offsets<<<Y.ntiles, kTile, 0, s>>>(Y);
  k_sym_pack<kInter><<<wide, 256, 0, s>>>(Y);
  k_sym_index<<<1, 256, 0, s>>>(Y);
}

static int kf_enqueue_step_inter(daala_b200_kf* kf, int phases) {
  cudaStream_t s = kf->stream;
  const Lists& L = kf->lists;
  const int wide = kf->sms * 8;
  if (phases & DAALA_B200_KF_LISTS) {
    k_unit_tile_sums<<<L.ntiles, kTile, 0, s>>>(L);
    k_tile_scan<<<1, 1024, 0, s>>>(L);
    k_unit_emit<<<L.ntiles, kTile, 0, s>>>(L);
    k_luma_items<<<wide, 256, 0, s>>>(L);
    k_chroma_items<<<wide, 256, 0, s>>>(L);
    if (kf->cfg.inter_mc) {
      if (cudaMemsetAsync(L.cnt + kMcBadRef, 0, 2 * sizeof(int32_t), s) != cudaSuccess) return (int)cudaGetLastError();
      int rc = daala_b200_launch_mc_leaves(&kf->mc, wide, s);
      if (rc) return rc;
    }
  }
  if (phases & DAALA_B200_KF_FORWARD) {
    int rc = kf->cfg.inter_mc ? daala_b200_launch_mc_obmc(&kf->mc, wide, s) : 0;
    if (!rc) rc = daala_b200_launch_forward(&kf->frame, 3, s);
    if (rc) return rc;
    for (int p = 0; kf->cfg.late_skip && p < 3; p++)
      if (cudaMemcpyAsync(kf->d_orig[p], kf->coeffs[p], sizeof(int32_t) * kf->plane_w[p] * kf->plane_h[p] * kf->F,
                          cudaMemcpyDeviceToDevice, s) != cudaSuccess)
        return (int)cudaGetLastError();
    rc = daala_b200_launch_forward(&kf->frame_pred, 3, s);
    if (rc) return rc;
  }
  const bool core = (phases & DAALA_B200_KF_SEARCH_ONLY) != 0;
  for (const Stage* S : {&kf->luma, &kf->chroma}) {
    if (!(phases & (S == &kf->luma ? DAALA_B200_KF_PVQ_LUMA : DAALA_B200_KF_PVQ_CHROMA))) continue;
    if (!core) k_gather<kGatherInter><<<wide, 256, 0, s>>>(*S);
    if (S->fq) enqueue_split<false, true>(kf, *S, s);
    else enqueue_split<false>(kf, *S, s);
    if (!core) k_finish_scatter<true><<<wide, 256, 0, s>>>(*S);
  }
  if (!core && (phases & DAALA_B200_KF_PVQ_CHROMA) && kf->cfg.late_skip) {
    const int rc = daala_b200_late_skip_enqueue(&kf->lsb, kf->sms * 3, s);
    if (rc) return rc;
  }
  if (!core && (phases & DAALA_B200_KF_PVQ_CHROMA) && kf->cfg.symbol_stream) enqueue_sym<true>(kf->sym, wide, s);
  if (phases & DAALA_B200_KF_INVERSE) {
    int rc = daala_b200_launch_inverse(&kf->frame, 3, s);
    if (rc) return rc;
  }
  return (int)cudaGetLastError();
}

static int kf_enqueue_step(daala_b200_kf* kf, int phases) {
  if (kf->cfg.inter) return kf_enqueue_step_inter(kf, phases);
  cudaStream_t s = kf->stream;
  const Lists& L = kf->lists;
  const int wide = kf->sms * 8;
  if (phases & DAALA_B200_KF_LISTS) {
    k_unit_tile_sums<<<L.ntiles, kTile, 0, s>>>(L);
    k_tile_scan<<<1, 1024, 0, s>>>(L);
    k_unit_emit<<<L.ntiles, kTile, 0, s>>>(L);
    const size_t nl = (size_t)L.max_luma * sizeof(int32_t);
    if (cudaMemsetAsync(L.succ_bottom, 0xff, nl, s) != cudaSuccess || cudaMemsetAsync(L.succ_right, 0xff, nl, s) != cudaSuccess)
      return (int)cudaGetLastError();
    if (L.lvl_hist && cudaMemsetAsync(L.lvl_hist, 0, sizeof(int32_t) * kLevelBins, s) != cudaSuccess) return (int)cudaGetLastError();
    if (cudaMemsetAsync(L.head_hist, 0, sizeof(int32_t) * kLevelBins, s) != cudaSuccess) return (int)cudaGetLastError();
    k_luma_deps<<<wide, 256, 0, s>>>(L);
    if (L.lvl_hist) {
      k_level_scan<<<1, 1024, 0, s>>>(L);
      k_level_scatter<<<wide, 256, 0, s>>>(L);
    }
    k_chroma_items<<<wide, 256, 0, s>>>(L);
  }
  if (phases & DAALA_B200_KF_FORWARD) {
    int rc = daala_b200_launch_forward(&kf->frame, 3, s);
    if (rc) return rc;
  }
  const int persist = kf->sms * (kf->cfg.persist_ctas_per_sm > 0 ? kf->cfg.persist_ctas_per_sm : kPersistCtas);
  const bool core = (phases & DAALA_B200_KF_SEARCH_ONLY) != 0;
  if (phases & DAALA_B200_KF_PVQ_LUMA) {
    if (cudaMemsetAsync(kf->luma.ring, 0xff, kf->chain_cap * sizeof(uint32_t), s) != cudaSuccess ||
        cudaMemsetAsync(kf->luma.join0, 0, (size_t)kf->luma.max_blocks * sizeof(int32_t), s) != cudaSuccess)
      return (int)cudaGetLastError();
    k_begin_pvq<<<1, 32, 0, s>>>(kf->lists.cnt, 1);
    if (!core) k_gather<kGatherLuma><<<wide, 256, 0, s>>>(kf->luma);
    if (kf->cfg.split_free > 1) enqueue_split<true>(kf, kf->luma, s);
    if (kf->luma.pre_ev) {
      k_pvq_prepass<2><<<kf->sms * 16, 128, 0, s>>>(kf->luma);
      k_pvq_prepass<1><<<kf->sms * 16, 128, 0, s>>>(kf->luma);
    }
    if (kf->cfg.level_chains) {
      if (cudaMemsetAsync(kf->lv_bar, 0, sizeof(int32_t) * 32, s) != cudaSuccess) return (int)cudaGetLastError();
      k_pvq_levels<<<kf->lvl_grid, 128, 0, s>>>(kf->luma);
    } else {
      k_pvq_persist<true><<<persist, kPersistThreads, 0, s>>>(kf->luma);
    }
    if (!core) k_finish_scatter<false><<<wide, 256, 0, s>>>(kf->luma);
  }
  if (phases & DAALA_B200_KF_PVQ_CHROMA) {
    k_begin_pvq<<<1, 32, 0, s>>>(kf->lists.cnt, 0);
    if (!core) k_cfl_plane<<<wide, 256, 0, s>>>(kf->chroma, kf->cfl_plane);
    if (!core) k_gather<kGatherChroma><<<wide, 256, 0, s>>>(kf->chroma);
    if (kf->cfg.split_free > 0) enqueue_split<false>(kf, kf->chroma, s);
    else k_pvq_persist<false><<<persist, kPersistThreads, 0, s>>>(kf->chroma);
    if (!core) k_finish_scatter<false><<<wide, 256, 0, s>>>(kf->chroma);
    if (!core && kf->cfg.symbol_stream) enqueue_sym<false>(kf->sym, wide, s);
  }
  if (phases & DAALA_B200_KF_INVERSE) {
    int rc = kf->cfg.dering ? enqueue_dering(kf, kf->dering, s) : daala_b200_launch_inverse(&kf->frame, 3, s);
    if (rc) return rc;
  }
  return (int)cudaGetLastError();
}

static int kf_enqueue_finish(daala_b200_kf* kf) {
  cudaStream_t s = kf->stream;
  const int wide = kf->sms * 8;
  if (kf->fin_form) k_fin_unstream<<<wide, 256, 0, s>>>(kf->unstream);
  if (cudaMemsetAsync(kf->fin_coded, 0, (size_t)kf->F * kf->nhsb * kf->nvsb, s) != cudaSuccess)
    return (int)cudaGetLastError();
  k_fin_patch<<<wide, 256, 0, s>>>(kf->fin);
  k_fin_skip_map<<<wide, 256, 0, s>>>(kf->fin);
  const int rc = enqueue_dering(kf, kf->dering, s);
  if (rc) return rc;
  if (kf->fin_slot_out) k_fin_pool_store<<<dim3(wide > kf->F ? wide / kf->F : 1, 3 * kf->F), 256, 0, s>>>(kf->store);
  return (int)cudaGetLastError();
}

extern "C" {

static thread_local char g_create_err[256] = "null engine";

daala_b200_kf* daala_b200_kf_create(const daala_b200_kf_config* cfg) {
  snprintf(g_create_err, sizeof(g_create_err), "daala_b200_kf_create: invalid configuration");
  if (cfg && cfg->inter_mc && (cfg->inter_mc != 1 || cfg->inter != 1)) {
    snprintf(g_create_err, sizeof(g_create_err), "daala_b200_kf_create: inter_mc is 0 or 1, and 1 requires inter = 1");
    return nullptr;
  }
  if (cfg && cfg->mc_next && (cfg->mc_next != 1 || cfg->inter_mc != 1)) {
    snprintf(g_create_err, sizeof(g_create_err), "daala_b200_kf_create: mc_next is 0 or 1, and 1 requires inter_mc = 1");
    return nullptr;
  }
  if (cfg && cfg->inter_finish && (cfg->inter_finish < 0 || cfg->inter_finish > 2 || cfg->inter != 1)) {
    snprintf(g_create_err, sizeof(g_create_err),
             "daala_b200_kf_create: inter_finish is 0, 1 or 2, and 1 and 2 require inter = 1");
    return nullptr;
  }
  if (cfg && (cfg->symbol_stream < 0 || cfg->symbol_stream > 2 || (cfg->symbol_stream == 2 && cfg->inter != 1))) {
    snprintf(g_create_err, sizeof(g_create_err),
             "daala_b200_kf_create: symbol_stream is 0, 1 or 2, and 2 requires inter = 1 (a keyframe's DC goes through "
             "the Haar pyramid and has no scalar index)");
    return nullptr;
  }
  if (cfg && cfg->late_skip && (cfg->late_skip != 1 || cfg->inter != 1)) {
    snprintf(g_create_err, sizeof(g_create_err),
             "daala_b200_kf_create: late_skip is 0 or 1, and 1 requires inter = 1 (keyframes have no late skip)");
    return nullptr;
  }
  if (cfg && cfg->frame_quant && (cfg->frame_quant != 1 || cfg->inter != 1)) {
    snprintf(g_create_err, sizeof(g_create_err),
             "daala_b200_kf_create: frame_quant is 0 or 1, and 1 requires inter = 1 (a keyframe batch shares one quantizer)");
    return nullptr;
  }
  if (cfg && cfg->mc_refs < 0) {
    snprintf(g_create_err, sizeof(g_create_err), "daala_b200_kf_create: mc_refs < 0");
    return nullptr;
  }
  if (cfg && cfg->inter) {
    const char* with = cfg->inter != 1 ? "a value other than 0 or 1"
                       : cfg->dering ? "dering (the all-zero skip map of the deringing stage is a keyframe property)"
                       : cfg->symbol_stream == 1 ? "symbol_stream = 1 (its block record has no DC field; "
                                                   "symbol_stream = 2 is the P-frame stream)"
                       : cfg->noref_prepass ? "noref_prepass"
                       : cfg->level_chains ? "level_chains"
                       : cfg->sb_rows > 0 ? "a row shard (sb_rows > 0)" : nullptr;
    if (with) {
      snprintf(g_create_err, sizeof(g_create_err), "daala_b200_kf_create: inter is not defined with %s", with);
      return nullptr;
    }
  }
  if (!cfg || cfg->pic_w <= 0 || cfg->pic_h <= 0 || cfg->nframes <= 0 || cfg->nframes > 255 || !cfg->qm ||
      !cfg->qm_inv || cfg->qm_stride <= 0)
    return nullptr;
  daala_b200_kf* kf = new (std::nothrow) daala_b200_kf();
  if (!kf) return nullptr;
  kf->cfg = *cfg;
  if (kf->cfg.level_chains && kf->cfg.split_free < 2) kf->cfg.split_free = 2;
  kf->nhsb = (cfg->pic_w + 63) / 64;
  kf->nvsb = (cfg->pic_h + 63) / 64;
  kf->F = cfg->nframes;
  if (kf->cfg.inter_mc && kf->cfg.mc_refs == 0) kf->cfg.mc_refs = (kf->cfg.mc_next ? 3 : 2) * kf->F;
  if (!kf->cfg.inter_mc) kf->cfg.mc_refs = 0;
  kf->slot_filled.assign((size_t)kf->cfg.mc_refs, 0);
  if (kf->cfg.sb_rows <= 0) {
    kf->cfg.sb_row0 = 0;
    kf->cfg.sb_rows = kf->nvsb;
  }
  for (int p = 0; p < 3; p++) {
    kf->plane_w[p] = (kf->nhsb * 64) >> (p ? 1 : 0);
    kf->plane_h[p] = (kf->nvsb * 64) >> (p ? 1 : 0);
  }
  if ((long long)kf->plane_w[0] * kf->plane_h[0] * kf->F >= (1ll << 31)) {
    delete kf;
    return nullptr;
  }
  int dev = 0;
  cudaDeviceProp prop;
  if (cudaGetDevice(&dev) != cudaSuccess || cudaGetDeviceProperties(&prop, dev) != cudaSuccess) {
    delete kf;
    return nullptr;
  }
  kf->sms = prop.multiProcessorCount;
  if (cfg->stream) {
    kf->stream = (cudaStream_t)cfg->stream;
  } else {
    if (cudaStreamCreateWithFlags(&kf->stream, cudaStreamNonBlocking) != cudaSuccess) {
      delete kf;
      return nullptr;
    }
    kf->own_stream = true;
  }
  if (kf_alloc(kf) != 0) {
    fprintf(stderr, "daala_b200_kf_create: %s\n", kf->err);
    snprintf(g_create_err, sizeof(g_create_err), "daala_b200_kf_create: %s", kf->err);
    daala_b200_kf_destroy(kf);
    return nullptr;
  }
  return kf;
}

void daala_b200_kf_destroy(daala_b200_kf* kf) {
  if (!kf) return;
  cudaStreamSynchronize(kf->stream);
  if (kf->exec) cudaGraphExecDestroy(kf->exec);
  if (kf->graph) cudaGraphDestroy(kf->graph);
  if (kf->fin_exec) cudaGraphExecDestroy(kf->fin_exec);
  if (kf->fin_graph) cudaGraphDestroy(kf->fin_graph);
  for (void* p : kf->allocs) cudaFree(p);
  if (kf->own_stream) cudaStreamDestroy(kf->stream);
  delete kf;
}

const char* daala_b200_kf_error(const daala_b200_kf* kf) { return kf ? kf->err : g_create_err; }

#ifdef DAALA_B200_CHAIN_TRACE
int daala_b200_kf_chain_trace(daala_b200_kf* kf, void** recs, int* cap) {
  if (!kf || !recs || !cap) return (int)cudaErrorInvalidValue;
  *recs = kf->luma.trace;
  *cap = kf->luma.trace_cap;
  return 0;
}
#endif

int daala_b200_kf_launches_per_step(const daala_b200_kf* kf) {
  if (!kf) return 0;
  auto split = [](const Stage& S) { return 3 * (S.sp_chunks[0] + S.sp_chunks[1] + S.sp_chunks[2]); };
  if (kf->cfg.inter)
    return 5 + 2 + (2 + split(kf->luma)) + (2 + split(kf->chroma)) + 2 + (kf->cfg.inter_mc ? 2 : 0) +
           (kf->cfg.symbol_stream ? 8 : 0) + (kf->cfg.late_skip ? kLateSkipLaunches : 0);
  int n = 5 + (kf->cfg.level_chains ? 2 : 0);
  n += 1;
  n += 3 + 1 + (kf->cfg.split_free > 1 ? split(kf->luma) : 0) + (kf->luma.pre_ev ? 2 : 0);
  n += 4 + (kf->cfg.split_free > 0 ? split(kf->chroma) : 1);
  n += kf->cfg.dering ? dering_launches(kf->dering) : 2;
  if (kf->cfg.symbol_stream) n += 8;
  return n;
}

int daala_b200_kf_device_buffers(daala_b200_kf* kf, daala_b200_kf_buffers* out) {
  if (!kf || !out) return (int)cudaErrorInvalidValue;
  memset(out, 0, sizeof(*out));
  for (int p = 0; p < 3; p++) {
    out->pixels[p] = kf->pixels[p];
    out->coeffs[p] = kf->coeffs[p];
    out->lapped[p] = kf->lapped[p];
    out->pixels_out[p] = kf->pixels_out[p];
    out->plane_w[p] = kf->plane_w[p];
    out->plane_h[p] = kf->plane_h[p];
  }
  out->bsize = kf->bsize;
  out->counts = kf->lists.cnt;
  out->luma_blocks = kf->lists.luma;
  out->chroma_blocks = kf->lists.chroma;
  out->dep_top = kf->lists.dep_top;
  out->dep_left = kf->lists.dep_left;
  for (int c = 0; c < 3; c++) {
    out->luma_items[c] = kf->lists.items_l[c];
    out->chroma_items[c] = kf->lists.items_c[c];
  }
  out->luma_heads = kf->lists.heads;
  out->luma_heads0 = kf->lists.heads0;
  out->luma_heads_raw = kf->lists.heads_raw;
  out->luma_head_bin = kf->lists.head_bin;
  out->succ_bottom = kf->lists.succ_bottom;
  out->succ_right = kf->lists.succ_right;
  out->luma_res = kf->luma.res_pack;
  out->chroma_res = kf->chroma.res_pack;
  out->luma_y16 = kf->luma.prm.y16;
  out->chroma_y16 = kf->chroma.prm.y16;
  out->luma_skip_diff = kf->luma.prm.res_skip_diff;
  out->chroma_skip_diff = kf->chroma.prm.res_skip_diff;
  out->chroma_flip = kf->chroma.prm.res_flip;
  out->max_luma_blocks = kf->lists.max_luma;
  out->max_chroma_blocks = kf->lists.max_chroma;
  out->stream = kf->stream;
  out->bytes_allocated = (long long)kf->bytes_allocated;
  for (int p = 0; p < 3; p++) {
    out->pred_pixels[p] = kf->pred_pixels[p];
    out->pred_coeffs[p] = kf->pred_coeffs[p];
    out->ref_pixels[p] = kf->ref_pixels[p];
  }
  out->ref_slot = kf->ref_slot;
  out->mv_grid = kf->mv_grid;
  out->mc_refs = kf->cfg.mc_refs;
  out->ref_slot_next = kf->ref_slot_next;
  out->mv1_grid = kf->mv1_grid;
  out->frame_quant = kf->fq;
  return 0;
}

int daala_b200_kf_run_device(daala_b200_kf* kf, int phases, int use_graph) {
  if (!kf) return (int)cudaErrorInvalidValue;
  if (!use_graph || phases != DAALA_B200_KF_ALL) return kf_enqueue_step(kf, phases);
  if (!kf->captured) {
    int rc = kf_enqueue_step(kf, phases);
    if (rc) return rc;
    KF_CHECK(cudaStreamSynchronize(kf->stream));
    KF_CHECK(cudaStreamBeginCapture(kf->stream, cudaStreamCaptureModeThreadLocal));
    rc = kf_enqueue_step(kf, phases);
    cudaError_t e = cudaStreamEndCapture(kf->stream, &kf->graph);
    if (rc) return rc;
    KF_CHECK(e);
    KF_CHECK(cudaGraphInstantiate(&kf->exec, kf->graph, 0));
    kf->captured = true;
  }
  KF_CHECK(cudaGraphLaunch(kf->exec, kf->stream));
  return 0;
}

int daala_b200_kf_time_device(daala_b200_kf* kf, int phases, int use_graph, int reps, float* ms) {
  if (!kf || !ms || reps <= 0) return (int)cudaErrorInvalidValue;
  cudaEvent_t e0, e1;
  KF_CHECK(cudaEventCreate(&e0));
  KF_CHECK(cudaEventCreate(&e1));
  if (use_graph && phases == DAALA_B200_KF_ALL && !kf->captured) {
    int rc = daala_b200_kf_run_device(kf, phases, 1);
    if (rc) return rc;
  }
  KF_CHECK(cudaStreamSynchronize(kf->stream));
  KF_CHECK(cudaEventRecord(e0, kf->stream));
  for (int i = 0; i < reps; i++) {
    int rc = daala_b200_kf_run_device(kf, phases, use_graph);
    if (rc) return rc;
  }
  KF_CHECK(cudaEventRecord(e1, kf->stream));
  KF_CHECK(cudaEventSynchronize(e1));
  KF_CHECK(cudaEventElapsedTime(ms, e0, e1));
  cudaEventDestroy(e0);
  cudaEventDestroy(e1);
  return 0;
}

int daala_b200_kf_count_blocks(const uint8_t* bsize, int nframes, long long frame_pitch, int bstride, int nhsb,
                               int nvsb, int sb_row0, int sb_rows, daala_b200_kf_totals* out) {
  if (!bsize || !out) return (int)cudaErrorInvalidValue;
  long long nl = 0, cl = 0, nc = 0, cc = 0;
  if (sb_rows <= 0) { sb_row0 = 0; sb_rows = nvsb; }
  for (int f = 0; f < nframes; f++) {
    for (int uy = sb_row0 * 8; uy < (sb_row0 + sb_rows) * 8; uy++) {
      const uint8_t* row = bsize + f * frame_pitch + (long long)uy * bstride;
      for (int ux = 0; ux < nhsb * 8; ux++) {
        const int b = row[ux];
        if (b == 0) { nl += 4; cl += 64; nc += 1; cc += 16; continue; }
        const int span = 1 << (b - 1);
        if ((ux & (span - 1)) | (uy & (span - 1))) continue;
        nl += 1;
        cl += b == 1 ? 64 : b == 2 ? 256 : 512;
        nc += 1;
        cc += b == 1 ? 16 : b == 2 ? 64 : b == 3 ? 256 : 512;
      }
    }
  }
  out->n_luma = nl;
  out->luma_coefs = cl;
  out->n_chroma = 2 * nc;
  out->chroma_coefs = 2 * cc;
  return 0;
}

int daala_b200_kf_symbol_bounds(const daala_b200_kf_totals* t, int nframes, daala_b200_kf_sym_bounds* out) {
  if (!t || !out || nframes <= 0) return (int)cudaErrorInvalidValue;
  const long long blocks = t->n_luma + t->n_chroma, coefs = t->luma_coefs + t->chroma_coefs;
  out->index = nframes;
  out->blocks = blocks;
  out->bands = 9 * blocks < coefs / 16 ? 9 * blocks : coefs / 16;
  out->pulse_bytes = 2 * coefs;
  return 0;
}

static int sym_target(const void* p, long long cap, long long need, uint8_t** dev) {
  *dev = nullptr;
  if (!p) return 0;
  if (cap < need) return (int)cudaErrorInvalidValue;
  cudaPointerAttributes a;
  if (cudaPointerGetAttributes(&a, p) != cudaSuccess) {
    cudaGetLastError();
    return (int)cudaErrorInvalidValue;
  }
  if (a.type != cudaMemoryTypeHost || !a.devicePointer) return (int)cudaErrorInvalidValue;
  *dev = (uint8_t*)a.devicePointer;
  return 0;
}

static std::mutex g_compute_mu;
static cudaEvent_t g_last_compute = nullptr;

int daala_b200_kf_submit(daala_b200_kf* kf, const daala_b200_kf_io* io) {
  if (!kf || !io) return (int)cudaErrorInvalidValue;
  cudaStream_t s = kf->stream;
  const int F = kf->F;
  if (!io->bsize) return (int)cudaErrorInvalidValue;
  daala_b200_kf_totals tot;
  if (io->totals) tot = *io->totals;
  else daala_b200_kf_count_blocks(io->bsize, F, (long long)kf->nhsb * 8 * kf->nvsb * 8, kf->nhsb * 8, kf->nhsb, kf->nvsb,
                                  kf->cfg.sb_row0, kf->cfg.sb_rows, &tot);
  if (tot.n_luma > kf->lists.max_luma || tot.n_chroma > kf->lists.max_chroma) return (int)cudaErrorInvalidValue;
  const bool have_pred = io->pred_pixels[0] || io->pred_pixels[1] || io->pred_pixels[2];
  const bool need_dc = kf->cfg.symbol_stream != 2 && (!io->luma_dc || !io->chroma_dc);
  if (kf->cfg.inter && !kf->cfg.inter_mc &&
      (!io->pred_pixels[0] || !io->pred_pixels[1] || !io->pred_pixels[2] || need_dc)) {
    snprintf(kf->err, sizeof(kf->err), "daala_b200_kf_submit: an inter engine needs pred_pixels[0..2], luma_dc and chroma_dc");
    return (int)cudaErrorInvalidValue;
  }
  if ((io->ref_slot_next || io->mv1_grid) && !kf->cfg.mc_next) {
    snprintf(kf->err, sizeof(kf->err), "daala_b200_kf_submit: ref_slot_next and mv1_grid need an engine with mc_next");
    return (int)cudaErrorInvalidValue;
  }
  if (io->ref_resident && !kf->cfg.inter_mc) {
    snprintf(kf->err, sizeof(kf->err), "daala_b200_kf_submit: ref_resident needs an engine with inter_mc");
    return (int)cudaErrorInvalidValue;
  }
  if (kf->cfg.inter_mc) {
    const bool resident = io->ref_resident != 0;
    const bool any_ref = io->ref_pixels[0] || io->ref_pixels[1] || io->ref_pixels[2];
    const char* why = need_dc ? "luma_dc and chroma_dc are required"
                      : !io->mv_grid ? "mv_grid is required"
                      : io->ref_resident != 0 && io->ref_resident != 1 ? "ref_resident is 0 or 1"
                      : resident && any_ref ? "ref_resident: ref_pixels must be NULL (the step reads the pool as it stands)"
                      : resident && io->nrefs != 0 ? "ref_resident: nrefs must be 0"
                      : !resident && (!io->ref_pixels[0] || !io->ref_pixels[1] || !io->ref_pixels[2])
                          ? "ref_pixels[0..2] are required"
                      : !io->ref_slot ? "ref_slot is required"
                      : kf->cfg.mc_next && !io->ref_slot_next ? "mc_next: ref_slot_next is required"
                      : kf->cfg.mc_next && !io->mv1_grid ? "mc_next: mv1_grid is required"
                      : have_pred ? "pred_pixels is refused: the engine makes the prediction"
                      : !resident && (io->nrefs < 1 || io->nrefs > kf->cfg.mc_refs) ? "nrefs is outside [1, mc_refs]"
                                                                                    : nullptr;
    const int nslot = (kf->cfg.mc_next ? 3 : 2) * F;
    bool in_next = false;
    for (int i = 0; !why && i < nslot; i++) {
      const int32_t r = i < 2 * F ? io->ref_slot[i] : io->ref_slot_next[i - 2 * F];
      in_next = i >= 2 * F;
      if (!resident && (r < 0 || r >= io->nrefs)) why = "a ref_slot entry is outside [0, nrefs)";
      else if (resident && (r < 0 || r >= kf->cfg.mc_refs)) why = "ref_resident: a ref_slot entry is outside [0, mc_refs)";
      else if (resident && !kf->slot_filled[r])
        why = "ref_resident: a ref_slot entry names a pool slot that holds no picture (pool_load, a host-upload "
              "submit or a finish with ref_slot_out writes one)";
    }
    if (why) {
      snprintf(kf->err, sizeof(kf->err), "daala_b200_kf_submit: inter_mc: %s%s", why, in_next ? " (ref_slot_next)" : "");
      return (int)cudaErrorInvalidValue;
    }
  }
  const char* ls_why = (io->luma_late_skip || io->chroma_late_skip || io->sym_late_skip) && !kf->cfg.late_skip
                           ? "luma_late_skip / chroma_late_skip / sym_late_skip need an engine with late_skip = 1"
                       : io->sym_late_skip && kf->cfg.symbol_stream != 2
                           ? "sym_late_skip needs an engine with symbol_stream = 2"
                           : nullptr;
  if (ls_why) {
    snprintf(kf->err, sizeof(kf->err), "daala_b200_kf_submit: %s", ls_why);
    return (int)cudaErrorInvalidValue;
  }
  int fq_dc_limit = 0;
  if (io->frame_quant || kf->cfg.frame_quant) {
    const char* why = !kf->cfg.frame_quant ? "frame_quant needs an engine with frame_quant = 1"
                      : !io->frame_quant  ? "frame_quant: the records ([nframes]) are required"
                                          : nullptr;
    for (int f = 0; !why && f < F; f++) {
      const daala_b200_kf_frame_quant& r = io->frame_quant[f];
      if (r.q0 < 1 || r.q0 > DAALA_B200_KF_MAX_Q0) why = "a record's q0 is outside [1, 8191]";
      else if (r.coded_quantizer < 1 || r.coded_quantizer > 63) why = "a record's coded_quantizer is outside [1, 63]";
      else if (!std::isfinite(r.dering_lambda) || r.dering_lambda < 0) why = "a record's dering_lambda is negative or not finite";
      for (int p = 0; !why && p < 3; p++)
        for (int i = 0; i < 30; i++)
          if (r.pvq_qm_q4[p][i] < 1) {
            why = "a record's pvq_qm_q4 entry is 0";
            break;
          }
    }
    if (why) {
      snprintf(kf->err, sizeof(kf->err), "daala_b200_kf_submit: %s", why);
      return (int)cudaErrorInvalidValue;
    }
    fq_dc_limit = daala_b200_kf_frame_quant_derive(io->frame_quant, F,
                                                   reinterpret_cast<int32_t(*)[2][6]>(kf->fq_tbl_host.data()));
  }
  SymCopy sc;
  memset(&sc, 0, sizeof(sc));
  const bool want_sym = io->sym_index || io->sym_blocks || io->sym_bands || io->sym_pulses || io->sym_dc ||
                        io->sym_late_skip;
  if (want_sym) {
    if (!kf->cfg.symbol_stream) return (int)cudaErrorInvalidValue;
    if (io->sym_dc && kf->cfg.symbol_stream != 2) {
      snprintf(kf->err, sizeof(kf->err), "daala_b200_kf_submit: sym_dc needs an engine with symbol_stream = 2");
      return (int)cudaErrorInvalidValue;
    }
    daala_b200_kf_sym_bounds bd;
    daala_b200_kf_symbol_bounds(&tot, F, &bd);
    int e = sym_target(io->sym_index, io->sym_index_cap, bd.index, &sc.dst[0]);
    if (!e) e = sym_target(io->sym_blocks, io->sym_blocks_cap, bd.blocks, &sc.dst[1]);
    if (!e) e = sym_target(io->sym_bands, io->sym_bands_cap, bd.bands, &sc.dst[2]);
    if (!e) e = sym_target(io->sym_pulses, io->sym_pulses_cap, bd.pulse_bytes, &sc.dst[3]);
    if (!e) e = sym_target(io->sym_dc, io->sym_dc_cap, bd.blocks, &sc.dst[4]);
    if (e) return e;
    if (sym_target(io->sym_late_skip, io->sym_late_skip_cap, bd.blocks, &sc.dst[5])) {
      snprintf(kf->err, sizeof(kf->err),
               "daala_b200_kf_submit: sym_late_skip must be pinned host memory of at least "
               "daala_b200_kf_symbol_bounds(...).blocks records");
      return (int)cudaErrorInvalidValue;
    }
    const Sym& Y = kf->sym;
    sc.src[0] = (const uint8_t*)Y.index;
    sc.src[1] = (const uint8_t*)Y.blocks;
    sc.src[2] = (const uint8_t*)Y.bands;
    sc.src[3] = Y.pulses;
    sc.src[4] = (const uint8_t*)Y.dc;
    sc.src[5] = (const uint8_t*)Y.late_skip;
    sc.unit[1] = sizeof(daala_b200_kf_sym_block);
    sc.unit[2] = 4 * sizeof(int16_t);
    sc.unit[3] = 1;
    sc.unit[4] = sizeof(daala_b200_kf_sym_dc);
    sc.unit[5] = sizeof(daala_b200_kf_late_skip);
    sc.index_bytes = (long long)F * sizeof(daala_b200_kf_sym_frame);
    sc.tot = Y.tot;
    const long long host[kSymSegs] = {io->sym_index_cap * (long long)sizeof(daala_b200_kf_sym_frame),
                                      io->sym_blocks_cap * (long long)sizeof(daala_b200_kf_sym_block),
                                      io->sym_bands_cap * 8, io->sym_pulses_cap,
                                      io->sym_dc_cap * (long long)sizeof(daala_b200_kf_sym_dc),
                                      io->sym_late_skip_cap * (long long)sizeof(daala_b200_kf_late_skip)};
    const long long dev[kSymSegs] = {sc.index_bytes, (long long)Y.cap_blocks * (long long)sizeof(daala_b200_kf_sym_block),
                                     Y.cap_bands * 8, Y.cap_bytes,
                                     Y.dc ? (long long)Y.cap_blocks * (long long)sizeof(daala_b200_kf_sym_dc) : 0,
                                     Y.late_skip ? (long long)Y.cap_blocks * (long long)sizeof(daala_b200_kf_late_skip) : 0};
    for (int i = 0; i < kSymSegs; i++) sc.cap[i] = host[i] < dev[i] ? host[i] : dev[i];
  }
  for (int p = 0; p < 3; p++) {
    if (!io->pixels[p]) return (int)cudaErrorInvalidValue;
    KF_CHECK(cudaMemcpyAsync(kf->pixels[p], io->pixels[p], (size_t)kf->plane_w[p] * kf->plane_h[p] * F,
                             cudaMemcpyHostToDevice, s));
    if (kf->cfg.inter_mc) {
      if (!io->ref_resident)
        KF_CHECK(cudaMemcpyAsync(kf->ref_pixels[p], io->ref_pixels[p],
                                 (size_t)kf->plane_w[p] * kf->plane_h[p] * io->nrefs, cudaMemcpyHostToDevice, s));
    } else if (kf->cfg.inter)
      KF_CHECK(cudaMemcpyAsync(kf->pred_pixels[p], io->pred_pixels[p], (size_t)kf->plane_w[p] * kf->plane_h[p] * F,
                               cudaMemcpyHostToDevice, s));
  }
  if (kf->cfg.inter_mc) {
    if (!io->ref_resident) std::fill(kf->slot_filled.begin(), kf->slot_filled.begin() + io->nrefs, 1);
    KF_CHECK(cudaMemcpyAsync(kf->ref_slot, io->ref_slot, sizeof(int32_t) * 2 * F, cudaMemcpyHostToDevice, s));
    KF_CHECK(cudaMemcpyAsync(kf->mv_grid, io->mv_grid,
                             sizeof(daala_b200_mv_pt) * F * (kf->nvsb * 8 + 1) * (kf->nhsb * 8 + 1),
                             cudaMemcpyHostToDevice, s));
    if (kf->cfg.mc_next) {
      KF_CHECK(cudaMemcpyAsync(kf->ref_slot_next, io->ref_slot_next, sizeof(int32_t) * F, cudaMemcpyHostToDevice, s));
      KF_CHECK(cudaMemcpyAsync(kf->mv1_grid, io->mv1_grid,
                               sizeof(int32_t) * 2 * F * (kf->nvsb * 8 + 1) * (kf->nhsb * 8 + 1),
                               cudaMemcpyHostToDevice, s));
    }
  }
  if (kf->cfg.frame_quant) {
    KF_CHECK(cudaMemcpyAsync(kf->fq, io->frame_quant, sizeof(daala_b200_kf_frame_quant) * F, cudaMemcpyHostToDevice, s));
    KF_CHECK(cudaMemcpyAsync(kf->fq_tbl, kf->fq_tbl_host.data(), sizeof(int32_t) * 12 * F, cudaMemcpyHostToDevice, s));
  }
  const size_t map_bytes = (size_t)kf->nhsb * 8 * kf->nvsb * 8 * F;
  KF_CHECK(cudaMemcpyAsync(kf->bsize, io->bsize, map_bytes, cudaMemcpyHostToDevice, s));
  if (kf->cfg.dering == 1) {
    if (!io->dering_level) return (int)cudaErrorInvalidValue;
    KF_CHECK(cudaMemcpyAsync(kf->dering.level, io->dering_level, (size_t)kf->nhsb * kf->nvsb * F, cudaMemcpyHostToDevice, s));
  }
  int rc;
  {
    std::lock_guard<std::mutex> lock(g_compute_mu);
    if (!g_last_compute) KF_CHECK(cudaEventCreateWithFlags(&g_last_compute, cudaEventDisableTiming));
    else if (kf->cfg.level_chains) KF_CHECK(cudaStreamWaitEvent(s, g_last_compute, 0));
    rc = daala_b200_kf_run_device(kf, DAALA_B200_KF_ALL, 1);
    if (rc) return rc;
    KF_CHECK(cudaEventRecord(g_last_compute, s));
  }
  kf->have_step = true;
  kf->last_tot = tot;
  if (kf->cfg.frame_quant) kf->fin_dc_limit = fq_dc_limit;
  for (int p = 0; p < 3; p++)
    if (io->pixels_out[p])
      KF_CHECK(cudaMemcpyAsync(io->pixels_out[p], kf->pixels_out[p], (size_t)kf->plane_w[p] * kf->plane_h[p] * F,
                               cudaMemcpyDeviceToHost, s));
  if (io->luma_blocks) KF_CHECK(cudaMemcpyAsync(io->luma_blocks, kf->lists.luma, sizeof(daala_b200_pvq_block) * tot.n_luma, cudaMemcpyDeviceToHost, s));
  if (io->chroma_blocks) KF_CHECK(cudaMemcpyAsync(io->chroma_blocks, kf->lists.chroma, sizeof(daala_b200_pvq_block) * tot.n_chroma, cudaMemcpyDeviceToHost, s));
  if (io->luma_res) KF_CHECK(cudaMemcpyAsync(io->luma_res, kf->luma.res_pack, 8 * 9 * (size_t)tot.n_luma, cudaMemcpyDeviceToHost, s));
  if (io->chroma_res) KF_CHECK(cudaMemcpyAsync(io->chroma_res, kf->chroma.res_pack, 8 * 9 * (size_t)tot.n_chroma, cudaMemcpyDeviceToHost, s));
  if (io->luma_y16) KF_CHECK(cudaMemcpyAsync(io->luma_y16, kf->luma.prm.y16, 2 * (size_t)tot.luma_coefs, cudaMemcpyDeviceToHost, s));
  if (io->chroma_y16) KF_CHECK(cudaMemcpyAsync(io->chroma_y16, kf->chroma.prm.y16, 2 * (size_t)tot.chroma_coefs, cudaMemcpyDeviceToHost, s));
  if (io->luma_skip_diff) KF_CHECK(cudaMemcpyAsync(io->luma_skip_diff, kf->luma.prm.res_skip_diff, 8 * (size_t)tot.n_luma, cudaMemcpyDeviceToHost, s));
  if (io->chroma_skip_diff) KF_CHECK(cudaMemcpyAsync(io->chroma_skip_diff, kf->chroma.prm.res_skip_diff, 8 * (size_t)tot.n_chroma, cudaMemcpyDeviceToHost, s));
  if (io->chroma_flip) KF_CHECK(cudaMemcpyAsync(io->chroma_flip, kf->chroma.prm.res_flip, 4 * (size_t)tot.n_chroma, cudaMemcpyDeviceToHost, s));
  for (int p = 0; p < 3; p++)
    if (kf->cfg.inter_mc && io->pred_pixels_out[p])
      KF_CHECK(cudaMemcpyAsync(io->pred_pixels_out[p], kf->pred_pixels[p], (size_t)kf->plane_w[p] * kf->plane_h[p] * F,
                               cudaMemcpyDeviceToHost, s));
  if (kf->cfg.inter && io->luma_dc)
    KF_CHECK(cudaMemcpyAsync(io->luma_dc, kf->luma.prm.res_dc, 4 * (size_t)tot.n_luma, cudaMemcpyDeviceToHost, s));
  if (kf->cfg.inter && io->chroma_dc)
    KF_CHECK(cudaMemcpyAsync(io->chroma_dc, kf->chroma.prm.res_dc, 4 * (size_t)tot.n_chroma, cudaMemcpyDeviceToHost, s));
  if (kf->dc_resid[0] && io->luma_dc_resid)
    KF_CHECK(cudaMemcpyAsync(io->luma_dc_resid, kf->dc_resid[0], 4 * (size_t)tot.n_luma, cudaMemcpyDeviceToHost, s));
  if (kf->dc_resid[1] && io->chroma_dc_resid)
    KF_CHECK(cudaMemcpyAsync(io->chroma_dc_resid, kf->dc_resid[1], 4 * (size_t)tot.n_chroma, cudaMemcpyDeviceToHost, s));
  if (io->luma_late_skip)
    KF_CHECK(cudaMemcpyAsync(io->luma_late_skip, kf->late_skip[0], sizeof(daala_b200_kf_late_skip) * tot.n_luma,
                             cudaMemcpyDeviceToHost, s));
  if (io->chroma_late_skip)
    KF_CHECK(cudaMemcpyAsync(io->chroma_late_skip, kf->late_skip[1], sizeof(daala_b200_kf_late_skip) * tot.n_chroma,
                             cudaMemcpyDeviceToHost, s));
  if (io->counts) KF_CHECK(cudaMemcpyAsync(io->counts, kf->lists.cnt, sizeof(int32_t) * 32, cudaMemcpyDeviceToHost, s));
  if (io->dering_level_out && kf->cfg.dering)
    KF_CHECK(cudaMemcpyAsync(io->dering_level_out, kf->dering.level, (size_t)kf->nhsb * kf->nvsb * F, cudaMemcpyDeviceToHost, s));
// ... 153 lines not shown
```

Before: 2353.

## Fork intra keyframe pipeline onto a priority side stream and drop CfL plane

Splits the intra keyframe step across a second high-priority stream with events. The forward transform overlaps list building, chroma PVQ and chroma reconstruction overlap luma scatter and reconstruction, and dering is split per plane. The separate CfL prediction-plane kernel and its buffer are removed; chroma gather now reads luma PVQ input/output coefficients directly through a per-unit offset table, recomputing the 4x4 Haar-based CfL inline. This adds cross-stream ordering complexity and per-lane recomputation in the gather.

Result: faster. 2437 (median of 6 runs) (+3.6%).

```diff
diff --git a/daala_b200/csrc/abi_host.cu b/daala_b200/csrc/abi_host.cu
--- a/daala_b200/csrc/abi_host.cu
+++ b/daala_b200/csrc/abi_host.cu
@@ -14,8 +14,8 @@
 int daala_b200_launch_forward(const FrameXformParams* prm, int nplanes, cudaStream_t stream);
 int daala_b200_launch_forward_no_tma(const FrameXformParams* prm, int nplanes, cudaStream_t stream);
 int daala_b200_launch_inverse(const FrameXformParams* prm, int nplanes, cudaStream_t stream);
-int daala_b200_launch_inverse_lapped_only(const FrameXformParams* prm, int nplanes, cudaStream_t stream);
-int daala_b200_launch_sb_postfilter_store(const FrameXformParams* prm, int nplanes, cudaStream_t stream);
+int daala_b200_launch_inverse_lapped_only(const FrameXformParams* prm, int plane0, int nplanes, cudaStream_t stream);
+int daala_b200_launch_sb_postfilter_store(const FrameXformParams* prm, int plane0, int nplanes, cudaStream_t stream);
 int daala_b200_launch_plane_sb_filter(int32_t* c, int stride, int nhsb, int nvsb, int xdec, int ydec,
                                       int post, cudaStream_t stream);
 int daala_b200_launch_block_transform(int32_t* blocks, int count, int ln, int mode, cudaStream_t stream);
@@ -462,10 +462,10 @@
   return daala_b200_launch_inverse(f, nplanes, (cudaStream_t)stream);
 }
 int daala_b200_inverse_frame_lapped(const daala_b200_frame* f, int nplanes, void* stream) {
-  return daala_b200_launch_inverse_lapped_only(f, nplanes, (cudaStream_t)stream);
+  return daala_b200_launch_inverse_lapped_only(f, 0, nplanes, (cudaStream_t)stream);
 }
 int daala_b200_sb_postfilter_store_frame(const daala_b200_frame* f, int nplanes, void* stream) {
-  return daala_b200_launch_sb_postfilter_store(f, nplanes, (cudaStream_t)stream);
+  return daala_b200_launch_sb_postfilter_store(f, 0, nplanes, (cudaStream_t)stream);
 }
 int daala_b200_plane_sb_filter(int32_t* c, int stride, int nhsb, int nvsb, int xdec, int ydec, int post,
                                void* stream) {
diff --git a/daala_b200/csrc/frame_transform.cu b/daala_b200/csrc/frame_transform.cu
--- a/daala_b200/csrc/frame_transform.cu
+++ b/daala_b200/csrc/frame_transform.cu
@@ -739,15 +739,26 @@
   return (int)cudaGetLastError();
 }
 
-int daala_b200_launch_inverse_lapped_only(const FrameXformParams* prm, int nplanes, cudaStream_t stream) {
+static FrameXformParams plane_range(const FrameXformParams* prm, int plane0) {
+  FrameXformParams q = *prm;
+  for (int p = 0; p + plane0 < 3; p++) {
+    q.plane[p] = prm->plane[plane0 + p];
+    q.post16[p] = prm->post16[plane0 + p];
+  }
+  return q;
+}
+
+int daala_b200_launch_inverse_lapped_only(const FrameXformParams* prm, int plane0, int nplanes, cudaStream_t stream) {
+  if (plane0 < 0 || nplanes < 1 || plane0 + nplanes > 3) return (int)cudaErrorInvalidValue;
   dim3 grid(prm->nhsb * prm->sb_rows, nplanes, prm->nframes);
-  k_inverse_sb<<<grid, kThreads, 0, stream>>>(*prm);
-  return (int)cudaGetLastError();
-}
-
-int daala_b200_launch_sb_postfilter_store(const FrameXformParams* prm, int nplanes, cudaStream_t stream) {
+  k_inverse_sb<<<grid, kThreads, 0, stream>>>(plane_range(prm, plane0));
+  return (int)cudaGetLastError();
+}
+
+int daala_b200_launch_sb_postfilter_store(const FrameXformParams* prm, int plane0, int nplanes, cudaStream_t stream) {
+  if (plane0 < 0 || nplanes < 1 || plane0 + nplanes > 3) return (int)cudaErrorInvalidValue;
   dim3 grid(prm->nhsb * prm->sb_rows, nplanes, prm->nframes);
-  k_sb_postfilter_store<<<grid, kPostThreads, 0, stream>>>(*prm);
+  k_sb_postfilter_store<<<grid, kPostThreads, 0, stream>>>(plane_range(prm, plane0));
   return (int)cudaGetLastError();
 }
 
diff --git a/daala_b200/csrc/kf_engine.cu b/daala_b200/csrc/kf_engine.cu
--- a/daala_b200/csrc/kf_engine.cu
+++ b/daala_b200/csrc/kf_engine.cu
@@ -60,6 +60,7 @@
   int ntiles;
   int4* tile_sum;
   int32_t* unit_lbase;
+  int32_t* unit_loff;
   daala_b200_pvq_block* luma;
   daala_b200_pvq_block* chroma;
   int32_t* dep_top;
@@ -201,6 +202,7 @@
   L.unit_lbase[((long long)f * L.UH + uy) * L.UW + ux] = pre.x;
   if (v.x == 0) return;
   if (pre.x + v.x > L.max_luma || 2 * (pre.z + v.z) > L.max_chroma) return;
+  if (L.unit_loff) L.unit_loff[((long long)f * L.UH + uy) * L.UW + ux] = pre.y;
   if (b == 0) {
     for (int q = 0; q < 4; q++)
       put_block(L.luma + pre.x + q, pre.y + 16 * q, ux * 8 + (q & 1) * 4, uy * 8 + (q >> 1) * 4, 0, 0, 0, f);
@@ -447,9 +449,9 @@
   int skip_lo;
   const double* rsqrt_tbl;
   int16_t* res_pack;
-  const int32_t* cfl_plane;
-  long long cfl_pitch;
-  int cfl_stride;
+  const int32_t* cfl_in;
+  const int32_t* cfl_out;
+  const int32_t* cfl_loff;
   int32_t* dc_resid;
   const daala_b200_kf_frame_quant* fq;
 #ifdef DAALA_B200_CHAIN_TRACE
@@ -495,6 +497,25 @@
   S.trace[i] = r;
 }
 #endif
+
+__constant__ int kCflScaling4[4][4] = {{128, 128, 100, 36}, {128, 80, 71, 35}, {100, 71, 35, 31}, {36, 35, 31, 18}};
+
+__device__ __forceinline__ int32_t cfl_ref(const Stage& S, const daala_b200_pvq_block& b, int lo, int i) {
+  if (!(b.xdec & 0x80)) return i == 0 ? S.cfl_in[lo] : S.cfl_out[lo + i];
+  int r = 0, c = 0;
+  if (i) scan_rc(i, &r, &c);
+  const int y = r >> 1, x = c >> 1, at = y + 2 * x;
+  int ll = at ? S.cfl_out[lo + at] : S.cfl_in[lo];
+  int lh = at ? S.cfl_out[lo + 16 + at] : S.cfl_in[lo + 16];
+  int hl = at ? S.cfl_out[lo + 32 + at] : S.cfl_in[lo + 32];
+  int hh = at ? S.cfl_out[lo + 48 + at] : S.cfl_in[lo + 48];
+  ll += lh; hh -= hl;
+  const int t = (ll - hh) >> 1;
+  hl = t - hl; lh = t - lh;
+  ll -= hl; hh += lh;
+  const int v = r == 3 * y ? (c == 3 * x ? ll : lh) : (c == 3 * x ? hl : hh);
+  return (kCflScaling4[c][r] * v + 64) >> 7;
+}
 
 enum { kGatherLuma = 0, kGatherChroma = 1, kGatherInter = 2 };
 template <int kKind>
@@ -521,13 +542,14 @@
         vref[i] = psrc[at];
       }
     } else {
-      const int32_t* psrc = S.cfl_plane + b.frame * S.cfl_pitch + (size_t)b.y0 * S.cfl_stride + b.x0;
+      const int lo = S.cfl_loff[b.frame * (prm.plane_frame_pitch[b.pli] >> 4) + (long long)(b.y0 >> 2) * (stride >> 2) +
+                                (b.x0 >> 2)];
       int32_t* vref = prm.ref + b.coef_off;
       const int qoff = prm.qm_stride + ((((1 << (2 * b.bs)) - 1) << 4) / 3);
       int32_t xy = 0;
       for (int i = lane; i < len; i += 32) {
         const int32_t vi = i == 0 ? src[0] : src[scan_to_raster(i, ln, stride)];
-        const int32_t vr = i == 0 ? psrc[0] : psrc[scan_to_raster(i, ln, S.cfl_stride)];
+        const int32_t vr = cfl_ref(S, b, lo, i);
         vin[i] = vi;
         vref[i] = vr;
         if (i >= 1 && i < 16) {
@@ -544,45 +566,6 @@
         for (int i = 1 + lane; i < end; i += 32) vref[i] = -vref[i];
       }
       if (lane == 0) prm.res_flip[blk] = flip;
-    }
-  }
-}
-
-__global__ void __launch_bounds__(256) k_cfl_plane(const __grid_constant__ Stage S, int32_t* pred_plane) {
-  const daala_b200_pvq_params& prm = S.prm;
-  const int n = min(S.cnt[S.n_blocks_at], S.max_blocks);
-  const int lane = threadIdx.x & 31;
-  const int nwarps = (gridDim.x * blockDim.x) >> 5;
-  for (int blk = (blockIdx.x * blockDim.x + threadIdx.x) >> 5; blk < n; blk += nwarps) {
-    const daala_b200_pvq_block b = prm.blocks[blk];
-    if (b.pli != 1) continue;
-    const int nn = 4 << b.bs;
-    const int lstride = prm.plane_stride[0];
-    const int32_t* luma = prm.coef_plane[0] + b.frame * prm.plane_frame_pitch[0] + (size_t)(2 * b.y0) * lstride + 2 * b.x0;
-    int32_t* dst = pred_plane + b.frame * S.cfl_pitch + (size_t)b.y0 * S.cfl_stride + b.x0;
-    if (b.xdec & 0x80) {
-      const int scaling4[4][4] = {{128, 128, 100, 36}, {128, 80, 71, 35}, {100, 71, 35, 31}, {36, 35, 31, 18}};
-      if (lane < 4) {
-        const int x = lane & 1, y = lane >> 1;
-        int ll = luma[(size_t)y * lstride + x], lh = luma[(size_t)y * lstride + x + 4];
-        int hl = luma[(size_t)(y + 4) * lstride + x], hh = luma[(size_t)(y + 4) * lstride + x + 4];
-        ll += lh; hh -= hl;
-        const int t = (ll - hh) >> 1;
-        hl = t - hl; lh = t - lh;
-        ll -= hl; hh += lh;
-        const int hs = x & 1, vs = y & 1;
-        int r, c;
-        r = 2 * y + vs; c = 2 * x + hs;         dst[(size_t)r * S.cfl_stride + c] = (scaling4[c][r] * ll + 64) >> 7;
-        r = 2 * y + vs; c = 2 * x + 1 - hs;     dst[(size_t)r * S.cfl_stride + c] = (scaling4[c][r] * lh + 64) >> 7;
-        r = 2 * y + 1 - vs; c = 2 * x + hs;     dst[(size_t)r * S.cfl_stride + c] = (scaling4[c][r] * hl + 64) >> 7;
-        r = 2 * y + 1 - vs; c = 2 * x + 1 - hs; dst[(size_t)r * S.cfl_stride + c] = (scaling4[c][r] * hh + 64) >> 7;
-      }
-    } else {
-      const int lim = nn > 32 ? 32 : nn;
-      for (int i = lane; i < lim * lim; i += 32) {
-        const int r = i / lim, c = i % lim;
-        dst[(size_t)r * S.cfl_stride + c] = luma[(size_t)r * lstride + c];
-      }
     }
   }
 }
@@ -940,9 +923,10 @@
   if (i < kTableDoubles) pvq_fill_rsqrt_table(tbl, i);
 }
 
-__global__ void k_begin_pvq(int32_t* cnt, int luma) {
+enum { kBeginLuma = 1, kBeginChroma = 2 };
+__global__ void k_begin_pvq(int32_t* cnt, int stages) {
   if (threadIdx.x == 0 && blockIdx.x == 0) {
-    if (luma) {
+    if (stages & kBeginLuma) {
       cnt[kHeadLoL] = 0;
       cnt[kHeadHi] = 0;
       cnt[kTailHi] = cnt[kNHeads0];
@@ -952,9 +936,8 @@
 #ifdef DAALA_B200_CHAIN_TRACE
       cnt[kTraceN] = 0;
 #endif
-    } else {
-      cnt[kHeadLoC] = 0;
-    }
+    }
+    if (stages & kBeginChroma) cnt[kHeadLoC] = 0;
   }
 }
 
@@ -1440,8 +1423,10 @@
 
 extern "C" int daala_b200_launch_forward(const daala_b200_frame* prm, int nplanes, cudaStream_t stream);
 extern "C" int daala_b200_launch_inverse(const daala_b200_frame* prm, int nplanes, cudaStream_t stream);
-extern "C" int daala_b200_launch_inverse_lapped_only(const daala_b200_frame* prm, int nplanes, cudaStream_t stream);
-extern "C" int daala_b200_launch_sb_postfilter_store(const daala_b200_frame* prm, int nplanes, cudaStream_t stream);
+extern "C" int daala_b200_launch_inverse_lapped_only(const daala_b200_frame* prm, int plane0, int nplanes,
+                                                     cudaStream_t stream);
+extern "C" int daala_b200_launch_sb_postfilter_store(const daala_b200_frame* prm, int plane0, int nplanes,
+                                                     cudaStream_t stream);
 
 struct Dering {
   daala_b200_frame frame;
@@ -1459,12 +1444,16 @@
   daala_b200_dering_search_batch sb;
 };
 
+enum { kEvLists, kEvForward, kEvLumaBands, kEvLumaScatter, kEvChroma, kNumEvents };
+
 struct daala_b200_kf {
   daala_b200_kf_config cfg;
   int nhsb, nvsb, F;
   int plane_w[3], plane_h[3];
   cudaStream_t stream;
   bool own_stream;
+  cudaStream_t side;
+  cudaEvent_t ev[kNumEvents];
   cudaGraph_t graph;
   cudaGraphExec_t exec;
   bool captured;
@@ -1475,7 +1464,6 @@
   uint8_t* pred_pixels[3];
   int32_t* pred_coeffs[3];
   uint8_t* bsize;
-  int32_t* cfl_plane;
   int16_t *qm, *qm_inv;
   double* rsqrt_tbl;
   int16_t* sp_vec[3];
@@ -1575,7 +1563,6 @@
   }
   const int UW = kf->nhsb * 8, UH = kf->nvsb * 8;
   KF_CHECK(dalloc(kf, &kf->bsize, (size_t)F * UW * UH));
-  if (!inter) KF_CHECK(dalloc(kf, &kf->cfl_plane, (size_t)kf->plane_w[1] * kf->plane_h[1] * F));
   if (kf->cfg.inter_mc) {
     daala_b200_mc_batch& B = kf->mc;
     const size_t nsb = (size_t)kf->nhsb * kf->nvsb;
@@ -1633,6 +1620,7 @@
   L.max_chroma = (int)(nunits * 2 / div) + 64;
   KF_CHECK(dalloc(kf, &L.tile_sum, (size_t)L.ntiles));
   KF_CHECK(dalloc(kf, &L.unit_lbase, (size_t)F * UW * UH));
+  if (!inter) KF_CHECK(dalloc(kf, &L.unit_loff, (size_t)F * UW * UH));
   KF_CHECK(dalloc(kf, &L.luma, (size_t)L.max_luma));
   KF_CHECK(dalloc(kf, &L.chroma, (size_t)L.max_chroma));
   const size_t ndep = inter ? 0 : (size_t)L.max_luma;
@@ -1784,10 +1772,6 @@
       S.heads0 = L.heads0;
       KF_CHECK(dalloc(kf, &S.ring, inter ? 0 : kf->chain_cap));
       KF_CHECK(dalloc(kf, &S.join0, ndep));
-    } else {
-      S.cfl_plane = kf->cfl_plane;
-      S.cfl_pitch = (long long)kf->plane_w[1] * kf->plane_h[1];
-      S.cfl_stride = kf->plane_w[1];
     }
     return 0;
   };
@@ -1795,6 +1779,12 @@
   if (rc) return rc;
   rc = setup_stage(kf->chroma, true);
   if (rc) return rc;
+  if (!inter) {
+    Stage& C = kf->chroma;
+    C.cfl_in = kf->luma.prm.in;
+    C.cfl_out = kf->luma.prm.out;
+    C.cfl_loff = L.unit_loff;
+  }
   (void)luma_px;
   if (kf->cfg.inter_finish || kf->cfg.symbol_stream == 2)
     for (int c = 0; c < 2; c++) {
@@ -2051,43 +2041,56 @@
   return 0;
 }
 
-static int enqueue_dering(daala_b200_kf* kf, const Dering& D, cudaStream_t s) {
-  int rc = daala_b200_launch_inverse_lapped_only(&D.frame, 3, s);
-  if (!rc) rc = daala_b200_launch_sb_postfilter_store(&D.frame, 3, s);
-  if (!rc && D.search) rc = daala_b200_dering_search_enqueue(&D.sb, s);
-  if (rc) return rc;
+static int enqueue_recon(const daala_b200_frame& frame, int p0, int n, cudaStream_t s) {
+  const int rc = daala_b200_launch_inverse_lapped_only(&frame, p0, n, s);
+  return rc ? rc : daala_b200_launch_sb_postfilter_store(&frame, p0, n, s);
+}
+
+static int enqueue_dering_plane(daala_b200_kf* kf, const Dering& D, int p, cudaStream_t s) {
+  const int nsb = kf->nhsb * kf->nvsb;
+  const long long per = (long long)kf->plane_w[p] * kf->plane_h[p];
+  daala_b200_dering_params dp;
+  memset(&dp, 0, sizeof(dp));
+  dp.y = nullptr;
+  dp.x = D.frame.post16[p];
+  dp.dir = D.dir;
+  dp.bskip = D.skip[p];
+  dp.sb_threshold = D.thr[p ? 1 : 0];
+  dp.ystride = dp.xstride = kf->plane_w[p];
+  dp.dir_stride = kf->nhsb * 8;
+  dp.skip_stride = D.skip_stride;
+  dp.nhsb = kf->nhsb;
+  dp.nvsb = kf->nvsb;
+  dp.xdec = p ? 1 : 0;
+  dp.pli = p;
+  dp.overlap = 1;
+  dp.coeff_shift = 4;
+  dp.dir_format = D.search ? 2 : 0;
+  return daala_b200_dering_plane_frames(&dp, kf->F, per, per, (long long)nsb * 64, nsb, D.skip_pitch[p],
+                                        D.frame.plane[p].pixels_out, s);
+}
+
+static int enqueue_dering_luma(daala_b200_kf* kf, const Dering& D, cudaStream_t s) {
+  if (D.search) {
+    const int rc = daala_b200_dering_search_enqueue(&D.sb, s);
+    if (rc) return rc;
+  }
   const int nsb = kf->nhsb * kf->nvsb;
   k_dering_thresholds<<<(kf->F * nsb + 255) / 256, 256, 0, s>>>(
       D.level, D.thr[0], D.thr[1], kf->F * nsb, make_int4(D.tbl[0][0], D.tbl[0][1], D.tbl[0][2], D.tbl[0][3]),
       make_int2(D.tbl[0][4], D.tbl[0][5]), make_int4(D.tbl[1][0], D.tbl[1][1], D.tbl[1][2], D.tbl[1][3]),
       make_int2(D.tbl[1][4], D.tbl[1][5]), D.coded, D.applied, D.frame_tbl, nsb);
-  for (int p = 0; p < 3; p++) {
-    const long long per = (long long)kf->plane_w[p] * kf->plane_h[p];
-    daala_b200_dering_params dp;
-    memset(&dp, 0, sizeof(dp));
-    dp.y = nullptr;
-    dp.x = D.frame.post16[p];
-    dp.dir = D.dir;
-    dp.bskip = D.skip[p];
-    dp.sb_threshold = D.thr[p ? 1 : 0];
-    dp.ystride = dp.xstride = kf->plane_w[p];
-    dp.dir_stride = kf->nhsb * 8;
-    dp.skip_stride = D.skip_stride;
-    dp.nhsb = kf->nhsb;
-    dp.nvsb = kf->nvsb;
-    dp.xdec = p ? 1 : 0;
-    dp.pli = p;
-    dp.overlap = 1;
-    dp.coeff_shift = 4;
-    dp.dir_format = D.search ? 2 : 0;
-    rc = daala_b200_dering_plane_frames(&dp, kf->F, per, per, (long long)nsb * 64, nsb, D.skip_pitch[p],
-                                        D.frame.plane[p].pixels_out, s);
-    if (rc) return rc;
-  }
-  return 0;
-}
-
-static int dering_launches(const Dering& D) { return 1 + 1 + (D.search ? 5 + 6 + 6 + 1 : 0) + 1 + 3; }
+  return enqueue_dering_plane(kf, D, 0, s);
+}
+
+static int enqueue_dering(daala_b200_kf* kf, const Dering& D, cudaStream_t s) {
+  int rc = enqueue_recon(D.frame, 0, 3, s);
+  if (!rc) rc = enqueue_dering_luma(kf, D, s);
+  for (int p = 1; !rc && p < 3; p++) rc = enqueue_dering_plane(kf, D, p, s);
+  return rc;
+}
+
+static int dering_launches(const Dering& D, int parts) { return 2 * parts + (D.search ? 5 + 6 + 6 + 1 : 0) + 1 + 3; }
 
 template <bool kZeroRef, bool kFq = false>
 static void enqueue_split(daala_b200_kf* kf, const Stage& S, cudaStream_t s) {
@@ -2166,60 +2169,111 @@
   return (int)cudaGetLastError();
 }
 
+static int enqueue_lists(daala_b200_kf* kf, cudaStream_t s) {
+  const Lists& L = kf->lists;
+  const int wide = kf->sms * 8;
+  k_unit_tile_sums<<<L.ntiles, kTile, 0, s>>>(L);
+  k_tile_scan<<<1, 1024, 0, s>>>(L);
+  k_unit_emit<<<L.ntiles, kTile, 0, s>>>(L);
+  const size_t nl = (size_t)L.max_luma * sizeof(int32_t);
+  if (cudaMemsetAsync(L.succ_bottom, 0xff, nl, s) != cudaSuccess || cudaMemsetAsync(L.succ_right, 0xff, nl, s) != cudaSuccess)
+    return (int)cudaGetLastError();
+  if (L.lvl_hist && cudaMemsetAsync(L.lvl_hist, 0, sizeof(int32_t) * kLevelBins, s) != cudaSuccess) return (int)cudaGetLastError();
+  if (cudaMemsetAsync(L.head_hist, 0, sizeof(int32_t) * kLevelBins, s) != cudaSuccess) return (int)cudaGetLastError();
+  k_luma_deps<<<wide, 256, 0, s>>>(L);
+  if (L.lvl_hist) {
+    k_level_scan<<<1, 1024, 0, s>>>(L);
+    k_level_scatter<<<wide, 256, 0, s>>>(L);
+  }
+  k_chroma_items<<<wide, 256, 0, s>>>(L);
+  return 0;
+}
+
+static int enqueue_luma_bands(daala_b200_kf* kf, bool core, int begin, cudaStream_t s) {
+  const int wide = kf->sms * 8;
+  const int persist = kf->sms * (kf->cfg.persist_ctas_per_sm > 0 ? kf->cfg.persist_ctas_per_sm : kPersistCtas);
+  if (cudaMemsetAsync(kf->luma.ring, 0xff, kf->chain_cap * sizeof(uint32_t), s) != cudaSuccess ||
+      cudaMemsetAsync(kf->luma.join0, 0, (size_t)kf->luma.max_blocks * sizeof(int32_t), s) != cudaSuccess)
+    return (int)cudaGetLastError();
+  k_begin_pvq<<<1, 32, 0, s>>>(kf->lists.cnt, begin);
+  if (!core) k_gather<kGatherLuma><<<wide, 256, 0, s>>>(kf->luma);
+  if (kf->cfg.split_free > 1) enqueue_split<true>(kf, kf->luma, s);
+  if (kf->luma.pre_ev) {
+    k_pvq_prepass<2><<<kf->sms * 16, 128, 0, s>>>(kf->luma);
+    k_pvq_prepass<1><<<kf->sms * 16, 128, 0, s>>>(kf->luma);
+  }
+  if (kf->cfg.level_chains) {
+    if (cudaMemsetAsync(kf->lv_bar, 0, sizeof(int32_t) * 32, s) != cudaSuccess) return (int)cudaGetLastError();
+    k_pvq_levels<<<kf->lvl_grid, 128, 0, s>>>(kf->luma);
+  } else {
+    k_pvq_persist<true><<<persist, kPersistThreads, 0, s>>>(kf->luma);
+  }
+  return 0;
+}
+
+static void enqueue_chroma(daala_b200_kf* kf, bool core, bool begin, cudaStream_t s) {
+  const int wide = kf->sms * 8;
+  if (begin) k_begin_pvq<<<1, 32, 0, s>>>(kf->lists.cnt, kBeginChroma);
+  if (!core) k_gather<kGatherChroma><<<wide, 256, 0, s>>>(kf->chroma);
+  if (kf->cfg.split_free > 0) enqueue_split<false>(kf, kf->chroma, s);
+  else k_pvq_persist<false><<<kf->sms * (kf->cfg.persist_ctas_per_sm > 0 ? kf->cfg.persist_ctas_per_sm : kPersistCtas),
+                              kPersistThreads, 0, s>>>(kf->chroma);
+  if (!core) k_finish_scatter<false><<<wide, 256, 0, s>>>(kf->chroma);
+}
+
+static int kf_enqueue_step_forked(daala_b200_kf* kf) {
+  cudaStream_t s = kf->stream, c = kf->side;
+  const daala_b200_frame& fr = kf->cfg.dering ? kf->dering.frame : kf->frame;
+  auto fork = [](cudaEvent_t e, cudaStream_t from, cudaStream_t to) {
+    return cudaEventRecord(e, from) == cudaSuccess && cudaStreamWaitEvent(to, e, 0) == cudaSuccess;
+  };
+  if (!fork(kf->ev[kEvLists], s, c)) return (int)cudaGetLastError();
+  int rc = daala_b200_launch_forward(&kf->frame, 3, c);
+  if (!rc) rc = enqueue_lists(kf, s);
+  if (rc) return rc;
+  if (!fork(kf->ev[kEvForward], c, s)) return (int)cudaGetLastError();
+  rc = enqueue_luma_bands(kf, false, kBeginLuma | kBeginChroma, s);
+  if (rc) return rc;
+  if (!fork(kf->ev[kEvLumaBands], s, c)) return (int)cudaGetLastError();
+  enqueue_chroma(kf, false, false, c);
+  k_finish_scatter<false><<<kf->sms * 128, 256, 0, s>>>(kf->luma);
+  if (kf->cfg.symbol_stream) {
+    if (!fork(kf->ev[kEvLumaScatter], s, c)) return (int)cudaGetLastError();
+    enqueue_sym<false>(kf->sym, kf->sms * 8, c);
+  }
+  rc = enqueue_recon(fr, 1, 2, c);
+  if (!rc) rc = enqueue_recon(fr, 0, 1, s);
+  if (!rc && kf->cfg.dering) rc = enqueue_dering_luma(kf, kf->dering, s);
+  if (rc) return rc;
+  if (!fork(kf->ev[kEvChroma], c, s)) return (int)cudaGetLastError();
+  for (int p = 1; kf->cfg.dering && p < 3; p++) {
+    rc = enqueue_dering_plane(kf, kf->dering, p, s);
+    if (rc) return rc;
+  }
+  return (int)cudaGetLastError();
+}
+
 static int kf_enqueue_step(daala_b200_kf* kf, int phases) {
   if (kf->cfg.inter) return kf_enqueue_step_inter(kf, phases);
+  if (phases == DAALA_B200_KF_ALL) return kf_enqueue_step_forked(kf);
   cudaStream_t s = kf->stream;
-  const Lists& L = kf->lists;
-  const int wide = kf->sms * 8;
   if (phases & DAALA_B200_KF_LISTS) {
-    k_unit_tile_sums<<<L.ntiles, kTile, 0, s>>>(L);
-    k_tile_scan<<<1, 1024, 0, s>>>(L);
-    k_unit_emit<<<L.ntiles, kTile, 0, s>>>(L);
-    const size_t nl = (size_t)L.max_luma * sizeof(int32_t);
-    if (cudaMemsetAsync(L.succ_bottom, 0xff, nl, s) != cudaSuccess || cudaMemsetAsync(L.succ_right, 0xff, nl, s) != cudaSuccess)
-      return (int)cudaGetLastError();
-    if (L.lvl_hist && cudaMemsetAsync(L.lvl_hist, 0, sizeof(int32_t) * kLevelBins, s) != cudaSuccess) return (int)cudaGetLastError();
-    if (cudaMemsetAsync(L.head_hist, 0, sizeof(int32_t) * kLevelBins, s) != cudaSuccess) return (int)cudaGetLastError();
-    k_luma_deps<<<wide, 256, 0, s>>>(L);
-    if (L.lvl_hist) {
-      k_level_scan<<<1, 1024, 0, s>>>(L);
-      k_level_scatter<<<wide, 256, 0, s>>>(L);
-    }
-    k_chroma_items<<<wide, 256, 0, s>>>(L);
+    const int rc = enqueue_lists(kf, s);
+    if (rc) return rc;
   }
   if (phases & DAALA_B200_KF_FORWARD) {
-    int rc = daala_b200_launch_forward(&kf->frame, 3, s);
+    const int rc = daala_b200_launch_forward(&kf->frame, 3, s);
     if (rc) return rc;
   }
-  const int persist = kf->sms * (kf->cfg.persist_ctas_per_sm > 0 ? kf->cfg.persist_ctas_per_sm : kPersistCtas);
   const bool core = (phases & DAALA_B200_KF_SEARCH_ONLY) != 0;
   if (phases & DAALA_B200_KF_PVQ_LUMA) {
-    if (cudaMemsetAsync(kf->luma.ring, 0xff, kf->chain_cap * sizeof(uint32_t), s) != cudaSuccess ||
-        cudaMemsetAsync(kf->luma.join0, 0, (size_t)kf->luma.max_blocks * sizeof(int32_t), s) != cudaSuccess)
-      return (int)cudaGetLastError();
-    k_begin_pvq<<<1, 32, 0, s>>>(kf->lists.cnt, 1);
-    if (!core) k_gather<kGatherLuma><<<wide, 256, 0, s>>>(kf->luma);
-    if (kf->cfg.split_free > 1) enqueue_split<true>(kf, kf->luma, s);
-    if (kf->luma.pre_ev) {
-      k_pvq_prepass<2><<<kf->sms * 16, 128, 0, s>>>(kf->luma);
-      k_pvq_prepass<1><<<kf->sms * 16, 128, 0, s>>>(kf->luma);
-    }
-    if (kf->cfg.level_chains) {
-      if (cudaMemsetAsync(kf->lv_bar, 0, sizeof(int32_t) * 32, s) != cudaSuccess) return (int)cudaGetLastError();
-      k_pvq_levels<<<kf->lvl_grid, 128, 0, s>>>(kf->luma);
-    } else {
-      k_pvq_persist<true><<<persist, kPersistThreads, 0, s>>>(kf->luma);
-    }
-    if (!core) k_finish_scatter<false><<<wide, 256, 0, s>>>(kf->luma);
+    const int rc = enqueue_luma_bands(kf, core, kBeginLuma, s);
+    if (rc) return rc;
+    if (!core) k_finish_scatter<false><<<kf->sms * 8, 256, 0, s>>>(kf->luma);
   }
   if (phases & DAALA_B200_KF_PVQ_CHROMA) {
-    k_begin_pvq<<<1, 32, 0, s>>>(kf->lists.cnt, 0);
-    if (!core) k_cfl_plane<<<wide, 256, 0, s>>>(kf->chroma, kf->cfl_plane);
-    if (!core) k_gather<kGatherChroma><<<wide, 256, 0, s>>>(kf->chroma);
-    if (kf->cfg.split_free > 0) enqueue_split<false>(kf, kf->chroma, s);
-    else k_pvq_persist<false><<<persist, kPersistThreads, 0, s>>>(kf->chroma);
-    if (!core) k_finish_scatter<false><<<wide, 256, 0, s>>>(kf->chroma);
-    if (!core && kf->cfg.symbol_stream) enqueue_sym<false>(kf->sym, wide, s);
+    enqueue_chroma(kf, core, true, s);
+    if (!core && kf->cfg.symbol_stream) enqueue_sym<false>(kf->sym, kf->sms * 8, s);
   }
   if (phases & DAALA_B200_KF_INVERSE) {
     int rc = kf->cfg.dering ? enqueue_dering(kf, kf->dering, s) : daala_b200_launch_inverse(&kf->frame, 3, s);
@@ -2335,6 +2389,17 @@
     }
     kf->own_stream = true;
   }
+  if (!cfg->inter) {
+    int least = 0, greatest = 0;
+    bool ok = cudaDeviceGetStreamPriorityRange(&least, &greatest) == cudaSuccess &&
+              cudaStreamCreateWithPriority(&kf->side, cudaStreamNonBlocking, greatest) == cudaSuccess;
+    for (int i = 0; ok && i < kNumEvents; i++) ok = cudaEventCreateWithFlags(&kf->ev[i], cudaEventDisableTiming) == cudaSuccess;
+    if (!ok) {
+      snprintf(g_create_err, sizeof(g_create_err), "daala_b200_kf_create: cannot create the second stream and its events");
+      daala_b200_kf_destroy(kf);
+      return nullptr;
+    }
+  }
   if (kf_alloc(kf) != 0) {
     fprintf(stderr, "daala_b200_kf_create: %s\n", kf->err);
     snprintf(g_create_err, sizeof(g_create_err), "daala_b200_kf_create: %s", kf->err);
@@ -2352,6 +2417,9 @@
   if (kf->fin_exec) cudaGraphExecDestroy(kf->fin_exec);
   if (kf->fin_graph) cudaGraphDestroy(kf->fin_graph);
   for (void* p : kf->allocs) cudaFree(p);
+  for (cudaEvent_t e : kf->ev)
+    if (e) cudaEventDestroy(e);
+  if (kf->side) cudaStreamDestroy(kf->side);
   if (kf->own_stream) cudaStreamDestroy(kf->stream);
   delete kf;
 }
@@ -2376,8 +2444,8 @@
   int n = 5 + (kf->cfg.level_chains ? 2 : 0);
   n += 1;
   n += 3 + 1 + (kf->cfg.split_free > 1 ? split(kf->luma) : 0) + (kf->luma.pre_ev ? 2 : 0);
-  n += 4 + (kf->cfg.split_free > 0 ? split(kf->chroma) : 1);
-  n += kf->cfg.dering ? dering_launches(kf->dering) : 2;
+  n += 2 + (kf->cfg.split_free > 0 ? split(kf->chroma) : 1);
+  n += kf->cfg.dering ? dering_launches(kf->dering, 2) : 4;
   if (kf->cfg.symbol_stream) n += 8;
   return n;
 }
@@ -2446,7 +2514,7 @@
     cudaError_t e = cudaStreamEndCapture(kf->stream, &kf->graph);
     if (rc) return rc;
     KF_CHECK(e);
-    KF_CHECK(cudaGraphInstantiate(&kf->exec, kf->graph, 0));
+    KF_CHECK(cudaGraphInstantiate(&kf->exec, kf->graph, cudaGraphInstantiateFlagUseNodePriority));
     kf->captured = true;
   }
   KF_CHECK(cudaGraphLaunch(kf->exec, kf->stream));
```
